# ka9q/ka9q-radio

Hardware: AMD Instinct MI355X
Metric: channels sustained @129.6 MS/s input (real-time-equivalent: channel-blocks/s / 50) (higher is better)
Workload: dtype f32; 1 GPU; config3: sig_gen real 129.6 MS/s, 1024 mixed usb/cw/iq 12 kHz channels (P=300), 1 MI355X; channels_total=1024, P=300, olen=240, N=3240000, L=2592000, M=648001, lanes=4

## Files before the change

include/chz_engine.h:

```cpp
#ifndef CHZ_ENGINE_H
#define CHZ_ENGINE_H
#include <stddef.h>
#ifdef __cplusplus
extern "C" {
#endif

#define CHZ_COMPLEX 1
#define CHZ_REAL    2
#define CHZ_ND      4

typedef struct chz_engine chz_engine;

typedef struct chz_info {
  int L, M, N, in_type, bins;
  int ring_blocks;
  int Na, Nb, Nc;
  int n_banks;
  int lanes;
  long spec_elems;
  int spec_na, spec_pitch, spec_off;
  char plan[320];
} chz_info;

typedef struct chz_timing {
  double total_ms;
  int blocks;
  double first_ms, cols_ms, rows_ms, notch_ms, chan_ms;
  int first_n, cols_n, rows_n, notch_n, chan_n;
  double enqueue_ms;
  double fix_ms; int fix_n;
  double demod_ms; int demod_n;
} chz_timing;

const char *chz_last_error(void);
int chz_process_exiting(void);
int chz_set_option(const char *name, const char *value);
int chz_device_count(void);

int chz_engine_create(chz_engine **out, int L, int M, int in_type, int device,
                      const char *plan_spec, int ring_blocks);
void chz_engine_destroy(chz_engine *e);
int chz_engine_info(const chz_engine *e, chz_info *info);
int chz_engine_set_stream(chz_engine *e, void *hip_stream);
int chz_sync(chz_engine *e);
int chz_engine_check(const chz_engine *e);

int chz_input_write(chz_engine *e, const float *host_samples, long n);
int chz_input_write_device(chz_engine *e, const float *dev_samples, long n);
int chz_input_write_i16(chz_engine *e, const short *host_samples, long n, float scale, int randomize);
int chz_input_write_i16_device(chz_engine *e, const short *dev_samples, long n, float scale, int randomize);
int chz_input_stats(chz_engine *e, int slot, unsigned long long *energy, unsigned *clips);
int chz_input_ring(chz_engine *e, float **dev_ring, long *ring_len_floats);
int chz_input_seek(chz_engine *e, unsigned job, const float *history);
int chz_input_mark(chz_engine *e, int k);
int chz_input_mark_wait(chz_engine *e, int k);
int chz_engine_notch_order(chz_engine *e, int by_event);

int chz_forward(chz_engine *e, unsigned job);
int chz_set_notches(chz_engine *e, const int *bins, int n, double alpha);
int chz_set_notches_alpha(chz_engine *e, const int *bins, const double *alpha, int n);
int chz_spectrum_read(chz_engine *e, int slot, float *host);
int chz_spectrum_device(chz_engine *e, int slot, float **dev);
int chz_slot_stream(chz_engine *e, int slot, void **hip_stream);
int chz_spectrum_attach(chz_engine *e, int slot, float *dev);

int chz_bank_create(chz_engine *e, int P, int olen, int capacity);
int chz_bank_create_real(chz_engine *e, int P, int olen, int capacity);
int chz_bank_create_shared(chz_engine *e, int P, int olen, int capacity, int nrows);
int chz_bank_set_rows(chz_engine *e, int bank, int ch0, int n, const int *rows);
int chz_bank_set_row_responses(chz_engine *e, int bank, int row0, int n, const float *resp);
int chz_bank_set_responses(chz_engine *e, int bank, int ch0, int n, const float *resp);
int chz_bank_set_shifts(chz_engine *e, int bank, int ch0, int n, const int *shifts);
int chz_bank_set_isb(chz_engine *e, int bank, int ch0, int n, const unsigned char *flags);
int chz_bank_set_beam(chz_engine *e, int bank, int ch0, int n, const double *ab, const unsigned char *on);
int chz_bank_set_active(chz_engine *e, int bank, int n);
int chz_bank_execute(chz_engine *e, int bank, unsigned job);
int chz_bank_execute_range(chz_engine *e, int bank, unsigned job, int ch0, int n);

int chz_bank_set_tuning(chz_engine *e, int bank, unsigned job, int ch0, int n, const int *shifts,
                        const double *freq, const double *rate);
int chz_bank_read_power(chz_engine *e, int bank, int slot, int ch0, int n, double *host);
int chz_bank_read_power_async(chz_engine *e, int bank, int slot, int ch0, int n, double *host);

int chz_bank_enable_noise(chz_engine *e, int bank, double samprate);
int chz_bank_read_noise(chz_engine *e, int bank, int slot, int ch0, int n, double *host);
int chz_bank_read_noise_async(chz_engine *e, int bank, int slot, int ch0, int n, double *host);
int chz_bank_destroy(chz_engine *e, int bank);
int chz_bank_read(chz_engine *e, int bank, int ch0, int n, float *host);
int chz_bank_read_async(chz_engine *e, int bank, int slot, int ch0, int n, float *host);
int chz_spectrum_read_async(chz_engine *e, int slot, float *host);
int chz_host_callback(chz_engine *e, int slot, void (*fn)(void *), void *arg);
int chz_slot_sync(chz_engine *e, int slot);
int chz_host_alloc(void **p, size_t bytes);
void chz_host_free(void *p);
int chz_host_register(void *p, size_t bytes);
void chz_host_unregister(void *p);
int chz_bank_output_device(chz_engine *e, int bank, int slot, float **dev);

int chz_step(chz_engine *e, unsigned job);

int chz_run_blocks(chz_engine *e, unsigned job0, int nblocks, int mode, int instrument,
                   chz_timing *timing);

#define CHZ_COMM_ID_BYTES 128
typedef struct chz_comm chz_comm;
int chz_comm_unique_id(void *id128);
int chz_comm_create(chz_comm **out, int rank, int world, const void *id128, int device);
int chz_comm_create_file(chz_comm **out, int rank, int world, const char *path, int device, double timeout_s);
int chz_comm_create_local(chz_comm **out, int n, const int *devices);
int chz_spectrum_broadcast_local(chz_engine *const *engines, chz_comm *const *comms, int n, int slot, int root);
void chz_comm_destroy(chz_comm *c);
int chz_comm_rank(const chz_comm *c);
int chz_comm_world(const chz_comm *c);
int chz_comm_barrier(chz_comm *c);
int chz_comm_allreduce_max(chz_comm *c, double *v, int n);
int chz_spectrum_broadcast(chz_engine *e, chz_comm *c, int slot, int root);
int chz_spectrum_exchange_rows(chz_engine *e, chz_comm *c, int slot, int root, const int *row_lo, const int *row_hi);
int chz_run_blocks_sharded(chz_engine *e, chz_comm *c, int root, int mode, const int *row_lo, const int *row_hi,
                           unsigned job0, int nblocks, chz_timing *timing);

#define CHZ_PCM_S16BE 0
#define CHZ_PCM_S16LE 1
#define CHZ_PCM_F32LE 2
#define CHZ_PCM_F32BE 3
#define CHZ_PCM_MULAW 4
#define CHZ_PCM_ALAW 5
#define CHZ_PCM_F16LE 6
#define CHZ_PCM_F16BE 7
typedef struct chz_demod_params {
  int channels;
  int env;
  int agc;
  int encoding;
  int snr_squelch;
  int squelch_tail;
  int tuned;
  int kind;
  double samprate;
  double headroom;
  double threshold, recovery_rate, hangtime, dc_alpha;
  double bandwidth;
  double shift;
  double squelch_open, squelch_close;
  double gain;
  double deemph_rate, deemph_gain;
  double threshold_extend;
  int pll_enable;
  int pll_square;
  double pll_loop_bw;
  double tone_freq;
} chz_demod_params;
#define CHZ_DEMOD_LINEAR 0
#define CHZ_DEMOD_FM 1
typedef struct chz_demod_status {
  int frame;
  int mute;
  int squelch_state;
  int pll_lock;
  double output_power;
  double gain;
  double n0;
  double snr;
  double foffset;
  double pdeviation;
  double pll_snr;
  double pll_cphase;
  double tone_deviation;
  int pll_rotations;
  int tone_mute;
} chz_demod_status;
int chz_bank_set_demod(chz_engine *e, int bank, unsigned job, int ch0, int n, const chz_demod_params *p, double blocktime);
int chz_bank_write_block(chz_engine *e, int bank, int slot, int ch0, int n, const float *samples, const double *bb_power, const double *n0);
int chz_bank_demod(chz_engine *e, int bank, unsigned job, int slot);
int chz_bank_demod_auto(chz_engine *e, int bank, int on);
int chz_bank_pcm_stride(chz_engine *e, int bank);
int chz_bank_set_pcm_stride(chz_engine *e, int bank, int bytes);
int chz_bank_read_pcm(chz_engine *e, int bank, int slot, int ch0, int n, void *pcm, chz_demod_status *status);
int chz_bank_read_pcm_async(chz_engine *e, int bank, int slot, int ch0, int n, void *pcm, chz_demod_status *status);
#define CHZ_FLAG_NO_SAMPLES 1
#define CHZ_FLAG_MUTE 2
#define CHZ_FLAG_PLL_LOCK 4
#define CHZ_FLAG_TONE_MUTE 8
int chz_bank_read_pcm_flags_async(chz_engine *e, int bank, int slot, int ch0, int n, void *pcm, unsigned char *flags);
int chz_bank_pcm_wait(chz_engine *e, int bank, int slot);

typedef struct chz_mini chz_mini;
int chz_mini_create(chz_mini **out, int L, int M, int capacity, int device);
void chz_mini_destroy(chz_mini *m);
int chz_mini_capacity(const chz_mini *m);
int chz_mini_add(chz_mini *m);
int chz_mini_release(chz_mini *m, int inst);
int chz_mini_set_response(chz_mini *m, int inst, const float *resp);
int chz_mini_execute(chz_mini *m, int n, const int *inst, const float *const *win, const int *shift, const unsigned char *isb,
                     float *const *out);

typedef struct chz_rmini chz_rmini;
int chz_rmini_create(chz_rmini **out, int L, int M, int nslaves, const int *olen, const int *out_type, int capacity, int device);
void chz_rmini_destroy(chz_rmini *m);
int chz_rmini_check(int L, int M, int nslaves, const int *olen, const int *out_type);
int chz_rmini_capacity(const chz_rmini *m);
int chz_rmini_add(chz_rmini *m);
int chz_rmini_release(chz_rmini *m, int inst);
int chz_rmini_set_response(chz_rmini *m, int inst, int slave, const float *resp);
int chz_rmini_execute(chz_rmini *m, int n, const int *inst, const float *const *win, const int *shift, const unsigned char *mask,
                      const unsigned char *isb, float *const *out);

int chz_welch_create(chz_engine *e, int fft_n, int capacity, int max_bins, int max_avg);
int chz_welch_destroy(chz_engine *e, int bank);
int chz_welch_set_window(chz_engine *e, int bank, int slot, const float *window);
// ... 21 lines not shown
```

ka9q-radio_amd/csrc/chz_engine.hip:

```cpp
#include <hip/hip_runtime.h>
#include <hip/hip_ext.h>
#include <atomic>
#include <condition_variable>
#include <cstdarg>
#include <cstdio>
#include <cstring>
#include <chrono>
#include <deque>
#include <functional>
#include <mutex>
#include <string>
#include <algorithm>
#include <vector>
#include <thread>
#include <cmath>
#include <unistd.h>
namespace chz_exit {
static std::atomic<int> exiting{0};
static std::atomic<long> inflight{0};
struct Scope {
  bool ok;
  Scope() { inflight.fetch_add(1, std::memory_order_seq_cst); ok = exiting.load(std::memory_order_seq_cst) == 0; }
  ~Scope() { inflight.fetch_sub(1, std::memory_order_release); }
};
// ... 47 lines not shown
  unsigned char* isb = nullptr;
  BeamDesc* beam = nullptr;
  std::vector<std::pair<int, int>> dirty[CHZ_ND];
  char* stage[CHZ_ND] = {nullptr, nullptr, nullptr, nullptr};
  hipEvent_t stage_ev[CHZ_ND][2] = {};
  bool stage_busy[CHZ_ND][2] = {};
  int stage_next[CHZ_ND] = {0, 0, 0, 0};
  float2* any_scratch = nullptr;
  DemodChan* dm_chan = nullptr;
  DemodState* dm_state = nullptr;
  DemodExt* dm_ext = nullptr;
  float2* dm_mix = nullptr;
  int dm_pll_lin = 0;
  int dm_fm_pll = 0, dm_fm_tone = 0;
  int dm_lin = 0, dm_fm = 0;
  int dm_fm_nopll = 0;
  DemodStatus* dm_status = nullptr;
  unsigned char* dm_flags = nullptr;
  unsigned char* dm_pcm = nullptr;
  std::vector<DemodChan> dm_chan_h;
  struct OscHost { bool init = false; double freq = 0.0, phase0 = 0.0; unsigned job0 = 0; };
  std::vector<OscHost> dm_osc;
  int shared_rows = 0;
  int dm_on = 0;
  bool dm_auto = true;
  int pcm_stride = 0;
  double dm_blocktime = 0.02;
  hipEvent_t ev_bank[CHZ_ND] = {nullptr, nullptr, nullptr, nullptr};
  hipEvent_t ev_tail[CHZ_ND] = {nullptr, nullptr, nullptr, nullptr};
  hipEvent_t ev_pcm[CHZ_ND] = {nullptr, nullptr, nullptr, nullptr};
  hipEvent_t ev_pcmgo[CHZ_ND] = {nullptr, nullptr, nullptr, nullptr};
  bool pcm_copying[CHZ_ND] = {false, false, false, false};
  bool tail_used[CHZ_ND] = {false, false, false, false};
  double* power = nullptr;
  double* agc_peak = nullptr;
  bool agc_peak_valid[CHZ_ND] = {false, false, false, false};
  double* n0 = nullptr;
  unsigned* noise_hint = nullptr;
  double noise_samprate = 0.0;
  BbRing* bb = nullptr;
  std::vector<BbRing> bb_h;
  int bb_n = 0;
  hipEvent_t ev_bb[CHZ_ND] = {nullptr, nullptr, nullptr, nullptr};
  bool bb_rec[CHZ_ND] = {false, false, false, false};
  unsigned bb_newest = 0;
  hipEvent_t bb_done = nullptr;
  int bb_busy = 0; unsigned bb_guard = 0;
};

struct Lane {
  hipStream_t s = nullptr;
  float2* buf = nullptr;
};

struct Issuer {
  std::thread th;
  std::mutex m;
  std::condition_variable cv;
  std::atomic<int> state{0};
  std::atomic<int> ready{0};
  bool sleeping = false;
  std::function<void()> fn;
  void loop() {
    for (;;) {
      const auto awake_until = std::chrono::steady_clock::now() + std::chrono::milliseconds(1);
      unsigned spins = 0;
      for (;;) {
        const int s = state.load(std::memory_order_acquire);
        if (s == 1 || s == 3) break;
        if ((++spins & 255u) || std::chrono::steady_clock::now() < awake_until) { __builtin_ia32_pause(); continue; }
        std::unique_lock<std::mutex> lk(m);
        sleeping = true;
        cv.wait(lk, [&] { const int t = state.load(std::memory_order_acquire); return t == 1 || t == 3; });
        sleeping = false;
      }
      if (state.load(std::memory_order_acquire) == 3) return;
      fn();
      state.store(2, std::memory_order_release);
    }
  }
  void post(std::function<void()> f) {
    fn = std::move(f);
    std::lock_guard<std::mutex> lk(m);
    state.store(1, std::memory_order_release);
    if (sleeping) cv.notify_one();
  }
  void wait() {
    while (state.load(std::memory_order_acquire) != 2) __builtin_ia32_pause();
    state.store(0, std::memory_order_release);
  }
  void quit() {
    { std::lock_guard<std::mutex> lk(m); state.store(3, std::memory_order_release); cv.notify_one(); }
    if (th.joinable()) th.join();
  }
};

struct NotchTurn {
  std::atomic<int> next{0};
  std::atomic<int> next_tail{0};
  std::atomic<int> abort{0};
};

#define CHZ_NOTCH_EVENTS 8
struct WelchBank;

struct chz_engine {
  int L = 0, M = 0, N = 0, in_type = 0, bins = 0, per = 1, device = 0, ring_blocks = 0;
  FwdPlan plan;
  float* energy[CHZ_ND] = {nullptr, nullptr, nullptr, nullptr};
  int noise_energy = -1;
  int demod_wave = -1;
  int chan_stage = -1;
  hipStream_t stream = nullptr;
  bool own_stream = false;
  hipStream_t upload = nullptr;
  hipStream_t tail = nullptr;
  hipStream_t pcmcopy = nullptr;
  Lane lanes[CHZ_MAX_LANES];
  int nlanes = 1;
#define CHZ_INPUT_MARKS 8
  hipEvent_t input_mark[CHZ_INPUT_MARKS] = {};
  hipEvent_t input_ready = nullptr;
  bool input_pending = false;
  float* ring = nullptr; long ring_len = 0;
  short* ring16 = nullptr; float scale16 = 1.0f; int derand = 0;
  unsigned long long* energy_part = nullptr; unsigned* clip_part = nullptr; int stat_n = 0;
  long wpos = 0;
  float2* spec[CHZ_ND] = {nullptr, nullptr, nullptr, nullptr};
  bool spec_owned[CHZ_ND] = {false, false, false, false};
  struct Blue {
    FwdPlan zp; long Mz = 0;
    float2* chirp = nullptr;
    float2* bf = nullptr;
    float2* za[CHZ_MAX_LANES] = {};
    float2* zs[CHZ_MAX_LANES] = {};
  };
  Blue* blue = nullptr;
  float2 *tw_sub_a = nullptr, *tw_sub_b = nullptr, *tw_sub_c = nullptr;
  float2 *tw1_tile = nullptr, *tw1_col = nullptr, *tw2_tile = nullptr, *tw2_col = nullptr, *tw2_full = nullptr;
  int n_notch = 0;
  int *notch_addr = nullptr, *notch_next = nullptr, *notch_head = nullptr;
  double* notch_alpha = nullptr; double* notch_state = nullptr;
  hipEvent_t notch_ev[CHZ_NOTCH_EVENTS] = {};
  unsigned notch_seq = 0; bool notch_have = false;
  bool opt_noise_hint = true, opt_pll_lane0 = false, opt_notch_fold = true;
  int notch_order = 0;
  long long notch_max_wait = 0;
  unsigned* notch_ver = nullptr;
  unsigned notch_tickets = 0;
  unsigned* notch_err = nullptr;
  NotchTables notch_tab; std::vector<double> notch_alpha_h;
  NotchOwn* notch_own = nullptr;
  RowsNotch notch_fold{};
  std::vector<Bank> banks;
  std::vector<WelchBank*> welch;
  hipStream_t welch_s = nullptr;
  hipEvent_t welch_in = nullptr, welch_done = nullptr;
  bool welch_busy = false;
  long long welch_lo = 0, welch_len = 0;
  hipGraphExec_t graph = nullptr; unsigned graph_job0 = 0; int graph_blocks = 0;
  int capture_blocks = 0;
  int graph_min_blocks = 32;
  hipEvent_t ev_t0 = nullptr, ev_t1 = nullptr, ev_fork = nullptr, ev_join[CHZ_MAX_LANES] = {nullptr, nullptr, nullptr, nullptr};
  hipEvent_t ev_begin[CHZ_MAX_LANES] = {nullptr, nullptr, nullptr, nullptr}, ev_end[CHZ_MAX_LANES] = {nullptr, nullptr, nullptr, nullptr}, ev_end_tail = nullptr;
  int tail_issued = 0;
  std::vector<Issuer*> issuers;
};

extern "C" { static int sync_all(chz_engine* e); }

template <class T> static int upload(T** dst, const std::vector<f2>& v) {
  *dst = nullptr;
  if (v.empty()) return 0;
  HIPOK(hipMalloc((void**)dst, v.size() * sizeof(f2)));
  HIPOK(hipMemcpy(*dst, v.data(), v.size() * sizeof(f2), hipMemcpyHostToDevice));
  return 0;
}

static void welch_free_all(chz_engine* e);
static void welch_bank_gone(chz_engine* e, int bank);
static int welch_guard(chz_engine* e, long long pos, long long n) {
  if (!e->welch_busy || n <= 0) return 0;
  const long long R = e->ring_len / e->per;
  { chz_exit::Scope xs; if (!xs.ok) return 0;
    if (hipEventQuery(e->welch_done) == hipSuccess) { e->welch_busy = false; return 0; }
    (void)hipGetLastError(); }
  const long long d1 = ((pos - e->welch_lo) % R + R) % R, d2 = ((e->welch_lo - pos) % R + R) % R;
  if (!(d1 < e->welch_len || d2 < n)) return 0;
  HIPOK(hipStreamWaitEvent(e->stream, e->welch_done, 0));
  e->welch_busy = false;
  return 0;
}

static void free_bank(Bank& b) {
  hipFree(b.resp); hipFree(b.desc); hipFree(b.out); hipFree(b.tw_sub); hipFree(b.any_scratch); b.any_scratch = nullptr;
  hipFree(b.fine); hipFree(b.power); hipFree(b.n0); hipFree(b.noise_hint); b.noise_hint = nullptr; hipFree(b.isb); hipFree(b.beam); hipFree(b.agc_peak); b.agc_peak = nullptr;
  hipFree(b.dm_chan); hipFree(b.dm_state); hipFree(b.dm_ext); hipFree(b.dm_status); hipFree(b.dm_flags); hipFree(b.dm_pcm); hipFree(b.dm_mix);
  b.dm_mix = nullptr; b.dm_pll_lin = 0; b.dm_fm_pll = 0; b.dm_fm_tone = 0; b.dm_lin = 0; b.dm_fm = 0; b.dm_fm_nopll = 0;
  b.dm_chan = nullptr; b.dm_state = nullptr; b.dm_ext = nullptr; b.dm_status = nullptr; b.dm_flags = nullptr; b.dm_pcm = nullptr; b.dm_on = 0; b.dm_chan_h.clear(); b.dm_osc.clear();
  for (int s = 0; s < CHZ_ND; s++) {
    if (b.ev_bank[s]) (void)hipEventDestroy(b.ev_bank[s]);
    if (b.ev_tail[s]) (void)hipEventDestroy(b.ev_tail[s]);
    if (b.ev_pcm[s]) (void)hipEventDestroy(b.ev_pcm[s]);
    if (b.ev_pcmgo[s]) (void)hipEventDestroy(b.ev_pcmgo[s]);
    b.ev_bank[s] = b.ev_tail[s] = b.ev_pcm[s] = b.ev_pcmgo[s] = nullptr; b.tail_used[s] = false; b.pcm_copying[s] = false;
  }
  hipFree(b.bb); b.bb = nullptr; b.bb_h.clear(); b.bb_n = 0; b.bb_busy = 0;
  if (b.bb_done) (void)hipEventDestroy(b.bb_done);
  b.bb_done = nullptr;
  for (int s = 0; s < CHZ_ND; s++) { if (b.ev_bb[s]) (void)hipEventDestroy(b.ev_bb[s]); b.ev_bb[s] = nullptr; b.bb_rec[s] = false; }
  for (int s = 0; s < CHZ_ND; s++) {
    if (b.stage[s]) (void)hipHostFree(b.stage[s]);
    for (int h = 0; h < 2; h++) { if (b.stage_ev[s][h]) (void)hipEventDestroy(b.stage_ev[s][h]); b.stage_ev[s][h] = nullptr; b.stage_busy[s][h] = false; }
    b.stage[s] = nullptr; b.stage_next[s] = 0; b.dirty[s].clear();
  }
  for (auto& r : b.retired) for (auto ev : r.ev) if (ev) (void)hipEventDestroy(ev);
  b.retired.clear(); b.free_rows.clear();
  b.resp = nullptr; b.desc = nullptr; b.out = nullptr; b.tw_sub = nullptr; b.fine = nullptr; b.power = nullptr;
  b.n0 = nullptr; b.isb = nullptr; b.beam = nullptr; b.noise_samprate = 0.0;
  b.desc_h.clear(); b.fine_h.clear(); b.fine_dh.clear(); b.isb_h.clear(); b.beam_h.clear();
  b.active = 0; b.cap = 0;
}

extern "C" {

int chz_process_exiting(void) { return chz_exit::exiting.load(std::memory_order_acquire); }
const char* chz_last_error(void) { return g_err; }

int chz_device_count(void) {
  int n = 0;
  if (hipGetDeviceCount(&n) != hipSuccess) return 0;
  return n;
}

int chz_gather_descriptor(int in_type, int master_bins, int P, int shift, int out6[6]) {
  ChanDescH d = make_chan_desc(in_type, master_bins, P, shift);
  out6[0] = d.t0; out6[1] = d.cnt; out6[2] = d.src0; out6[3] = d.dir; out6[4] = d.conj; out6[5] = d.wrap;
  return 0;
}

struct ChzOptions {
  int chan_stage = -1;
  int noise_energy = -1;
  int demod_wave = -1;
  int enq_threads = 2;
  int graph_blocks = 32;
  int notch_fold = 1;
  int noise_hint = 1;
  int pll_lane0 = 0;
  double notch_wait_ms = 3000.0;
  int fault_ticket_skew = 0;
  int allow_fault_injection = 0;
  int welch_packed = 1;
  char launch_id[64] = {0};
};
static ChzOptions g_opt;
static std::mutex g_opt_mu;
extern "C" int chz_set_option(const char* name, const char* value) {
  if (!name) return fail(-1, "null option name");
  std::lock_guard<std::mutex> lk(g_opt_mu);
  const ChzOptions def{};
  const bool d = value == nullptr || value[0] == 0;
  const int iv = d ? 0 : atoi(value);
  const std::string n(name);
  if (n == "chan_stage") g_opt.chan_stage = d ? def.chan_stage : (iv != 0);
  else if (n == "noise_energy") g_opt.noise_energy = d ? def.noise_energy : (iv != 0);
  else if (n == "demod_wave") g_opt.demod_wave = d ? def.demod_wave : (iv != 0);
  else if (n == "enq_threads") g_opt.enq_threads = d ? def.enq_threads : ((iv == 2 || iv == 4) ? iv : 1);
  else if (n == "graph_blocks") g_opt.graph_blocks = (d || iv <= 0 || iv > 4096) ? def.graph_blocks : iv;
  else if (n == "notch_fold") g_opt.notch_fold = d ? def.notch_fold : (value[0] != '0');
  else if (n == "noise_hint") g_opt.noise_hint = d ? def.noise_hint : (value[0] != '0');
  else if (n == "pll_lane0") g_opt.pll_lane0 = d ? def.pll_lane0 : 1;
  else if (n == "notch_wait_ms") g_opt.notch_wait_ms = (d || !(atof(value) > 0)) ? def.notch_wait_ms : atof(value);
  else if (n == "fault_ticket_skew") g_opt.fault_ticket_skew = d ? 0 : iv;
  else if (n == "allow_fault_injection") g_opt.allow_fault_injection = d ? 0 : (value[0] == '1');
  else if (n == "welch_packed") g_opt.welch_packed = d ? def.welch_packed : (iv != 0);
  else if (n == "launch_id") snprintf(g_opt.launch_id, sizeof g_opt.launch_id, "%s", d ? "" : value);
  else return fail(-1, "unknown option '%s'", name);
  return 0;
}
static ChzOptions options() { std::lock_guard<std::mutex> lk(g_opt_mu); return g_opt; }

static int own_queues() { static const int m = [] { const char* v = getenv("CHZ_OWN_QUEUES"); const int k = v ? atoi(v) : 1; return (k >= 0 && k <= 4) ? k : 1; }(); return m; }
static hipError_t stream_create_masked(hipStream_t* s, bool tail) {
#ifndef HIPEMU
  if (tail && own_queues() >= 3) {
    int lo = 0, hi = 0;
    if (hipDeviceGetStreamPriorityRange(&lo, &hi) == hipSuccess && lo != hi) {
      const hipError_t r = hipStreamCreateWithPriority(s, hipStreamNonBlocking, own_queues() == 3 ? hi : lo);
      if (r == hipSuccess) return r;
      (void)hipGetLastError();
    }
    return hipStreamCreateWithFlags(s, hipStreamNonBlocking);
  }
  if (own_queues() == 2 || (own_queues() == 1 && tail)) {
    int dev = 0, cus = 0;
    if (hipGetDevice(&dev) == hipSuccess && hipDeviceGetAttribute(&cus, hipDeviceAttributeMultiprocessorCount, dev) == hipSuccess && cus > 0 && cus <= 1024) {
      uint32_t mask[32] = {};
      for (int i = 0; i < cus; i++) mask[i / 32] |= 1u << (i % 32);
      const hipError_t r = hipExtStreamCreateWithCUMask(s, (uint32_t)((cus + 31) / 32), mask);
      if (r == hipSuccess) return r;
      (void)hipGetLastError();
    }
  }
#endif
  (void)tail;
  return hipStreamCreateWithFlags(s, hipStreamNonBlocking);
}

static int blue_setup(chz_engine* e);
int chz_engine_create(chz_engine** out, int L, int M, int in_type, int device, const char* plan_spec, int ring_blocks) {
  if (!out) return fail(-1, "null out pointer");
  *out = nullptr;
  if (L < 1 || M < 1) return fail(-1, "bad L/M");
  if (in_type != CHZ_REAL && in_type != CHZ_COMPLEX) return fail(-1, "in_type must be REAL or COMPLEX");
  int ndev = 0;
  if (hipGetDeviceCount(&ndev) != hipSuccess || ndev < 1)
    return fail(-2, "no HIP device: the channelizer engine has no CPU fallback");
  if (device < 0 || device >= ndev) return fail(-2, "device %d out of range (%d devices)", device, ndev);
  HIPOK(hipSetDevice(device));
  { void* probe = nullptr; HIPOK(hipMalloc(&probe, 256)); HIPOK(hipFree(probe)); }
  chz_exit::arm();
  const int N = L + M - 1;
  const int bins = in_type == CHZ_COMPLEX ? N : N / 2 + 1;
  if (bins < 2) return fail(-1, "transform too small");
  if (in_type == CHZ_REAL && (L & 1)) return fail(-1, "real input needs an even block length L");
  chz_engine* e = new chz_engine();
  struct Guard { chz_engine* e; ~Guard() { if (e) chz_engine_destroy(e); } } guard{e};
  e->L = L; e->M = M; e->N = N; e->in_type = in_type; e->bins = bins; e->device = device;
  e->per = in_type == CHZ_REAL ? 1 : 2;
  const char* envspec = getenv("CHZ_PLAN");
  if ((!plan_spec || !*plan_spec) && envspec && *envspec) plan_spec = envspec;
  if (!build_fwd_plan(N, in_type, plan_spec, e->plan)) {
    if (plan_spec && *plan_spec)
      return fail(-3, "no transform plan for N=%d (spec '%s'): N must factor into the compiled axis lengths, and no pass may want more than 1024 threads or 160 KB of LDS", N, plan_spec);
    chz_engine::Blue* bl = new chz_engine::Blue();
    e->blue = bl;
    double best = 1e300;
    for (long m = 2L * N - 1; m <= 4L * N + 4096 && m < (1L << 30); m++) {
      if (bl->Mz && (double)m > 1.04 * (double)bl->Mz + 64) break;
      { long r = m;
        for (int q : {2, 3, 5, 13, 19}) while (r % q == 0) r /= q;
        if (r != 1) continue; }
      FwdPlan cand; double sc = 0.0;
      if (!build_fwd_plan((int)m, CHZ_COMPLEX, nullptr, cand, &sc)) continue;
      if (!bl->Mz) bl->Mz = m;
      sc *= (double)m;
      if (sc < best) { best = sc; bl->zp = cand; }
    }
    if (bl->Mz) bl->Mz = bl->zp.N;
    if (!bl->Mz) return fail(-3, "no transform plan for N=%d, and no planned length above 2N-1 for the chirp-z form either", N);
    FwdPlan& q = e->plan;
    q = FwdPlan();
    q.N = N; q.in_type = in_type; q.bins = bins; q.Na = 128; q.Nb = 1; q.Nc = (bins + 127) / 128;
    q.spec_pitch = 128; q.spec_off = 0; q.spec_elems = (long)q.Nc * 128 + 16;
    char d[256];
    snprintf(d, sizeof d, "N=%d %s as chirp-z over [%s]", N, in_type == CHZ_REAL ? "real" : "complex", bl->zp.desc.c_str());
    q.desc = d;
  }
  const FwdPlan& tp = e->blue ? e->blue->zp : e->plan;
  if (fwd_lds_prepare(tp, !e->blue && in_type == CHZ_REAL))
    return fail(-3, "the forward kernels of N=%d (%s) cannot have the LDS their tiles need", N, tp.desc.c_str());
  const int minblocks = (N + L - 1) / L + 1;
  if (ring_blocks < minblocks) ring_blocks = minblocks < 8 ? 8 : minblocks;
  e->ring_blocks = ring_blocks;
  e->ring_len = (long)ring_blocks * L * e->per;
  HIPOK(stream_create_masked(&e->stream, false));
  e->own_stream = true;
  const ChzOptions opt = options();
  e->opt_noise_hint = opt.noise_hint != 0; e->opt_pll_lane0 = opt.pll_lane0 != 0; e->opt_notch_fold = opt.notch_fold != 0;
  if (opt.chan_stage >= 0) e->chan_stage = opt.chan_stage;
  if (opt.noise_energy >= 0) e->noise_energy = opt.noise_energy;
  if (opt.demod_wave >= 0) e->demod_wave = opt.demod_wave;
  const char* envl = getenv("CHZ_STREAMS");
  int nl = envl ? atoi(envl) : 4;
  e->nlanes = (nl >= 4) ? 4 : (nl >= 2) ? 2 : 1;
  HIPOK(hipEventCreateWithFlags(&e->input_ready, hipEventDisableTiming));
  HIPOK(hipEventCreate(&e->ev_t0)); HIPOK(hipEventCreate(&e->ev_t1));
  HIPOK(hipEventCreateWithFlags(&e->ev_fork, hipEventDisableTiming));
  for (int i = 0; i < CHZ_MAX_LANES; i++) HIPOK(hipEventCreateWithFlags(&e->ev_join[i], hipEventDisableTiming));
  for (int i = 0; i < CHZ_MAX_LANES; i++) { HIPOK(hipEventCreate(&e->ev_begin[i])); HIPOK(hipEventCreate(&e->ev_end[i])); }
  HIPOK(hipEventCreate(&e->ev_end_tail));
  for (int i = 0; i < CHZ_NOTCH_EVENTS; i++) HIPOK(hipEventCreateWithFlags(&e->notch_ev[i], hipEventDisableTiming | hipEventReleaseToDevice));
  {
    int khz = 0;
    if (hipDeviceGetAttribute(&khz, hipDeviceAttributeWallClockRate, e->device) != hipSuccess || khz <= 0) khz = 100000;
    const double ms = opt.notch_wait_ms;
    e->notch_max_wait = (long long)(ms * (double)khz);
  }
  e->graph_min_blocks = opt.graph_blocks;
  if (const char* no = getenv("CHZ_NOTCH_ORDER")) e->notch_order = strcmp(no, "event") == 0 ? 1 : (strcmp(no, "unordered-timing-only") == 0 ? 2 : 0);
  if (own_queues() == 2 && e->notch_order == 0) e->notch_order = 1;
  HIPOK(hipHostMalloc((void**)&e->notch_err, sizeof(unsigned), hipHostMallocMapped));
  *e->notch_err = 0;
  for (int i = 0; i < e->nlanes; i++) {
    if (i == 0) e->lanes[i].s = e->stream;
    else HIPOK(stream_create_masked(&e->lanes[i].s, false));
    HIPOK(hipMalloc((void**)&e->lanes[i].buf, sizeof(float2) * (size_t)tp.Ra * tp.inner));
  }
  HIPOK(hipMalloc((void**)&e->ring, sizeof(float) * (size_t)e->ring_len));
  HIPOK(hipMemset(e->ring, 0, sizeof(float) * (size_t)e->ring_len));
  e->wpos = (long)(M - 1) * e->per;
  for (int i = 0; i < CHZ_ND; i++) {
    HIPOK(hipMalloc((void**)&e->spec[i], sizeof(float2) * (size_t)e->plan.spec_elems));
    HIPOK(hipMemset(e->spec[i], 0, sizeof(float2) * (size_t)e->plan.spec_elems));
    e->spec_owned[i] = true;
  }
  int r;
  if ((r = upload(&e->tw_sub_a, tp.tw_sub_a)) || (r = upload(&e->tw_sub_b, tp.tw_sub_b)) ||
      (r = upload(&e->tw_sub_c, tp.tw_sub_c)) || (r = upload(&e->tw1_tile, tp.tw1_tile)) ||
      (r = upload(&e->tw1_col, tp.tw1_col)) || (r = upload(&e->tw2_tile, tp.tw2_tile)) ||
      (r = upload(&e->tw2_col, tp.tw2_col)) || (r = upload(&e->tw2_full, tp.tw2_full)))
    return r;
  HIPOK(hipDeviceSynchronize());
  if (e->blue) { r = blue_setup(e); if (r) return r; }
  guard.e = nullptr;
  *out = e;
  return 0;
}

static void drop_graph(chz_engine* e) {
  if (e->graph) { hipGraphExecDestroy(e->graph); e->graph = nullptr; }
}

static void free_notches(chz_engine* e) {
  hipFree(e->notch_addr); hipFree(e->notch_next); hipFree(e->notch_head); hipFree(e->notch_alpha); hipFree(e->notch_state); hipFree(e->notch_ver);
  hipFree(e->notch_own); e->notch_own = nullptr;
  e->notch_addr = e->notch_next = e->notch_head = nullptr; e->notch_alpha = nullptr; e->notch_state = nullptr; e->notch_ver = nullptr;
  e->n_notch = 0; e->notch_have = false; e->notch_tickets = 0; e->notch_fold = RowsNotch{};
}

void chz_engine_destroy(chz_engine* e) {
  if (!e) return;
  hipSetDevice(e->device);
  for (Issuer* is : e->issuers) { is->quit(); delete is; }
  e->issuers.clear();
  for (int i = 0; i < e->nlanes; i++) if (e->lanes[i].s) hipStreamSynchronize(e->lanes[i].s);
  if (e->upload) hipStreamSynchronize(e->upload);
  if (e->tail) hipStreamSynchronize(e->tail);
  if (e->pcmcopy) hipStreamSynchronize(e->pcmcopy);
  if (e->welch_s) hipStreamSynchronize(e->welch_s);
  drop_graph(e);
  welch_free_all(e);
  for (int i = 0; i < e->nlanes; i++) {
    hipFree(e->lanes[i].buf);
    if (i > 0 && e->lanes[i].s) hipStreamDestroy(e->lanes[i].s);
  }
  if (e->input_ready) hipEventDestroy(e->input_ready);
  for (auto ev : e->input_mark) if (ev) hipEventDestroy(ev);
  if (e->ev_t0) hipEventDestroy(e->ev_t0);
  if (e->ev_t1) hipEventDestroy(e->ev_t1);
  if (e->ev_fork) hipEventDestroy(e->ev_fork);
  for (auto ev : e->ev_join) if (ev) hipEventDestroy(ev);
  for (auto ev : e->ev_begin) if (ev) hipEventDestroy(ev);
  for (auto ev : e->ev_end) if (ev) hipEventDestroy(ev);
  if (e->ev_end_tail) hipEventDestroy(e->ev_end_tail);
  for (auto ev : e->notch_ev) if (ev) hipEventDestroy(ev);
  for (auto& b : e->banks) free_bank(b);
  hipFree(e->ring); hipFree(e->ring16); hipFree(e->energy_part); hipFree(e->clip_part);
  for (int i = 0; i < CHZ_ND; i++) if (e->spec_owned[i]) hipFree(e->spec[i]);
  for (int i = 0; i < CHZ_ND; i++) if (e->energy[i]) hipFree(e->energy[i]);
  if (e->blue) {
    hipFree(e->blue->chirp); hipFree(e->blue->bf);
    for (int i = 0; i < CHZ_MAX_LANES; i++) { hipFree(e->blue->za[i]); hipFree(e->blue->zs[i]); }
    delete e->blue;
  }
  hipFree(e->tw_sub_a); hipFree(e->tw_sub_b); hipFree(e->tw_sub_c);
  hipFree(e->tw1_tile); hipFree(e->tw1_col); hipFree(e->tw2_tile); hipFree(e->tw2_col); hipFree(e->tw2_full);
  free_notches(e);
  if (e->notch_err) (void)hipHostFree(e->notch_err);
  if (e->upload) hipStreamDestroy(e->upload);
  if (e->tail) hipStreamDestroy(e->tail);
  if (e->pcmcopy) hipStreamDestroy(e->pcmcopy);
  if (e->welch_s) hipStreamDestroy(e->welch_s);
  if (e->welch_in) hipEventDestroy(e->welch_in);
  if (e->welch_done) hipEventDestroy(e->welch_done);
  if (e->own_stream && e->stream) hipStreamDestroy(e->stream);
  delete e;
}

int chz_engine_info(const chz_engine* e, chz_info* info) {
  if (!e || !info) return fail(-1, "null argument");
  memset(info, 0, sizeof *info);
  info->L = e->L; info->M = e->M; info->N = e->N; info->in_type = e->in_type; info->bins = e->bins;
  info->ring_blocks = e->ring_blocks; info->Na = e->plan.Na; info->Nb = e->plan.Nb; info->Nc = e->plan.Nc;
  info->n_banks = (int)e->banks.size();
  info->spec_elems = e->plan.spec_elems; info->spec_na = e->plan.Na; info->spec_pitch = e->plan.spec_pitch; info->spec_off = e->plan.spec_off;
  info->lanes = e->nlanes;
  snprintf(info->plan, sizeof info->plan, "%s", e->plan.desc.c_str());
  return 0;
}

int chz_engine_set_stream(chz_engine* e, void* hip_stream) {
  if (e) { chz_exit::Scope _xd; if (_xd.ok) (void)hipSetDevice(e->device); }
  if (!e) return fail(-1, "null engine");
  int r = sync_all(e);
  if (r) return r;
  drop_graph(e);
  for (int i = 1; i < e->nlanes; i++) { hipFree(e->lanes[i].buf); hipStreamDestroy(e->lanes[i].s); e->lanes[i] = Lane(); }
  e->nlanes = 1;
  if (e->own_stream) { hipStreamDestroy(e->stream); e->own_stream = false; }
  e->stream = (hipStream_t)hip_stream;
  e->lanes[0].s = e->stream;
  e->notch_have = false;
  return 0;
}

static int check_device_errors(const chz_engine* e) {
  const unsigned v = e->notch_err ? __atomic_load_n(e->notch_err, __ATOMIC_ACQUIRE) : 0u;
  if (v) return fail(-8, "spur-notch ordering failed at ticket %u: a block's notch kernel waited for its predecessor in vain; "
                         "the engine must be re-created (CHZ_NOTCH_ORDER=event orders by HIP events instead)", v - 1u);
  return 0;
}
static int sync_all(chz_engine* e) {
  if (e) { chz_exit::Scope _xd; if (_xd.ok) (void)hipSetDevice(e->device); }
  for (int i = 0; i < e->nlanes; i++) HIPOK(hipStreamSynchronize(e->lanes[i].s));
  if (e->tail) HIPOK(hipStreamSynchronize(e->tail));
  if (e->pcmcopy) HIPOK(hipStreamSynchronize(e->pcmcopy));
  if (e->welch_s) { HIPOK(hipStreamSynchronize(e->welch_s)); e->welch_busy = false; for (auto& b : e->banks) b.bb_busy = 0; }
  for (auto& b : e->banks) for (int s = 0; s < CHZ_ND; s++) b.pcm_copying[s] = false;
  return check_device_errors(e);
}
int chz_sync(chz_engine* e) {
  if (!e) return fail(-1, "null engine");
  return sync_all(e);
}
int chz_engine_check(const chz_engine* e) {
  if (!e) return fail(-1, "null engine");
  return check_device_errors(e);
}

static int ring_write(chz_engine* e, const float* src, long n, hipMemcpyKind kind) {
  if (e) { chz_exit::Scope _xd; if (_xd.ok) (void)hipSetDevice(e->device); }
  if (e->ring16) return fail(-1, "int16 and float input cannot be mixed on one engine");
  const long nf = n * e->per;
  if (nf < 0 || nf > e->ring_len) return fail(-1, "write of %ld samples does not fit the ring", n);
  { int r = welch_guard(e, e->wpos / e->per, n); if (r) return r; }
  const long first = (e->wpos + nf <= e->ring_len) ? nf : e->ring_len - e->wpos;
  if (first > 0) HIPOK(hipMemcpyAsync(e->ring + e->wpos, src, sizeof(float) * (size_t)first, kind, e->stream));
  if (nf > first) HIPOK(hipMemcpyAsync(e->ring, src + first, sizeof(float) * (size_t)(nf - first), kind, e->stream));
  e->wpos = (e->wpos + nf) % e->ring_len;
  if (e->nlanes > 1) { HIPOK(hipEventRecord(e->input_ready, e->stream)); e->input_pending = true; }
  return 0;
}
int chz_input_write(chz_engine* e, const float* host, long n) {
  if (!e || !host) return fail(-1, "null argument");
  return ring_write(e, host, n, hipMemcpyHostToDevice);
}
int chz_input_write_device(chz_engine* e, const float* dev, long n) {
  if (!e || !dev) return fail(-1, "null argument");
  return ring_write(e, dev, n, hipMemcpyDeviceToDevice);
}
static inline int blue_grid(long n);
static int ring16_write(chz_engine* e, const short* src, long n, float scale, int randomize, hipMemcpyKind kind) {
  if (e->in_type != CHZ_REAL) return fail(-1, "int16 input is a real A/D stream");
  if (n < 0 || n > e->ring_len) return fail(-1, "write of %ld samples does not fit the ring", n);
  HIPOK(hipSetDevice(e->device));
  if (!e->ring16) {
    if (e->wpos != (long)(e->M - 1)) return fail(-1, "int16 and float input cannot be mixed on one engine");
    HIPOK(hipMalloc((void**)&e->ring16, sizeof(short) * (size_t)e->ring_len));
    HIPOK(hipMemset(e->ring16, 0, sizeof(short) * (size_t)e->ring_len));
    e->stat_n = e->blue ? blue_grid(e->blue->Mz) * 4 : e->plan.grid1 * (e->plan.block1 / 64);
    HIPOK(hipMalloc((void**)&e->energy_part, sizeof(unsigned long long) * (size_t)CHZ_ND * e->stat_n));
    HIPOK(hipMalloc((void**)&e->clip_part, sizeof(unsigned) * (size_t)CHZ_ND * e->stat_n));
    HIPOK(hipMemset(e->energy_part, 0, sizeof(unsigned long long) * (size_t)CHZ_ND * e->stat_n));
    HIPOK(hipMemset(e->clip_part, 0, sizeof(unsigned) * (size_t)CHZ_ND * e->stat_n));
    HIPOK(hipDeviceSynchronize());
    drop_graph(e);
  }
  if (scale != e->scale16 || (randomize != 0) != (e->derand != 0)) drop_graph(e);
  e->scale16 = scale; e->derand = randomize != 0;
  { int r = welch_guard(e, e->wpos, n); if (r) return r; }
  const long first = (e->wpos + n <= e->ring_len) ? n : e->ring_len - e->wpos;
  if (first > 0) HIPOK(hipMemcpyAsync(e->ring16 + e->wpos, src, sizeof(short) * (size_t)first, kind, e->stream));
  if (n > first) HIPOK(hipMemcpyAsync(e->ring16, src + first, sizeof(short) * (size_t)(n - first), kind, e->stream));
  e->wpos = (e->wpos + n) % e->ring_len;
  if (e->nlanes > 1) { HIPOK(hipEventRecord(e->input_ready, e->stream)); e->input_pending = true; }
  return 0;
}
int chz_input_write_i16(chz_engine* e, const short* host, long n, float scale, int randomize) {
  if (!e || !host) return fail(-1, "null argument");
  return ring16_write(e, host, n, scale, randomize, hipMemcpyHostToDevice);
}
int chz_input_write_i16_device(chz_engine* e, const short* dev, long n, float scale, int randomize) {
  if (!e || !dev) return fail(-1, "null argument");
  return ring16_write(e, dev, n, scale, randomize, hipMemcpyDeviceToDevice);
}
int chz_input_stats(chz_engine* e, int slot, unsigned long long* energy, unsigned* clips) {
  if (e) { chz_exit::Scope _xd; if (_xd.ok) (void)hipSetDevice(e->device); }
  if (!e || slot < 0 || slot >= CHZ_ND) return fail(-1, "bad argument");
  if (!e->ring16) return fail(-1, "input statistics exist for int16 input only");
  std::vector<unsigned long long> en((size_t)e->stat_n); std::vector<unsigned> cl((size_t)e->stat_n);
  hipStream_t st = e->lanes[slot % e->nlanes].s;
  HIPOK(hipMemcpyAsync(en.data(), e->energy_part + (size_t)slot * e->stat_n, sizeof(unsigned long long) * en.size(), hipMemcpyDeviceToHost, st));
  HIPOK(hipMemcpyAsync(cl.data(), e->clip_part + (size_t)slot * e->stat_n, sizeof(unsigned) * cl.size(), hipMemcpyDeviceToHost, st));
  HIPOK(hipStreamSynchronize(st));
  unsigned long long se = 0; unsigned sc = 0;
  for (size_t i = 0; i < en.size(); i++) { se += en[i]; sc += cl[i]; }
  if (energy) *energy = se;
  if (clips) *clips = sc;
  return 0;
}
int chz_input_seek(chz_engine* e, unsigned job, const float* history) {
  if (!e) return fail(-1, "null engine");
  if (e->ring16) return fail(-1, "chz_input_seek re-seats a float ring (this engine takes int16 input)");
  HIPOK(hipSetDevice(e->device));
  { int r = sync_all(e); if (r) return r; }
  const long start = (long)(((unsigned long long)job * (unsigned long long)e->L) % (unsigned long long)((long)e->ring_blocks * e->L)) * e->per;
  const long nh = (long)(e->M - 1) * e->per;
  e->wpos = start;
  if (history) { int r = ring_write(e, history, e->M - 1, hipMemcpyHostToDevice); if (r) return r; }
  else {
    const long first = (start + nh <= e->ring_len) ? nh : e->ring_len - start;
    if (first > 0) HIPOK(hipMemsetAsync(e->ring + start, 0, sizeof(float) * (size_t)first, e->stream));
    if (nh > first) HIPOK(hipMemsetAsync(e->ring, 0, sizeof(float) * (size_t)(nh - first), e->stream));
    e->wpos = (start + nh) % e->ring_len;
  }
  HIPOK(hipStreamSynchronize(e->stream));
  e->input_pending = false;
  return 0;
}
int chz_input_mark(chz_engine* e, int k) {
  if (e) { chz_exit::Scope _xd; if (_xd.ok) (void)hipSetDevice(e->device); }
  if (!e || k < 0 || k >= CHZ_INPUT_MARKS) return fail(-1, "bad argument");
  if (!e->input_mark[k]) HIPOK(hipEventCreateWithFlags(&e->input_mark[k], hipEventDisableTiming));
  HIPOK(hipEventRecord(e->input_mark[k], e->stream));
  return 0;
}
int chz_input_mark_wait(chz_engine* e, int k) {
  if (e) { chz_exit::Scope _xd; if (_xd.ok) (void)hipSetDevice(e->device); }
  if (!e || k < 0 || k >= CHZ_INPUT_MARKS) return fail(-1, "bad argument");
  if (e->input_mark[k]) HIPOK(hipEventSynchronize(e->input_mark[k]));
  return 0;
}
int chz_engine_notch_order(chz_engine* e, int by_event) {
  if (!e) return fail(-1, "null engine");
  { int r = sync_all(e); if (r) return r; }
  drop_graph(e);
  e->notch_order = by_event ? 1 : 0;
  e->notch_have = false;
  return 0;
}
int chz_input_ring(chz_engine* e, float** dev_ring, long* ring_len_floats) {
  if (!e) return fail(-1, "null engine");
  if (dev_ring) *dev_ring = e->ring;
  if (ring_len_floats) *ring_len_floats = e->ring_len;
  return 0;
}

struct Instr {
  Instr() = default;
  Instr(const Instr&) = delete;
  ~Instr() { for (auto e : ev) hipEventDestroy(e); }
  bool on = false;
  std::vector<hipEvent_t> ev;
  std::vector<int> kind;
  hipEvent_t e0 = nullptr, e1 = nullptr;
};
static void mark(Instr* in, hipStream_t, int kind, bool begin) {
  if (!in || !in->on) return;
  if (begin) {
    hipEventCreate(&in->e0); hipEventCreate(&in->e1);
    in->ev.push_back(in->e0); in->ev.push_back(in->e1); in->kind.push_back(kind);
  } else { in->e0 = nullptr; in->e1 = nullptr; }
}
#define IN_E0(in) ((in) && (in)->on ? (in)->e0 : nullptr)
#define IN_E1(in) ((in) && (in)->on ? (in)->e1 : nullptr)

static inline int lane_of(const chz_engine* e, unsigned job, const Instr* in) {
  return (in && in->on) ? 0 : (int)(job % (unsigned)e->nlanes);
}

static int enqueue_notch(chz_engine* e, int slot, hipStream_t st, Instr* in, NotchTurn* turn, int seq, bool capture_first, bool capturing) {
  if (e->n_notch <= 0) return 0;
  if (turn) {
    while (turn->next.load(std::memory_order_acquire) != seq) {
      if (turn->abort.load(std::memory_order_relaxed)) return fail(-6, "another issuing thread failed");
      __builtin_ia32_pause();
    }
  }
  int rc = 0;
  const bool by_event = e->notch_order == 1;
  do {
    if (by_event && e->notch_have && !capture_first && e->nlanes > 1) {
      hipError_t he = hipStreamWaitEvent(st, e->notch_ev[(e->notch_seq - 1u) % CHZ_NOTCH_EVENTS], 0);
      if (he != hipSuccess) { rc = fail(-10, "hipStreamWaitEvent failed: %s", hipGetErrorString(he)); break; }
    }
    NotchFixParams q{};
    q.spec = e->spec[slot]; q.addr = e->notch_addr; q.next = e->notch_next; q.head = e->notch_head;
    q.alpha = e->notch_alpha; q.state = e->notch_state; q.n = e->n_notch;
    e->notch_tab.fill_inline(q, e->notch_alpha_h.data());
    q.err = e->notch_err; q.max_wait = e->notch_max_wait;
    const bool ticket = !by_event && e->nlanes > 1 && e->notch_order != 2;
    if (ticket && capturing) {
      q.ver = e->notch_ver; q.seq_base = e->notch_ver + 2; q.seq = (unsigned)seq;
      q.adv = seq == e->capture_blocks - 1 ? (unsigned)e->capture_blocks : 0u;
    } else if (ticket) { q.ver = e->notch_ver; q.seq = e->notch_tickets; }
    mark(in, st, 5, true);
    if (launch_notch_fix(st, q, IN_E0(in), IN_E1(in))) { rc = fail(-4, "notch list too long"); break; }
    mark(in, st, 5, false);
    if (ticket && !capturing) e->notch_tickets++;
    if (by_event && e->nlanes > 1) {
      hipError_t he = hipEventRecord(e->notch_ev[e->notch_seq % CHZ_NOTCH_EVENTS], st);
      if (he != hipSuccess) { rc = fail(-10, "hipEventRecord failed: %s", hipGetErrorString(he)); break; }
      e->notch_seq++; e->notch_have = true;
    }
  } while (0);
  if (turn) {
    if (rc) turn->abort.store(1, std::memory_order_relaxed);
    turn->next.store(seq + 1, std::memory_order_release);
  }
  return rc;
}

static int blue_fft(chz_engine* e, const float2* za, float2* lbuf, float2* zs, hipStream_t st) {
  const FwdPlan& p = e->blue->zp;
  ColsParams a{};
  a.in = za; a.in_len = 0; a.in_start = 0; a.out = lbuf; a.rows = 1; a.inner = p.inner; a.T = p.T1; a.padk = p.padk1;
  a.tw_sub = e->tw_sub_a; a.tw_tile = e->tw1_tile; a.tw_col = e->tw1_col;
  if (launch_cols(p.ra, p.grid1, p.block1, p.lds1, st, a)) return fail(-4, "no kernel for axis a");
  if (p.Nb > 1) {
    ColsParams b{};
    b.in = lbuf; b.in_len = 0; b.in_start = 0; b.out = lbuf; b.rows = p.Ra; b.inner = p.Nc; b.T = p.T2;
    b.padk = p.padk2; b.tw_sub = e->tw_sub_b; b.tw_tile = e->tw2_tile; b.tw_col = e->tw2_col; b.tw_full = e->tw2_full;
    if (launch_cols(p.rb, p.grid2, p.block2, p.lds2, st, b)) return fail(-4, "no kernel for axis b");
  }
  RowsParams c{};
  c.lay = SpecLayout{p.Na, p.spec_pitch, p.spec_off}; c.ka_shift = p.ka_shift;
  c.buf = lbuf; c.spec = zs; c.Ra = p.Ra; c.Na = p.Na; c.Nb = p.Nb; c.Ta = p.Ta; c.ld = p.ld3;
  c.padg = p.padg3; c.N = p.N; c.mirror = false; c.tw_sub = e->tw_sub_c;
  if (launch_rows(p.rc, p.grid3, p.block3, p.lds3, st, c)) return fail(-4, "no kernel for axis c");
  return 0;
}
static inline int blue_grid(long n) { const long g = (n + 255) / 256; return (int)(g > 4096 ? 4096 : (g < 1 ? 1 : g)); }
static int blue_setup(chz_engine* e) {
  chz_engine::Blue& b = *e->blue;
  const int N = e->N; const long Mz = b.Mz;
  std::vector<f2> c((size_t)N);
  for (long n = 0; n < N; n++) c[(size_t)n] = root_of_unity((long long)((unsigned long long)n * (unsigned long long)n % (unsigned long long)(2L * N)), 2LL * N, -1);
  int r = upload(&b.chirp, c);
  if (r) return r;
  for (int i = 0; i < e->nlanes; i++) {
    HIPOK(hipMalloc((void**)&b.za[i], sizeof(float2) * (size_t)Mz));
    HIPOK(hipMalloc((void**)&b.zs[i], sizeof(float2) * (size_t)b.zp.spec_elems));
    HIPOK(hipMemset(b.zs[i], 0, sizeof(float2) * (size_t)b.zp.spec_elems));
  }
  HIPOK(hipMalloc((void**)&b.bf, sizeof(float2) * (size_t)b.zp.spec_elems));
  std::vector<f2> bz((size_t)Mz, f2{0.f, 0.f});
  for (long m = 0; m < N; m++) {
    const f2 v{c[(size_t)m].x, -c[(size_t)m].y};
    bz[(size_t)m] = v;
    if (m) bz[(size_t)(Mz - m)] = v;
  }
  HIPOK(hipMemcpy(b.za[0], bz.data(), sizeof(f2) * (size_t)Mz, hipMemcpyHostToDevice));
  HIPOK(hipDeviceSynchronize());
  r = blue_fft(e, b.za[0], e->lanes[0].buf, b.zs[0], e->stream);
  if (r) return r;
  HIPOK(hipMemcpyAsync(b.bf, b.zs[0], sizeof(float2) * (size_t)b.zp.spec_elems, hipMemcpyDeviceToDevice, e->stream));
  HIPOK(hipStreamSynchronize(e->stream));
  HIPOK(hipGetLastError());
  return 0;
}
static int enqueue_forward_blue(chz_engine* e, unsigned job, int ln, hipStream_t st, long start, Instr* in) {
  chz_engine::Blue& b = *e->blue;
  const int slot = job % CHZ_ND;
  float2* lbuf = e->lanes[ln].buf;
  const SpecLayout zlay{b.zp.Na, b.zp.spec_pitch, b.zp.spec_off};
  mark(in, st, 0, true);
  BluePreParams pre{e->ring, e->ring_len, start, e->per, b.chirp, b.za[ln], e->N, b.Mz, nullptr, 1.0f, 0, 0, nullptr, nullptr};
  if (e->ring16) {
    pre.ring16 = e->ring16; pre.scale16 = e->scale16; pre.derand = e->derand; pre.new_from = e->M - 1;
    pre.energy_part = e->energy_part + (size_t)slot * e->stat_n; pre.clip_part = e->clip_part + (size_t)slot * e->stat_n;
  }
  CHZ_LAUNCH(blue_pre, blue_grid(b.Mz), 256, 0, st, IN_E0(in), IN_E1(in), pre);
  mark(in, st, 0, false);
  int r = blue_fft(e, b.za[ln], lbuf, b.zs[ln], st);
  if (r) return r;
  mark(in, st, 1, true);
  BlueMulParams mul{b.zs[ln], b.bf, b.za[ln], zlay, b.Mz};
  CHZ_LAUNCH(blue_mul, blue_grid(b.Mz), 256, 0, st, IN_E0(in), IN_E1(in), mul);
  mark(in, st, 1, false);
  r = blue_fft(e, b.za[ln], lbuf, b.zs[ln], st);
  if (r) return r;
  mark(in, st, 2, true);
  BluePostParams post{b.zs[ln], b.chirp, e->spec[slot], zlay, SpecLayout{e->plan.Na, e->plan.spec_pitch, e->plan.spec_off}, e->bins, (float)(1.0 / (double)b.Mz)};
  CHZ_LAUNCH(blue_post, blue_grid(e->bins), 256, 0, st, IN_E0(in), IN_E1(in), post);
  mark(in, st, 2, false);
  return 0;
}

static int enqueue_forward(chz_engine* e, unsigned job, Instr* in, NotchTurn* turn = nullptr, int seq = 0, bool capture_first = false, bool capturing = false) {
  const FwdPlan& p = e->plan;
  const int slot = job % CHZ_ND;
  const int ln = lane_of(e, job, in);
  hipStream_t st = e->lanes[ln].s;
  float2* lbuf = e->lanes[ln].buf;
  if (ln != 0 && e->input_pending) HIPOK(hipStreamWaitEvent(st, e->input_ready, 0));
  const long start = (long)(((unsigned long long)job * (unsigned long long)e->L) % (unsigned long long)((long)e->ring_blocks * e->L)) * e->per;
  if (e->blue) {
    const int r = enqueue_forward_blue(e, job, ln, st, start, in);
    return r ? r : enqueue_notch(e, slot, st, in, turn, seq, capture_first, capturing);
  }
  if (e->in_type == CHZ_REAL) {
    FirstRealParams a{};
    a.ring = e->ring; a.ring_len = e->ring_len; a.start = start; a.buf = lbuf; a.inner = p.inner;
    a.T = p.T1; a.Ra = p.Ra; a.padk = p.padk1; a.tw_sub = e->tw_sub_a; a.tw_tile = e->tw1_tile; a.tw_col = e->tw1_col;
#if CHZ_TW_SHUFFLE
    if (p.T1 != 16) return fail(-4, "this A/B build generates its twiddles across rows of 16 lanes: T1 must be 16");
#endif
    if (e->ring16) {
      a.ring16 = e->ring16; a.scale16 = e->scale16; a.derand = e->derand; a.new_from = e->M - 1;
      a.energy_part = e->energy_part + (size_t)slot * e->stat_n; a.clip_part = e->clip_part + (size_t)slot * e->stat_n;
    }
    mark(in, st, 0, true);
    if (launch_first_real(p.ra, p.grid1, p.block1, p.lds1, st, a, IN_E0(in), IN_E1(in))) return fail(-4, "no kernel for axis a");
    mark(in, st, 0, false);
  } else {
    ColsParams a{};
    a.in = reinterpret_cast<const float2*>(e->ring); a.in_len = e->ring_len / 2; a.in_start = start / 2;
    a.out = lbuf; a.rows = 1; a.inner = p.inner; a.T = p.T1; a.padk = p.padk1;
    a.tw_sub = e->tw_sub_a; a.tw_tile = e->tw1_tile; a.tw_col = e->tw1_col;
    mark(in, st, 0, true);
    if (launch_cols(p.ra, p.grid1, p.block1, p.lds1, st, a, IN_E0(in), IN_E1(in))) return fail(-4, "no kernel for axis a");
    mark(in, st, 0, false);
  }
  if (p.Nb > 1) {
    ColsParams b{};
    b.in = lbuf; b.in_len = 0; b.in_start = 0; b.out = lbuf; b.rows = p.Ra; b.inner = p.Nc; b.T = p.T2;
    b.padk = p.padk2; b.tw_sub = e->tw_sub_b; b.tw_tile = e->tw2_tile; b.tw_col = e->tw2_col;
    b.tw_full = e->tw2_full;
    mark(in, st, 1, true);
    if (launch_cols(p.rb, p.grid2, p.block2, p.lds2, st, b, IN_E0(in), IN_E1(in))) return fail(-4, "no kernel for axis b");
    mark(in, st, 1, false);
  }
  RowsParams c{};
  c.lay = SpecLayout{p.Na, p.spec_pitch, p.spec_off}; c.ka_shift = p.ka_shift;
  c.buf = lbuf; c.spec = e->spec[slot]; c.Ra = p.Ra; c.Na = p.Na; c.Nb = p.Nb; c.Ta = p.Ta; c.ld = p.ld3;
  c.padg = p.padg3; c.N = p.N; c.mirror = e->in_type == CHZ_REAL; c.tw_sub = e->tw_sub_c;
  const bool by_event = e->notch_order == 1;
  const bool fold = e->n_notch > 0 && e->notch_fold.n > 0 && !by_event && e->notch_order != 2;
  if (fold) {
    if (turn) {
      while (turn->next.load(std::memory_order_acquire) != seq) {
        if (turn->abort.load(std::memory_order_relaxed)) return fail(-6, "another issuing thread failed");
        __builtin_ia32_pause();
      }
    }
    c.nf = e->notch_fold;
    c.nf.state = e->notch_state; c.nf.err = e->notch_err; c.nf.max_wait = e->notch_max_wait;
    const bool ticket = e->nlanes > 1;
    if (ticket && capturing) {
      c.nf.ver = e->notch_ver; c.nf.seq_base = e->notch_ver + 2; c.nf.seq = (unsigned)seq;
      c.nf.adv = seq == e->capture_blocks - 1 ? (unsigned)e->capture_blocks : 0u;
    } else if (ticket) { c.nf.ver = e->notch_ver; c.nf.seq = e->notch_tickets; }
    mark(in, st, 2, true);
    const int lr = launch_rows(p.rc, p.grid3, p.block3, p.lds3, st, c, IN_E0(in), IN_E1(in));
    mark(in, st, 2, false);
    if (!lr && ticket && !capturing) e->notch_tickets++;
    if (turn) {
      if (lr) turn->abort.store(1, std::memory_order_relaxed);
      turn->next.store(seq + 1, std::memory_order_release);
    }
    if (lr) return fail(-4, "no kernel for axis c");
    return 0;
  }
  mark(in, st, 2, true);
  if (launch_rows(p.rc, p.grid3, p.block3, p.lds3, st, c, IN_E0(in), IN_E1(in))) return fail(-4, "no kernel for axis c");
  mark(in, st, 2, false);
  return enqueue_notch(e, slot, st, in, turn, seq, capture_first, capturing);
}

static inline size_t bank_sample_bytes(const Bank& b) { return b.out_real ? sizeof(float) : sizeof(float2); }
static inline float2* bank_out(const Bank& b, int slot) {
  return reinterpret_cast<float2*>(reinterpret_cast<char*>(b.out) + (size_t)slot * b.cap * b.olen * bank_sample_bytes(b));
}
static inline char* bank_out_at(const Bank& b, int slot, int ch) {
  return reinterpret_cast<char*>(bank_out(b, slot)) + (size_t)ch * b.olen * bank_sample_bytes(b);
}

#define CHZ_DIRTY_MAX 16
static inline void mark_dirty(Bank& b, int ch0, int n) {
  if (n <= 0) return;
  for (int s = 0; s < CHZ_ND; s++) {
    auto& d = b.dirty[s];
    int lo = ch0, hi = ch0 + n;
    size_t i = 0;
    while (i < d.size() && d[i].second < lo) i++;
    size_t j = i;
    while (j < d.size() && d[j].first <= hi) { if (d[j].first < lo) lo = d[j].first; if (d[j].second > hi) hi = d[j].second; j++; }
    d.erase(d.begin() + (long)i, d.begin() + (long)j);
    d.insert(d.begin() + (long)i, std::make_pair(lo, hi));
    while (d.size() > CHZ_DIRTY_MAX) {
      size_t best = 0; int gap = d[1].first - d[0].second;
      for (size_t k = 1; k + 1 < d.size(); k++) if (d[k + 1].first - d[k].second < gap) { gap = d[k + 1].first - d[k].second; best = k; }
      d[best].second = d[best + 1].second;
      d.erase(d.begin() + (long)best + 1);
    }
  }
}
static inline size_t stage_bytes_per_channel() { return sizeof(ChanDesc) + sizeof(FineDesc) + sizeof(BeamDesc) + 1; }

static int refresh_slot(chz_engine* e, Bank& b, int slot, hipStream_t st) {
  if (b.dirty[slot].empty()) return 0;
  const int chunk = b.cap < CHZ_STAGE_CAP ? b.cap : CHZ_STAGE_CAP;
  const size_t half_bytes = (stage_bytes_per_channel() * (size_t)chunk + 64 + 63) & ~(size_t)63;
  if (!b.stage[slot]) {
    HIPOK(hipHostMalloc((void**)&b.stage[slot], 2 * half_bytes, hipHostMallocDefault));
    for (int h = 0; h < 2; h++) HIPOK(hipEventCreateWithFlags(&b.stage_ev[slot][h], hipEventDisableTiming));
  }
  for (const auto& range : b.dirty[slot]) {
    const int lo = range.first, hi = range.second > b.cap ? b.cap : range.second;
    for (int c0 = lo; c0 < hi; c0 += chunk) {
      const int n = hi - c0 < chunk ? hi - c0 : chunk;
      const int h = b.stage_next[slot]; b.stage_next[slot] ^= 1;
      if (b.stage_busy[slot][h]) HIPOK(hipEventSynchronize(b.stage_ev[slot][h]));
      char* sp = b.stage[slot] + (size_t)h * half_bytes;
      PushParams pp{};
      auto seg = [&](void* dst, const void* src, size_t bytes) {
        memcpy(sp, src, bytes);
        pp.seg[pp.nseg].dst = dst; pp.seg[pp.nseg].src = sp; pp.seg[pp.nseg].bytes = (unsigned)bytes; pp.nseg++;
        sp += (bytes + 7) & ~(size_t)7;
      };
      seg(b.desc + (size_t)slot * b.cap + c0, b.desc_h.data() + c0, sizeof(ChanDesc) * (size_t)n);
      if (b.fine) seg(b.fine + (size_t)slot * b.cap + c0, b.fine_dh.data() + c0, sizeof(FineDesc) * (size_t)n);
      if (b.beam) seg(b.beam + (size_t)slot * b.cap + c0, b.beam_h.data() + c0, sizeof(BeamDesc) * (size_t)n);
      if (b.isb) seg(b.isb + (size_t)slot * b.cap + c0, b.isb_h.data() + c0, (size_t)n);
      launch_desc_push(pp, st);
      HIPOK(hipEventRecord(b.stage_ev[slot][h], st));
      b.stage_busy[slot][h] = true;
    }
  }
  b.dirty[slot].clear();
  return 0;
}
static int refresh_all_bulk(chz_engine* e, Bank& b) {
  int r = sync_all(e);
  if (r) return r;
  for (int s = 0; s < CHZ_ND; s++) {
    for (const auto& range : b.dirty[s]) {
      const int lo = range.first, hi = range.second > b.cap ? b.cap : range.second;
      if (lo >= hi) continue;
      const size_t n = (size_t)(hi - lo), off = (size_t)s * b.cap + lo;
      HIPOK(hipMemcpy(b.desc + off, b.desc_h.data() + lo, sizeof(ChanDesc) * n, hipMemcpyHostToDevice));
      if (b.fine) HIPOK(hipMemcpy(b.fine + off, b.fine_dh.data() + lo, sizeof(FineDesc) * n, hipMemcpyHostToDevice));
      if (b.beam) HIPOK(hipMemcpy(b.beam + off, b.beam_h.data() + lo, sizeof(BeamDesc) * n, hipMemcpyHostToDevice));
      if (b.isb) HIPOK(hipMemcpy(b.isb + off, b.isb_h.data() + lo, n, hipMemcpyHostToDevice));
    }
    b.dirty[s].clear();
  }
  return 0;
}
static int after_edit(chz_engine* e, Bank& b, int ch0, int n) {
  mark_dirty(b, ch0, n);
  if (n > CHZ_STAGE_CAP) return refresh_all_bulk(e, b);
  return 0;
}

static void demod_paths(const chz_engine* e, const Bank& b, DemodParams& d) {
  d.lin_lanes = (b.dm_lin > 0 && (e->demod_wave == 0 || (e->demod_wave < 0 && b.dm_lin >= 65536))) ? 1 : 0;
  d.fm_lanes = (b.dm_fm_nopll > 0 && b.dm_mix != nullptr && (e->demod_wave == 0 || (e->demod_wave < 0 && b.dm_fm_nopll >= 65536))) ? 1 : 0;
  if (d.fm_lanes) d.mix = b.dm_mix;
  const bool fm_wave = b.dm_fm > 0 && (!d.fm_lanes || b.dm_fm > b.dm_fm_nopll);
  const bool lin_wave = b.dm_lin > 0 && (!d.lin_lanes || (b.dm_pll_lin > 0 && d.mix == nullptr));
  d.wave_any = (fm_wave || lin_wave) ? 1 : 0;
}
static int enqueue_bb_append(chz_engine* e, Bank& b, unsigned job, int slot, hipStream_t st, int ch0, int n, bool whole) {
  const auto by_ch = [](const BbRing& a, int ch) { return a.ch < ch; };
  const int lo = (int)(std::lower_bound(b.bb_h.begin(), b.bb_h.end(), ch0, by_ch) - b.bb_h.begin());
  const int hi = (int)(std::lower_bound(b.bb_h.begin(), b.bb_h.end(), ch0 + n, by_ch) - b.bb_h.begin());
  if (hi <= lo) return 0;
  if (__atomic_load_n(&b.bb_busy, __ATOMIC_ACQUIRE) && (int)(job - b.bb_guard) > 0) HIPOK(hipStreamWaitEvent(st, b.bb_done, 0));
  const int prev = (slot + CHZ_ND - 1) % CHZ_ND;
  if (whole && b.bb_rec[prev]) HIPOK(hipStreamWaitEvent(st, b.ev_bb[prev], 0));
  BbAppendParams q{};
  q.out = bank_out(b, slot); q.list = b.bb; q.first = lo; q.olen = b.olen; q.job = job;
  launch_bb_append(q, hi - lo, st);
  HIPOK(hipEventRecord(b.ev_bb[slot], st));
  b.bb_rec[slot] = true;
  unsigned cur = __atomic_load_n(&b.bb_newest, __ATOMIC_RELAXED);
  while (whole && (int)(job - cur) > 0 && !__atomic_compare_exchange_n(&b.bb_newest, &cur, job, true, __ATOMIC_RELAXED, __ATOMIC_RELAXED)) {}
  return 0;
}
static int enqueue_bank(chz_engine* e, int bank, unsigned job, Instr* in, int ch0 = 0, int n = -1, bool partial = false) {
  Bank& b = e->banks[(size_t)bank];
  if (n < 0) n = b.active;
  if (n <= 0 || !b.resp) return 0;
  const int slot = (int)(job % CHZ_ND);
  hipStream_t st = e->lanes[lane_of(e, (unsigned)slot, in)].s;
  __atomic_store_n(&b.last_slot, slot, __ATOMIC_RELAXED);
  { int r = refresh_slot(e, b, slot, st); if (r) return r; }
  const bool whole_bank = !partial && ch0 == 0 && n == b.active;
  if (b.tail_used[slot] && !(in && in->on)) HIPOK(hipStreamWaitEvent(st, b.ev_tail[slot], 0));
  const size_t so = (size_t)slot * b.cap;
  ChanParams c{};
  if (!chan_layout(c, SpecLayout{e->plan.Na, e->plan.spec_pitch, e->plan.spec_off}, e->bins)) return fail(-4, "spectrum layout beyond the reach of the index reciprocal");
  c.spec = e->spec[slot]; c.resp = b.resp; c.desc = b.desc + so; c.out = bank_out(b, slot); c.ch0 = ch0; c.nch = n; c.olen = b.olen;
  c.tw_sub = b.tw_sub;
  c.stage = e->chan_stage >= 0 ? e->chan_stage : (n >= 16384);
  c.isb = b.isb ? b.isb + so : nullptr; c.beam = b.beam ? b.beam + so : nullptr;
  c.fine = b.fine ? b.fine + so : nullptr; c.power = b.power ? b.power + so : nullptr; c.job = job;
  if (b.fine) fine_launch(c, 1 + e->L / (e->M - 1), job);
  const bool peaks = b.agc_peak && whole_bank && c.stage && !b.g.any && !b.out_real && (c.fine || c.power) && b.dm_on > 0 && b.dm_auto &&
                     b.dm_lin > b.dm_pll_lin && (e->demod_wave == 0 || (e->demod_wave < 0 && b.dm_lin >= 65536));
  if (peaks) { c.agc_peak = b.agc_peak + so; int sps = (int)std::rint(b.olen * .002 / b.dm_blocktime); c.agc_sps = sps < 1 ? 1 : sps; }
  if (whole_bank) b.agc_peak_valid[slot] = peaks;
  const int per_block = b.g.any ? 1 : b.g.wpb * b.g.cpw;
  const int grid = (n + per_block - 1) / per_block;
  mark(in, st, 4, true);
  if (b.g.any) {
    c.m_bins = e->bins; c.m_real = e->in_type == CHZ_REAL;
    if (b.out_real) { c.fine = nullptr; c.power = nullptr; }
    if (launch_chan_any(b.g, n, st, c, b.tw_sub, b.out_real != 0, b.any_scratch ? b.any_scratch + (size_t)slot * b.cap * 2 * b.g.lb + (size_t)ch0 * 2 * b.g.lb : nullptr,
                        IN_E0(in), IN_E1(in))) return fail(-4, "no scratch for P=%d", b.P);
  } else if (b.out_real) {
    c.m_bins = e->bins; c.m_real = e->in_type == CHZ_REAL; c.fine = nullptr; c.power = nullptr; c.stage = 0;
    if (launch_chan_real(b.g.r, grid, b.g.wpb * 64, b.g.lds, st, c, IN_E0(in), IN_E1(in))) return fail(-4, "no real-output kernel for P=%d", b.P);
  } else if (launch_chan(b.g.r, grid, b.g.wpb * 64, b.g.lds, st, c, IN_E0(in), IN_E1(in))) return fail(-4, "no kernel for P=%d", b.P);
  mark(in, st, 4, false);
  if (b.bb_n > 0) { int r = enqueue_bb_append(e, b, job, slot, st, ch0, n, whole_bank); if (r) return r; }
  if (b.n0 && b.noise_samprate > 0.0) {
// ... 575 lines not shown
  HIPOK(hipGetLastError());
  return 0;
}
int chz_bank_pcm_stride(chz_engine* e, int bank) {
  BANK_CHECK(e, bank, 0, 0);
  const Bank& b = e->banks[(size_t)bank];
  return b.pcm_stride ? b.pcm_stride : b.olen * 8;
}
int chz_bank_set_pcm_stride(chz_engine* e, int bank, int bytes) {
  if (e) { chz_exit::Scope _xd; if (_xd.ok) (void)hipSetDevice(e->device); }
  BANK_CHECK(e, bank, 0, 0);
  Bank& b = e->banks[(size_t)bank];
  if (b.dm_chan) return fail(-1, "the PCM row size is fixed once demodulators exist");
  if (bytes < b.olen || bytes > 8 * b.olen || (bytes & 3)) return fail(-1, "PCM rows hold %d..%d bytes, a multiple of 4", b.olen, 8 * b.olen);
  b.pcm_stride = bytes;
  return 0;
}
static int read_pcm(chz_engine* e, int bank, int slot, int ch0, int n, void* pcm, chz_demod_status* status, bool wait) {
  BANK_CHECK(e, bank, ch0, n);
  if (slot < 0 || slot >= CHZ_ND) return fail(-1, "bad slot");
  Bank& b = e->banks[(size_t)bank];
  if (!b.dm_chan) return fail(-1, "bank has no demodulator: call chz_bank_set_demod first");
  static_assert(sizeof(chz_demod_status) == sizeof(DemodStatus), "status layouts must agree");
  const size_t so = (size_t)slot * b.cap + ch0, stride = (size_t)b.pcm_stride;
  if (b.pcm_copying[slot]) HIPOK(hipStreamWaitEvent(e->tail, b.ev_pcm[slot], 0));
  if (pcm) HIPOK(hipMemcpyAsync(pcm, b.dm_pcm + so * stride, stride * (size_t)n, hipMemcpyDeviceToHost, e->tail));
  if (status) HIPOK(hipMemcpyAsync(status, b.dm_status + so, sizeof(DemodStatus) * (size_t)n, hipMemcpyDeviceToHost, e->tail));
  HIPOK(hipEventRecord(b.ev_pcm[slot], e->tail));
  if (wait) HIPOK(hipStreamSynchronize(e->tail));
  return 0;
}
int chz_bank_read_pcm_flags_async(chz_engine* e, int bank, int slot, int ch0, int n, void* pcm, unsigned char* flags) {
  if (e) { chz_exit::Scope _xd; if (_xd.ok) (void)hipSetDevice(e->device); }
  BANK_CHECK(e, bank, ch0, n);
  if (slot < 0 || slot >= CHZ_ND) return fail(-1, "bad slot");
  Bank& b = e->banks[(size_t)bank];
  if (!b.dm_chan) return fail(-1, "bank has no demodulator: call chz_bank_set_demod first");
  const size_t so = (size_t)slot * b.cap + ch0, stride = (size_t)b.pcm_stride;
  if (!e->pcmcopy) HIPOK(stream_create_masked(&e->pcmcopy, true));
  HIPOK(hipEventRecord(b.ev_pcmgo[slot], e->tail));
  HIPOK(hipStreamWaitEvent(e->pcmcopy, b.ev_pcmgo[slot], 0));
  if (pcm) HIPOK(hipMemcpyAsync(pcm, b.dm_pcm + so * stride, stride * (size_t)n, hipMemcpyDeviceToHost, e->pcmcopy));
  if (flags) HIPOK(hipMemcpyAsync(flags, b.dm_flags + so, (size_t)n, hipMemcpyDeviceToHost, e->pcmcopy));
  HIPOK(hipEventRecord(b.ev_pcm[slot], e->pcmcopy));
  b.pcm_copying[slot] = true;
  return 0;
}
int chz_bank_pcm_wait(chz_engine* e, int bank, int slot) {
  if (e) { chz_exit::Scope _xd; if (_xd.ok) (void)hipSetDevice(e->device); }
  BANK_CHECK(e, bank, 0, 0);
  if (slot < 0 || slot >= CHZ_ND) return fail(-1, "bad slot");
  Bank& b = e->banks[(size_t)bank];
  if (!b.dm_chan) return fail(-1, "bank has no demodulator: call chz_bank_set_demod first");
  HIPOK(hipEventSynchronize(b.ev_pcm[slot]));
  return check_device_errors(e);
}
int chz_bank_read_pcm(chz_engine* e, int bank, int slot, int ch0, int n, void* pcm, chz_demod_status* status) {
  return read_pcm(e, bank, slot, ch0, n, pcm, status, true);
}
int chz_bank_read_pcm_async(chz_engine* e, int bank, int slot, int ch0, int n, void* pcm, chz_demod_status* status) {
  if (e) { chz_exit::Scope _xd; if (_xd.ok) (void)hipSetDevice(e->device); }
  return read_pcm(e, bank, slot, ch0, n, pcm, status, false);
}
int chz_bank_set_active(chz_engine* e, int bank, int n) {
  BANK_CHECK(e, bank, 0, n);
  if (e->banks[(size_t)bank].active != n) drop_graph(e);
  e->banks[(size_t)bank].active = n;
  return 0;
}
int chz_bank_execute(chz_engine* e, int bank, unsigned job) {
  BANK_CHECK(e, bank, 0, 0);
  HIPOK(hipSetDevice(e->device));
  int r = enqueue_bank(e, bank, job, nullptr);
  if (r) return r;
  HIPOK(hipGetLastError());
  return 0;
}
int chz_bank_execute_range(chz_engine* e, int bank, unsigned job, int ch0, int n) {
  BANK_CHECK(e, bank, ch0, n);
  HIPOK(hipSetDevice(e->device));
  int r = enqueue_bank(e, bank, job, nullptr, ch0, n, true);
  if (r) return r;
  HIPOK(hipGetLastError());
  return 0;
}
int chz_bank_destroy(chz_engine* e, int bank) {
  if (e) { chz_exit::Scope _xd; if (_xd.ok) (void)hipSetDevice(e->device); }
  BANK_CHECK(e, bank, 0, 0);
  Bank& b = e->banks[(size_t)bank];
  { int r = sync_all(e); if (r) return r; }
  drop_graph(e);
  welch_bank_gone(e, bank);
  free_bank(b);
  return 0;
}
int chz_bank_read_async(chz_engine* e, int bank, int slot, int ch0, int n, float* host) {
  if (e) { chz_exit::Scope _xd; if (_xd.ok) (void)hipSetDevice(e->device); }
  BANK_CHECK(e, bank, ch0, n);
  if (slot < 0 || slot >= CHZ_ND) return fail(-1, "bad slot");
  Bank& b = e->banks[(size_t)bank];
  if (n == 0) return 0;
  HIPOK(hipMemcpyAsync(host, bank_out_at(b, slot, ch0), bank_sample_bytes(b) * (size_t)n * b.olen,
                       hipMemcpyDeviceToHost, slot_stream(e, slot)));
  return 0;
}
int chz_spectrum_read_async(chz_engine* e, int slot, float* host) {
  if (e) { chz_exit::Scope _xd; if (_xd.ok) (void)hipSetDevice(e->device); }
  if (!e || !host || slot < 0 || slot >= CHZ_ND) return fail(-1, "bad argument");
  return copy_spectrum(e, slot, host, slot_stream(e, slot));
}
int chz_host_callback(chz_engine* e, int slot, void (*fn)(void*), void* arg) {
  if (e) { chz_exit::Scope _xd; if (_xd.ok) (void)hipSetDevice(e->device); }
  if (e && fn && slot == CHZ_SLOT_WELCH && e->welch_s) { HIPOK(hipLaunchHostFunc(e->welch_s, fn, arg)); return 0; }
  if (!e || !fn || slot < 0 || slot >= CHZ_ND) return fail(-1, "bad argument");
  HIPOK(hipLaunchHostFunc(slot_stream(e, slot), fn, arg));
  return 0;
}
int chz_slot_sync(chz_engine* e, int slot) {
  if (e) { chz_exit::Scope _xd; if (_xd.ok) (void)hipSetDevice(e->device); }
  if (e && slot == CHZ_SLOT_WELCH && e->welch_s) { HIPOK(hipStreamSynchronize(e->welch_s)); return 0; }
  if (!e || slot < 0 || slot >= CHZ_ND) return fail(-1, "bad argument");
  HIPOK(hipStreamSynchronize(slot_stream(e, slot)));
  return 0;
}
int chz_host_alloc(void** p, size_t bytes) {
  if (!p) return fail(-1, "null pointer");
  HIPOK(hipHostMalloc(p, bytes ? bytes : 1, hipHostMallocPortable));
  return 0;
}
void chz_host_free(void* p) { if (p) (void)hipHostFree(p); }
int chz_host_register(void* p, size_t bytes) {
  if (!p || !bytes) return fail(-1, "bad argument");
  hipError_t e = hipHostRegister(p, bytes, hipHostRegisterPortable);
  if (e != hipSuccess) { (void)hipGetLastError(); return fail(-10, "hipHostRegister failed: %s", hipGetErrorString(e)); }
  return 0;
}
void chz_host_unregister(void* p) { if (p) (void)hipHostUnregister(p); }
int chz_bank_read(chz_engine* e, int bank, int ch0, int n, float* host) {
  if (e) { chz_exit::Scope _xd; if (_xd.ok) (void)hipSetDevice(e->device); }
  BANK_CHECK(e, bank, ch0, n);
  Bank& b = e->banks[(size_t)bank];
  hipStream_t st = slot_stream(e, b.last_slot);
  HIPOK(hipMemcpyAsync(host, bank_out_at(b, b.last_slot, ch0), bank_sample_bytes(b) * (size_t)n * b.olen, hipMemcpyDeviceToHost, st));
  HIPOK(hipStreamSynchronize(st));
  return 0;
}
int chz_bank_output_device(chz_engine* e, int bank, int slot, float** dev) {
  BANK_CHECK(e, bank, 0, 0);
  if (slot < 0 || slot >= CHZ_ND) return fail(-1, "bad slot");
  *dev = reinterpret_cast<float*>(bank_out(e->banks[(size_t)bank], slot));
  return 0;
}

static int enqueue_step(chz_engine* e, unsigned job, Instr* in, NotchTurn* turn = nullptr, int seq = 0, bool capture_first = false, bool capturing = false) {
  int r = enqueue_forward(e, job, in, turn, seq, capture_first, capturing);
  if (r) return r;
  bool demod = false;
  for (const Bank& b : e->banks) demod = demod || b.dm_on > 0 || b.bb_n > 0;
  if (demod && turn) {
    while (turn->next_tail.load(std::memory_order_acquire) != seq) {
      if (turn->abort.load(std::memory_order_relaxed)) return fail(-6, "another issuing thread failed");
      __builtin_ia32_pause();
    }
  }
  for (int b = 0; b < (int)e->banks.size() && !r; b++) r = enqueue_bank(e, b, job, in);
  if (demod && turn) {
    if (r) turn->abort.store(1, std::memory_order_relaxed);
    turn->next_tail.store(seq + 1, std::memory_order_release);
  }
  return r;
}

int chz_step(chz_engine* e, unsigned job) {
  if (!e) return fail(-1, "null engine");
  HIPOK(hipSetDevice(e->device));
  int r = enqueue_step(e, job, nullptr);
  if (r) return r;
  HIPOK(hipGetLastError());
  return 0;
}

static int lanes_fork(chz_engine* e, hipEvent_t ev) {
  if (e->nlanes < 2) return 0;
  HIPOK(hipEventRecord(ev, e->lanes[0].s));
  for (int i = 1; i < e->nlanes; i++) HIPOK(hipStreamWaitEvent(e->lanes[i].s, ev, 0));
  return 0;
}
static int lanes_join(chz_engine* e, hipEvent_t* evs) {
  for (int i = 1; i < e->nlanes; i++) {
    HIPOK(hipEventRecord(evs[i], e->lanes[i].s));
    HIPOK(hipStreamWaitEvent(e->lanes[0].s, evs[i], 0));
  }
  return 0;
}

static int issue_threads() {
  return options().enq_threads;
}

int chz_run_blocks(chz_engine* e, unsigned job0, int nblocks, int mode, int instrument, chz_timing* timing) {
  if (!e || nblocks < 0) return fail(-1, "bad argument");
  if (mode == 1)
    for (const Bank& b : e->banks)
      if (b.fine || b.dm_on || b.bb_n) return fail(-5, "graph replay bakes the block number into the captured launches; fine-tuned and demodulated banks and banks with attached spectrum analysers need eager mode");
  HIPOK(hipSetDevice(e->device));
  { int r = sync_all(e); if (r) return r; }
  e->input_pending = false;
  e->notch_have = false;
  e->tail_issued = 0;
  hipEvent_t t0 = e->ev_t0, t1 = e->ev_t1, fork_ev = e->ev_fork;
  hipEvent_t* join_ev = e->ev_join;
  Instr in; in.on = instrument != 0 && mode == 0;
  const bool host_join = mode == 0 && !in.on;
  hipStream_t s0 = e->lanes[0].s;
  int done = 0, rc = 0;
  const auto host_t0 = std::chrono::steady_clock::now();
  if (mode == 1) {
    int unit = e->ring_blocks;
    while (unit % CHZ_ND) unit += e->ring_blocks;
    int cycle = unit;
    while (cycle < e->graph_min_blocks && cycle + unit <= nblocks) cycle += unit;
    const unsigned phase = job0 % (unsigned)unit;
    if (!e->graph || e->graph_blocks != cycle || e->graph_job0 != phase) {
      drop_graph(e);
      for (Bank& b : e->banks) { int r = refresh_all_bulk(e, b); if (r) return r; }
      hipGraph_t g = nullptr;
      e->capture_blocks = cycle;
      HIPOK(hipStreamBeginCapture(s0, hipStreamCaptureModeThreadLocal));
      rc = lanes_fork(e, fork_ev);
      for (int i = 0; i < cycle && !rc; i++) rc = enqueue_step(e, phase + (unsigned)i, nullptr, nullptr, i, i == 0, true);
      if (!rc) rc = lanes_join(e, join_ev);
      hipError_t ce = hipStreamEndCapture(s0, &g);
      e->capture_blocks = 0;
      e->notch_have = false;
      if (rc) { if (g) hipGraphDestroy(g); return rc; }
      if (ce != hipSuccess) return fail(-10, "graph capture failed: %s", hipGetErrorString(ce));
      HIPOK(hipGraphInstantiate(&e->graph, g, nullptr, nullptr, 0));
      hipGraphDestroy(g);
      e->graph_blocks = cycle; e->graph_job0 = phase;
    }
    for (Bank& b : e->banks) { int r = refresh_all_bulk(e, b); if (r) return r; }
    const bool graph_ticket = e->n_notch > 0 && e->nlanes > 1 && e->notch_order == 0;
    if (graph_ticket)
      HIPOK(hipMemsetD32Async(reinterpret_cast<hipDeviceptr_t>(e->notch_ver + 2), (int)e->notch_tickets, 1, s0));
    HIPOK(hipEventRecord(t0, s0));
    while (nblocks - done >= cycle) {
      HIPOK(hipGraphLaunch(e->graph, s0)); done += cycle;
      if (graph_ticket) e->notch_tickets += (unsigned)cycle;
    }
    if (done < nblocks) {
      if ((rc = lanes_fork(e, fork_ev))) return rc;
      for (; done < nblocks; done++) if ((rc = enqueue_step(e, job0 + (unsigned)done, nullptr))) return rc;
      if ((rc = lanes_join(e, join_ev))) return rc;
    }
  } else {
    if (!host_join) HIPOK(hipEventRecord(t0, s0));
    if (!host_join && !in.on && (rc = lanes_fork(e, fork_ev))) return rc;
    auto issue = [&](int b, Instr* ins, NotchTurn* turn) -> int {
      const unsigned job = job0 + (unsigned)b;
      const int ln = (int)(job % (unsigned)e->nlanes);
      if (host_join && b < e->nlanes) HIPOK(hipEventRecord(e->ev_begin[ln], e->lanes[ln].s));
      const int r = enqueue_step(e, job, ins, turn, b);
      if (r) return r;
      if (host_join && b >= nblocks - e->nlanes) HIPOK(hipEventRecord(e->ev_end[ln], e->lanes[ln].s));
      return 0;
    };
    const int T = issue_threads();
    if (T > 1 && !in.on && e->nlanes >= T) {
      while ((int)e->issuers.size() < T - 1) {
        Issuer* is = new Issuer();
        const int dev = e->device;
        is->th = std::thread([is, dev] { (void)hipSetDevice(dev); is->ready.store(1, std::memory_order_release); is->loop(); });
        e->issuers.push_back(is);
      }
    }
    bool issuers_ready = T > 1 && (int)e->issuers.size() >= T - 1;
    for (int t = 1; t < T && issuers_ready; t++) issuers_ready = e->issuers[(size_t)(t - 1)]->ready.load(std::memory_order_acquire) != 0;
    if (issuers_ready && !in.on && done == 0 && e->nlanes >= T && nblocks >= 2 * e->nlanes) {
      NotchTurn turn;
      std::vector<int> rcs((size_t)T, 0);
      std::vector<std::string> errs((size_t)T);
      auto work = [&](int t) {
        for (int b = done; b < nblocks && !rcs[(size_t)t]; b++) {
          const unsigned job = job0 + (unsigned)b;
          if ((int)(job % (unsigned)e->nlanes) % T != t) continue;
          if ((rcs[(size_t)t] = issue(b, nullptr, &turn))) { errs[(size_t)t] = g_err; turn.abort.store(1); }
        }
      };
      for (int t = 1; t < T; t++) e->issuers[(size_t)(t - 1)]->post([&work, t] { work(t); });
      work(0);
      for (int t = 1; t < T; t++) e->issuers[(size_t)(t - 1)]->wait();
      for (size_t t = 0; t < rcs.size(); t++) if (rcs[t]) return fail(rcs[t], "%s", errs[t].c_str());
      for (Bank& b : e->banks) b.last_slot = (int)((job0 + (unsigned)nblocks - 1u) % CHZ_ND);
      done = nblocks;
    }
    for (; done < nblocks; done++) if ((rc = issue(done, &in, nullptr))) return rc;
    if (!host_join && !in.on && (rc = lanes_join(e, join_ev))) return rc;
  }
  double enqueue_ms = 0.0, total_ms = 0.0;
  if (host_join) {
    const bool tail = __atomic_load_n(&e->tail_issued, __ATOMIC_RELAXED) != 0;
    if (tail) HIPOK(hipEventRecord(e->ev_end_tail, e->tail));
    enqueue_ms = std::chrono::duration<double, std::milli>(std::chrono::steady_clock::now() - host_t0).count();
    const int used = nblocks < e->nlanes ? nblocks : e->nlanes;
    for (int i = 0; i < used; i++) HIPOK(hipEventSynchronize(e->ev_end[(job0 + (unsigned)i) % (unsigned)e->nlanes]));
    if (tail) HIPOK(hipEventSynchronize(e->ev_end_tail));
    HIPOK(hipGetLastError());
    if (timing && used > 0) {
      hipEvent_t ref = e->ev_begin[job0 % (unsigned)e->nlanes];
      float lo = 0.f, hi = 0.f, d = 0.f;
      for (int i = 0; i < used; i++) {
        const unsigned ln = (job0 + (unsigned)i) % (unsigned)e->nlanes;
        if (i) { HIPOK(hipEventElapsedTime(&d, ref, e->ev_begin[ln])); if (d < lo) lo = d; }
        HIPOK(hipEventElapsedTime(&d, ref, e->ev_end[ln])); if (d > hi) hi = d;
      }
      if (tail) { HIPOK(hipEventElapsedTime(&d, ref, e->ev_end_tail)); if (d > hi) hi = d; }
      total_ms = (double)hi - (double)lo;
    }
  } else {
    if (e->tail && !in.on) {
      HIPOK(hipEventRecord(join_ev[0], e->tail));
      HIPOK(hipStreamWaitEvent(s0, join_ev[0], 0));
    }
    HIPOK(hipEventRecord(t1, s0));
    enqueue_ms = std::chrono::duration<double, std::milli>(std::chrono::steady_clock::now() - host_t0).count();
    HIPOK(hipEventSynchronize(t1));
    HIPOK(hipGetLastError());
    if (timing) { float ms = 0; HIPOK(hipEventElapsedTime(&ms, t0, t1)); total_ms = ms; }
  }
  if (timing) {
    memset(timing, 0, sizeof *timing);
    timing->enqueue_ms = enqueue_ms;
    timing->total_ms = total_ms; timing->blocks = nblocks;
    double* acc[7] = {&timing->first_ms, &timing->cols_ms, &timing->rows_ms, &timing->notch_ms, &timing->chan_ms, &timing->fix_ms, &timing->demod_ms};
    int* cnt[7] = {&timing->first_n, &timing->cols_n, &timing->rows_n, &timing->notch_n, &timing->chan_n, &timing->fix_n, &timing->demod_n};
    for (size_t i = 0; i < in.kind.size(); i++) {
      float k = 0; hipEventElapsedTime(&k, in.ev[2 * i], in.ev[2 * i + 1]);
      *acc[in.kind[i]] += k; *cnt[in.kind[i]] += 1;
    }
  }
  return 0;
}

}

#include "chz_comm.inc"
#include "chz_mini.inc"
#include "chz_rmini.inc"
#include "chz_welch.inc"
```

ka9q-radio_amd/csrc/chz_kernels.h:

```cpp
#pragma once
#include <hip/hip_runtime.h>
#include "regfft.h"

#if defined(__HIP_DEVICE_COMPILE__)
#define CHZ_ROUNDED_F32(x) asm volatile("" : "+v"(x))
#define CHZ_ROUNDED_F64(x) asm volatile("" : "+v"(x))
#else
#define CHZ_ROUNDED_F32(x) ((void)0)
#define CHZ_ROUNDED_F64(x) ((void)0)
#endif

#if defined(__HIP_DEVICE_COMPILE__)
#define CHZ_WAVE_SYNC() __builtin_amdgcn_wave_barrier()
#elif defined(HIPEMU)
#define CHZ_WAVE_SYNC() hipemu_wave_barrier(hipemu_linear_tid())
#else
#define CHZ_WAVE_SYNC() ((void)0)
#endif

namespace chz {

#ifndef CHZ_WT
#define CHZ_WT 1
#endif
// ... 329 lines not shown
__global__ void fwd_cols(ColsParams p) {
  constexpr int NP = R1 * R2;
  HIP_DYNAMIC_SHARED(float2, lds)
  const int tid = threadIdx.x;
  const int T = p.T;
  const int tpr = p.inner / T;
  const int row = blockIdx.x / tpr, ct = blockIdx.x - row * tpr;
  const int c0 = ct * T;
  const long base = (long)row * NP * p.inner + c0;
  const float2* __restrict__ gin = p.in;
  float2* __restrict__ gout = p.out;
  const float2* __restrict__ tws = p.tw_sub;
  const float2* __restrict__ twt = p.tw_tile;
  const float2* __restrict__ twc = p.tw_col;

  const int k1o = tid / T, to = tid - k1o * T;
  const bool act2 = tid < R1 * T;
  float2 wt[R2], wc[R2];
  const bool full = p.tw_full != nullptr;
  if (act2) {
    if (full) {
      const float2* __restrict__ twf = p.tw_full + c0 + to;
      static_for<R2>([&](auto k2) { constexpr int K2 = decltype(k2)::value; wt[K2] = twf[(k1o + R1 * K2) * p.inner]; });
    } else {
      static_for<R2>([&](auto k2) {
        constexpr int K2 = decltype(k2)::value;
        const int k = k1o + R1 * K2;
        wt[K2] = twt[ct * NP + k];
        wc[K2] = twc[k * T + to];
      });
    }
  }
  const int gstep = R2 * T + p.padk;
  if (tid < R2 * T) {
    const int j = tid / T, t = tid - j * T;
    float2 v[R1], w1[R1];
    const int qstep = R2 * p.inner;
    if (p.in_len) {
      const int first = (int)((base + p.in_start + (long)j * p.inner + t) % p.in_len);
      const int len = (int)p.in_len;
      static_for<R1>([&](auto q) {
        constexpr int Q = decltype(q)::value;
        int idx = first + Q * qstep;
        if (idx >= len) idx -= len;
        v[Q] = gin[idx];
        if constexpr (Q > 0) w1[Q] = tws[j * R1 + Q];
      });
    } else {
      const float2* __restrict__ g0 = gin + base + (long)j * p.inner + t;
      static_for<R1>([&](auto q) {
        constexpr int Q = decltype(q)::value;
        v[Q] = g0[Q * qstep];
        if constexpr (Q > 0) w1[Q] = tws[j * R1 + Q];
      });
    }
    reg_dft<R1, -1>(v);
    const int l1 = j * T + t;
    static_for<R1>([&](auto k1) {
      constexpr int K1 = decltype(k1)::value;
      float2 x = v[K1];
      if constexpr (K1 > 0) x = cmul(x, w1[K1]);
      lds[l1 + K1 * gstep] = x;
    });
  }
  __syncthreads();
  if (act2) {
    float2 u[R2];
    const int l2 = k1o * gstep + to;
    static_for<R2>([&](auto j) {
      constexpr int J = decltype(j)::value;
      u[J] = lds[l2 + J * T];
    });
    reg_dft<R2, -1>(u);
    CHZ_OUT_DESC(odesc, gout);
    const int o0 = (int)base + k1o * p.inner + to;
    const int ostep = R1 * p.inner;
    static_for<R2>([&](auto k2) {
      constexpr int K2 = decltype(k2)::value;
      CHZ_STORE(odesc, gout, o0 + K2 * ostep, cmul(u[K2], full ? wt[K2] : cmul(wt[K2], wc[K2])));
    });
  }
}

__device__ __forceinline__ float2 rows_notch_apply(const RowsNotch& nf, int e, int addr_e, double alpha_e, float2 x, int at, bool stored) {
  if (at != addr_e || !stored) {
#if defined(__HIP_DEVICE_COMPILE__)
    if (nf.ver != nullptr) __hip_atomic_store(nf.ver + 1, 1u, __ATOMIC_RELAXED, __HIP_MEMORY_SCOPE_AGENT);
    if (nf.err != nullptr) __hip_atomic_store(nf.err, 0x80000000u | (unsigned)e, __ATOMIC_RELAXED, __HIP_MEMORY_SCOPE_SYSTEM);
#else
    if (nf.err != nullptr) *nf.err = 0x80000000u | (unsigned)e;
#endif
    return x;
  }
#if defined(__HIP_DEVICE_COMPILE__)
  if (nf.ver != nullptr) {
    if (__hip_atomic_load(nf.ver + 1, __ATOMIC_RELAXED, __HIP_MEMORY_SCOPE_AGENT) != 0u) return x;
    unsigned seq = nf.seq;
    if (nf.seq_base != nullptr) seq += __hip_atomic_load(nf.seq_base, __ATOMIC_RELAXED, __HIP_MEMORY_SCOPE_AGENT);
    unsigned v = 0;
    const long long t0 = wall_clock64();
    for (;;) {
      v = __hip_atomic_load(nf.ver, __ATOMIC_RELAXED, __HIP_MEMORY_SCOPE_AGENT);
      if (v == seq || wall_clock64() - t0 > nf.max_wait) break;
      __builtin_amdgcn_s_sleep(8);
    }
    __builtin_amdgcn_fence(__ATOMIC_ACQUIRE, "agent");
    if (v != seq) {
      __hip_atomic_store(nf.ver + 1, 1u, __ATOMIC_RELAXED, __HIP_MEMORY_SCOPE_AGENT);
      __hip_atomic_store(nf.err, seq + 1u, __ATOMIC_RELAXED, __HIP_MEMORY_SCOPE_SYSTEM);
      return x;
    }
  }
#endif
  for (int q = e; q >= 0; q = nf.next[q]) {
    double sr = nf.state[2 * q], si = nf.state[2 * q + 1];
    const double al = q == e ? alpha_e : nf.alpha[q];
    double dr = al * ((double)x.x - sr), di = al * ((double)x.y - si);
    CHZ_ROUNDED_F64(dr); CHZ_ROUNDED_F64(di);
    sr += dr; si += di;
    nf.state[2 * q] = sr; nf.state[2 * q + 1] = si;
    x = make_float2((float)((double)x.x - sr), (float)((double)x.y - si));
  }
#if defined(__HIP_DEVICE_COMPILE__)
  asm volatile("s_waitcnt vmcnt(0)" ::: "memory");
#endif
  return x;
}
__device__ __forceinline__ void rows_notch_publish(const RowsNotch& nf, int tid) {
#if defined(__HIP_DEVICE_COMPILE__)
  if (nf.ver == nullptr) return;
  __syncthreads();
  if (tid == 0) {
    bool last = true;
    if (nf.nwg > 1) {
      const unsigned c = __hip_atomic_fetch_add(nf.ver + 3, 1u, __ATOMIC_ACQ_REL, __HIP_MEMORY_SCOPE_AGENT) + 1u;
      last = c == (unsigned)nf.nwg;
      if (last) __hip_atomic_store(nf.ver + 3, 0u, __ATOMIC_RELAXED, __HIP_MEMORY_SCOPE_AGENT);
    }
    if (last && __hip_atomic_load(nf.ver + 1, __ATOMIC_RELAXED, __HIP_MEMORY_SCOPE_AGENT) == 0u) {
      unsigned seq = nf.seq;
      if (nf.seq_base != nullptr) seq += __hip_atomic_load(nf.seq_base, __ATOMIC_RELAXED, __HIP_MEMORY_SCOPE_AGENT);
      if (nf.adv != 0u) __hip_atomic_store(nf.seq_base, seq + 1u, __ATOMIC_RELAXED, __HIP_MEMORY_SCOPE_AGENT);
      __builtin_amdgcn_fence(__ATOMIC_RELEASE, "agent");
      asm volatile("s_waitcnt vmcnt(0)" ::: "memory");
      __hip_atomic_store(nf.ver, seq + 1u, __ATOMIC_RELAXED, __HIP_MEMORY_SCOPE_AGENT);
    }
  }
#else
  (void)nf; (void)tid;
#endif
}

template <int R1, int R2>
__global__ void fwd_rows(RowsParams p) {
  constexpr int NC = R1 * R2;
  HIP_DYNAMIC_SHARED(float2, lds)
  const int tid = threadIdx.x, nthr = blockDim.x;
  const int Ta = p.Ta, ld = p.ld, padg = p.padg;
  const int kb = blockIdx.x % p.Nb, at = blockIdx.x / p.Nb;
  const int a0 = at * Ta - p.ka_shift;
  const int rowstride = p.Nb * NC;
  const int gstep = R2 * ld + padg;

  const float2* __restrict__ tws = p.tw_sub;
  const float2* __restrict__ gin = p.buf + (long)kb * NC;
  bool nf_owner = false;
  static_for<CHZ_NOTCH_INLINE>([&](auto ee) { constexpr int E = decltype(ee)::value; nf_owner = nf_owner || (E < p.nf.n && p.nf.wg[E] == (int)blockIdx.x); });
  unsigned nf_mask = 0;
  float2 nf_x = make_float2(0.f, 0.f); int nf_at = -1; bool nf_ok = false;
  int nf_e = -1, nf_addr = -1; double nf_alpha = 0.0;
  if (nf_owner)
    for (int e = 0; e < p.nf.n; e++)
      if (p.nf.head[e] != 0 && p.nf.own[e].wg == (int)blockIdx.x && p.nf.own[e].tid == tid) {
        nf_mask |= 1u << p.nf.own[e].k2; nf_e = e; nf_addr = p.nf.addr[e]; nf_alpha = p.nf.alpha[e];
      }
  if constexpr (R2 % 16 == 0) {
    const int r1 = tid / R2, j1 = tid - r1 * R2;
    const bool act1 = tid < R2 * Ta;
    if (act1) {
      const int ka = a0 + r1;
      const bool in = ka >= 0 && ka < p.Ra;
      const float2* __restrict__ g = gin + (in ? ka : 0) * rowstride + j1;
      float2 v[R1], w1[R1];
      static_for<R1>([&](auto q) {
        constexpr int Q = decltype(q)::value;
        v[Q] = g[Q * R2];
        if constexpr (Q > 0) w1[Q] = tws[j1 * R1 + Q];
      });
      if (!in) static_for<R1>([&](auto q) { constexpr int Q = decltype(q)::value; v[Q] = make_float2(0.f, 0.f); });
      reg_dft<R1, -1>(v);
      const int b1 = j1 * ld + r1;
      static_for<R1>([&](auto k1) {
        constexpr int K1 = decltype(k1)::value;
        float2 x = v[K1];
        if constexpr (K1 > 0) x = cmul(x, w1[K1]);
        lds[b1 + K1 * gstep] = x;
      });
    }
  } else {
  const int j1 = tid / Ta, r1 = tid - j1 * Ta;
  const bool act1 = tid < R2 * Ta;
  float2 w1[R1];
  static_for<R1>([&](auto q) {
    constexpr int Q = decltype(q)::value;
    if constexpr (Q > 0) w1[Q] = tws[(act1 ? j1 : 0) * R1 + Q];
  });
  constexpr int LOAD_U = 6;
  for (int e0 = tid; e0 < Ta * NC; e0 += nthr * LOAD_U) {
    float2 x[LOAD_U];
    int la[LOAD_U];
    static_for<LOAD_U>([&](auto u) {
      constexpr int U = decltype(u)::value;
      const int e = e0 + U * nthr;
      const int r = e / NC, nc = e - r * NC;
      const int ka = a0 + r;
      la[U] = (e < Ta * NC) ? nc * ld + (nc / R2) * padg + r : -1;
      x[U] = make_float2(0.f, 0.f);
      if (la[U] >= 0 && ka >= 0 && ka < p.Ra) x[U] = gin[ka * rowstride + nc];
    });
    static_for<LOAD_U>([&](auto u) {
      constexpr int U = decltype(u)::value;
      if (la[U] >= 0) lds[la[U]] = x[U];
    });
  }
  __syncthreads();
  if (act1) {
    const int b1 = j1 * ld + r1;
    float2 v[R1];
    static_for<R1>([&](auto q) {
      constexpr int Q = decltype(q)::value;
      v[Q] = lds[b1 + Q * gstep];
    });
    reg_dft<R1, -1>(v);
    static_for<R1>([&](auto k1) {
      constexpr int K1 = decltype(k1)::value;
      float2 x = v[K1];
      if constexpr (K1 > 0) x = cmul(x, w1[K1]);
      lds[b1 + K1 * gstep] = x;
    });
  }
  }
  __syncthreads();
  if (tid < R1 * Ta) {
    const int k1 = tid / Ta, r = tid - k1 * Ta;
    const int ka = a0 + r;
    const int b2 = k1 * gstep + r;
    float2 u[R2];
    static_for<R2>([&](auto j) {
      constexpr int J = decltype(j)::value;
      u[J] = lds[b2 + J * ld];
    });
    reg_dft<R2, -1>(u);
    if (ka >= 0 && ka < p.Ra) {
      const bool selfconj = (ka == 0) || (2 * ka == p.Na);
      const int half = (int)(p.N >> 1);
      const int xrows = (int)(p.N / p.Na);
      const int x0 = kb + p.Nb * k1, xs = p.Nb * R1;
      const int kk0 = ka + p.Na * x0, kks = p.Na * xs;
      const int d0 = x0 * p.lay.pitch + p.lay.off + ka, ds = xs * p.lay.pitch;
      const int m0 = (xrows - 1 - x0) * p.lay.pitch + p.lay.off + (p.Na - ka);
      float2* __restrict__ sp = p.spec;
      CHZ_OUT_DESC(sdesc, sp);
      static_for<R2>([&](auto k2) {
        constexpr int K2 = decltype(k2)::value;
        const bool direct = !p.mirror || kk0 + K2 * kks <= half;
        const int at = direct ? d0 + K2 * ds : m0 - K2 * ds;
        float2 x = u[K2];
        if (!direct) x.y = -x.y;
        if (nf_mask >> K2 & 1u) { nf_x = x; nf_at = at; nf_ok = direct || !selfconj; }
        CHZ_STORE_IF(sdesc, sp, at, x, direct || !selfconj);
      });
      if (nf_mask != 0u) {
        const float2 y = rows_notch_apply(p.nf, nf_e, nf_addr, nf_alpha, nf_x, nf_at, nf_ok);
        CHZ_STORE_IF(sdesc, sp, nf_at, y, nf_ok);
      }
    }
  }
  if (nf_owner) rows_notch_publish(p.nf, tid);
}

struct NotchFixParams {
  float2* spec;
  const int* addr;
  const int* next;
  const int* head;
  const double* alpha;
  double* state;
  int n;
  int inl;
  unsigned* ver;
  unsigned seq;
  unsigned* seq_base;
  unsigned adv;
  unsigned* err;
  long long max_wait;
  int i_addr[CHZ_NOTCH_INLINE];
  signed char i_next[CHZ_NOTCH_INLINE], i_head[CHZ_NOTCH_INLINE];
  double i_alpha[CHZ_NOTCH_INLINE];
};
__global__ void __launch_bounds__(1024) notch_fix(NotchFixParams p) {
  const int i = (int)threadIdx.x;
  bool mine = false; int a = 0;
  if (i < p.n) {
    if (p.inl) { mine = p.i_head[i] != 0; a = p.i_addr[i]; }
    else { mine = p.head[i] != 0; a = p.addr[i]; }
  }
  float2 x = mine ? p.spec[a] : make_float2(0.f, 0.f);
  unsigned seq = p.seq; (void)seq;
#if defined(__HIP_DEVICE_COMPILE__)
  if (p.ver != nullptr) {
    if (__hip_atomic_load(p.ver + 1, __ATOMIC_RELAXED, __HIP_MEMORY_SCOPE_AGENT) != 0u) return;
    if (p.seq_base != nullptr) seq += __hip_atomic_load(p.seq_base, __ATOMIC_RELAXED, __HIP_MEMORY_SCOPE_AGENT);
    unsigned v = 0;
    const long long t0 = wall_clock64();
    for (;;) {
      v = __hip_atomic_load(p.ver, __ATOMIC_RELAXED, __HIP_MEMORY_SCOPE_AGENT);
      if (v == seq || wall_clock64() - t0 > p.max_wait) break;
      __builtin_amdgcn_s_sleep(8);
    }
    __builtin_amdgcn_fence(__ATOMIC_ACQUIRE, "agent");
    if (v != seq) {
      if (i == 0) {
        __hip_atomic_store(p.ver + 1, 1u, __ATOMIC_RELAXED, __HIP_MEMORY_SCOPE_AGENT);
        __hip_atomic_store(p.err, seq + 1u, __ATOMIC_RELAXED, __HIP_MEMORY_SCOPE_SYSTEM);
      }
      return;
    }
  }
#endif
  if (mine) {
    for (int e = i; e >= 0; e = p.inl ? (int)p.i_next[e] : p.next[e]) {
      double sr = p.state[2 * e], si = p.state[2 * e + 1];
      const double al = p.inl ? p.i_alpha[e] : p.alpha[e];
      double dr = al * ((double)x.x - sr), di = al * ((double)x.y - si);
      CHZ_ROUNDED_F64(dr); CHZ_ROUNDED_F64(di);
      sr += dr; si += di;
      p.state[2 * e] = sr; p.state[2 * e + 1] = si;
      x = make_float2((float)((double)x.x - sr), (float)((double)x.y - si));
    }
    p.spec[a] = x;
  }
#if defined(__HIP_DEVICE_COMPILE__)
  if (p.ver != nullptr) {
    __syncthreads();
    if (i == 0) {
      if (p.adv != 0u) __hip_atomic_store(p.seq_base, seq + 1u, __ATOMIC_RELAXED, __HIP_MEMORY_SCOPE_AGENT);
      __builtin_amdgcn_fence(__ATOMIC_RELEASE, "agent");
      asm volatile("s_waitcnt vmcnt(0)" ::: "memory");
      __hip_atomic_store(p.ver, seq + 1u, __ATOMIC_RELAXED, __HIP_MEMORY_SCOPE_AGENT);
    }
  }
#endif
}

template <int R1, int R2, int EPI>
__global__ void __launch_bounds__(256, (R1 <= 15 && R2 <= 20) ? (EPI == 0 ? 6 : (EPI == 1 ? 5 : 1)) : 1) chan_ifft(ChanParams p) {
  constexpr int P = R1 * R2;
  constexpr int LPC = R1 > R2 ? R1 : R2;
  constexpr int CPW = 64 / LPC;
  constexpr int LDC = R2 + 1;
  static_assert(CPW >= 1, "radix too wide for one wavefront");
  HIP_DYNAMIC_SHARED(float2, lds)
  const int tid = threadIdx.x;
  const int wave = tid >> 6, lane = tid & 63;
  const int wpb = blockDim.x >> 6;
  const int cw = lane / LPC, jl = lane - cw * LPC;
  const int lc = (blockIdx.x * wpb + wave) * CPW + cw;
  const int ch = p.ch0 + lc;
  const bool live = (cw < CPW) && (lc < p.nch);
  float2* my = lds + ((wave * CPW + (cw < CPW ? cw : 0)) * (R1 * LDC));
  const float2* __restrict__ tws = p.tw_sub;

  float2 v[R1];
  const bool act1 = live && jl < R2;
  if (act1) {
    const ChanDesc d = p.desc[ch];
    const float2* __restrict__ H = p.resp + (long)d.row * P;
    const float2* __restrict__ X = p.spec;
    float2 h[R1];
    bool ok[R1];
    int srcs[EPI == 2 ? R1 : 1];
    CHZ_IN_DESC(xdesc, X);
    const int dm = d.dir >> 31;
    const float2* __restrict__ Hl = H + jl;
    static_for<R1>([&](auto q) {
      constexpr int Q = decltype(q)::value;
      constexpr int H2 = (P + 1) / 2;
      const int i = jl + Q * R2;
      int t = i - H2; if (t < 0) t += P;
      const int u = t - d.t0;
      ok[Q] = ((unsigned)u < (unsigned)d.cnt) && (i != H2);
      int src = d.src0 + ((u ^ dm) - dm);
      if (d.wrap && src >= d.wrap) src -= d.wrap;
      if (!ok[Q]) src = 0;
      v[Q] = CHZ_LOAD2(xdesc, X, spec_index(p.lay.off, p.magic, p.dpitch, src));
      h[Q] = CHZ_LOAD_RESP(Hl + Q * R2);
      if constexpr (EPI == 2) srcs[Q] = src;
    });
    bool beamed = false;
    if constexpr (EPI == 2) {
      if (p.beam != nullptr) {
        const BeamDesc bd = p.beam[ch];
        if (bd.on && d.wrap > 0) {
          beamed = true;
          float2 w[R1];
          static_for<R1>([&](auto q) {
            constexpr int Q = decltype(q)::value;
            int mp = srcs[Q] == 0 ? 0 : d.wrap - srcs[Q];
            int row = (int)((float)mp * p.inv_na), col = mp - row * p.lay.na;
            if (col < 0) { row--; col += p.lay.na; } else if (col >= p.lay.na) { row++; col -= p.lay.na; }
            w[Q] = X[(long)row * p.lay.pitch + p.lay.off + col];
          });
          static_for<R1>([&](auto q) {
            constexpr int Q = decltype(q)::value;
            const double xr = v[Q].x, xi = v[Q].y, hr = h[Q].x, hi = h[Q].y;
            double sr, si;
            if (srcs[Q] == 0 || srcs[Q] == d.wrap / 2) {
              const double t1r = xr * bd.ar, t1i = xr * bd.ai, t2r = xi * bd.br, t2i = xi * bd.bi;
              sr = (t1r * hr - t1i * hi) + (t2r * hr - t2i * hi);
              si = (t1r * hi + t1i * hr) + (t2r * hi + t2i * hr);
            } else {
              const double yr = w[Q].x, yi = -(double)w[Q].y;
              const double cr = (bd.ar * xr - bd.ai * xi) + (bd.br * yr - bd.bi * yi);
              const double ci = (bd.ar * xi + bd.ai * xr) + (bd.br * yi + bd.bi * yr);
              sr = cr * hr - ci * hi; si = cr * hi + ci * hr;
            }
            v[Q] = ok[Q] ? make_float2((float)sr, (float)si) : make_float2(0.f, 0.f);
          });
        }
      }
    }
    if (!beamed) {
      static_for<R1>([&](auto q) {
        constexpr int Q = decltype(q)::value;
        float2 x = v[Q];
        if (d.conj) x.y = -x.y;
        x = cmul(x, h[Q]);
        v[Q] = ok[Q] ? x : make_float2(0.f, 0.f);
      });
    }
  }
  if constexpr (EPI == 2) {
    if (p.isb != nullptr) {
      const bool mine = act1 && p.isb[ch] != 0;
      const int src_lane = (cw < CPW ? cw : 0) * LPC + (jl == 0 || jl >= R2 ? 0 : R2 - jl);
      float2 part2[R1];
      static_for<R1>([&](auto q) {
        constexpr int Q = decltype(q)::value;
        const float2 mine_v = act1 ? v[R1 - 1 - Q] : make_float2(0.f, 0.f);
        part2[Q] = make_float2(__shfl(mine_v.x, src_lane), __shfl(mine_v.y, src_lane));
      });
      if (mine) {
        float2 orig[R1];
        static_for<R1>([&](auto q) { constexpr int Q = decltype(q)::value; orig[Q] = v[Q]; });
        static_for<R1>([&](auto q) {
          constexpr int Q = decltype(q)::value;
          const int i = jl + Q * R2;
          float2 partner = part2[Q];
          if (jl == 0) { if constexpr (Q >= 1) partner = orig[R1 - Q]; else partner = make_float2(0.f, 0.f); }
          if (i == 0) v[Q] = make_float2(0.f, 0.f);
          else if (2 * i < P) v[Q] = make_float2(orig[Q].x + partner.x, orig[Q].y - partner.y);
          else if (2 * i > P) v[Q] = make_float2(orig[Q].x - partner.x, orig[Q].y + partner.y);
          if (i == (P + 1) / 2) v[Q] = make_float2(0.f, 0.f);
        });
      }
    }
  }
  if (act1) {
    reg_dft<R1, +1>(v);
    static_for<R1>([&](auto k1) {
      constexpr int K1 = decltype(k1)::value;
      float2 x = v[K1];
      if constexpr (K1 > 0) x = cmul(x, tws[jl * R1 + K1]);
      my[K1 * LDC + jl] = x;
    });
  }
  __syncthreads();
  double part = 0.0;
  float2 u[R2];
  if (live && jl < R1) {
    static_for<R2>([&](auto j) {
      constexpr int J = decltype(j)::value;
      u[J] = my[jl * LDC + J];
    });
  }
  CHZ_WAVE_SYNC();
  if (live && jl < R1) {
    reg_dft<R2, +1>(u);
    const int drop = P - p.olen;
    if (EPI && p.fine != nullptr) {
      const FineDesc f = p.fine[ch];
      if (f.on) {
        const double kb = (double)(p.job - f.job0);
        const int m0 = jl - drop;
        const double g0 = kb * (double)p.olen + (double)m0;
        const int V = p.fine_V;
        int kbm = p.fine_jobm - f.job0m + (p.job < f.job0 ? p.fine_wrapm : 0);
        kbm += kbm < 0 ? V : 0; kbm -= kbm >= V ? V : 0;
        const double x = (double)(kbm + 1) * (double)f.adj_num;
        double r = fma(-floor(x * p.fine_invV), (double)V, x);
        r += r < 0.0 ? (double)V : 0.0; r -= r >= (double)V ? (double)V : 0.0;
        const double base = f.phase0 + r * p.fine_invV;
        if (f.rate == 0.0) {
          double hi = g0 * f.freq, lo = fma(g0, f.freq, -hi);
          hi -= rint(hi);
          double s0, c0, s1, c1;
          sincospi(2.0 * (base + hi + lo), &s0, &c0);
          c1 = f.step_c; s1 = f.step_s;
          static_for<R2>([&](auto k2) {
            constexpr int K2 = decltype(k2)::value;
            const double xr = u[K2].x, xi = u[K2].y;
            u[K2] = make_float2((float)(xr * c0 - xi * s0), (float)(xr * s0 + xi * c0));
            const double nc = c0 * c1 - s0 * s1; s0 = c0 * s1 + s0 * c1; c0 = nc;
          });
        } else {
          static_for<R2>([&](auto k2) {
            constexpr int K2 = decltype(k2)::value;
            const double g = g0 + (double)(R1 * K2);
            double hi = g * f.freq, lo = fma(g, f.freq, -hi);
            hi -= rint(hi);
            double q = 0.5 * f.rate * g * (g + 1.0);
            q -= rint(q);
            double sn, cs;
            sincospi(2.0 * (base + hi + lo + q), &sn, &cs);
            const double xr = u[K2].x, xi = u[K2].y;
            u[K2] = make_float2((float)(xr * cs - xi * sn), (float)(xr * sn + xi * cs));
          });
        }
      }
    }
    if (p.stage) {
      static_for<R2>([&](auto k2) {
        constexpr int K2 = decltype(k2)::value;
        const int n = jl + R1 * K2;
        if (n >= drop) my[n - drop] = u[K2];
      });
    } else {
      float2* __restrict__ o = p.out + (long)ch * p.olen;
      static_for<R2>([&](auto k2) {
        constexpr int K2 = decltype(k2)::value;
        const int n = jl + R1 * K2;
        if (n >= drop) o[n - drop] = u[K2];
      });
    }
    if constexpr (EPI) {
      static_for<R2>([&](auto k2) {
        constexpr int K2 = decltype(k2)::value;
        if (jl + R1 * K2 >= drop) part += (double)(u[K2].x * u[K2].x + u[K2].y * u[K2].y);
      });
    }
  }
  CHZ_WAVE_SYNC();
  if constexpr (EPI) {
    if (p.stage && p.agc_peak != nullptr) {
      const int sps = p.agc_sps, N = p.olen;
      double peak = 0.0;
      if (live) {
        for (int s0 = jl; (s0 + 1) * sps < N; s0 += LPC) {
          double energy = 0.0;
          for (int n = s0 * sps; n < (s0 + 1) * sps; n++) {
            const float2 w = my[n];
            float a = w.x * w.x, b = w.y * w.y;
            CHZ_ROUNDED_F32(a); CHZ_ROUNDED_F32(b);
            energy += (double)(a + b);
          }
          if (energy > peak) peak = energy;
        }
      }
      double tot = peak;
#pragma unroll
      for (int d = 32; d >= 1; d >>= 1) if (d < LPC) { const double o = __shfl_down(tot, (unsigned)d); if (jl + d < LPC && o > tot) tot = o; }
      if (live && jl == 0) p.agc_peak[ch] = tot;
    }
  }
  if (p.stage) {
    const int first_lc = (blockIdx.x * wpb + wave) * CPW;
    int nl = p.nch - first_lc; if (nl > CPW) nl = CPW;
    const int tot2 = nl > 0 ? (nl * p.olen) >> 1 : 0;
    const float2* wl = lds + (wave * CPW) * (R1 * LDC);
    float4* __restrict__ og = reinterpret_cast<float4*>(p.out + (long)(p.ch0 + first_lc) * p.olen);
    (void)tot2;
    const int half = p.olen >> 1;
    for (int c = 0; c < nl; c++) {
      const float2* wc = wl + c * (R1 * LDC);
      float4* __restrict__ oc = og + (long)c * half;
      for (int e = lane; e < half; e += 64) {
        const float2 a = wc[2 * e], b = wc[2 * e + 1];
        CHZ_STORE_OUT4(oc + e, make_float4(a.x, a.y, b.x, b.y));
      }
    }
  }
  if (EPI && p.power != nullptr) {
    double tot = part;
#pragma unroll
    for (int d = 32; d >= 1; d >>= 1) if (d < LPC) { const double o = __shfl_down(tot, (unsigned)d); if (jl + d < LPC) tot += o; }
    if (live && jl == 0) p.power[ch] = tot / (double)p.olen;
  }
}

template <int R1, int R2>
__global__ void __launch_bounds__(256) chan_c2r(ChanParams p) {
  constexpr int P = R1 * R2;
  constexpr int LPC = R1 > R2 ? R1 : R2;
  constexpr int CPW = 64 / LPC;
  constexpr int LDC = R2 + 1;
  static_assert(CPW >= 1, "radix too wide for one wavefront");
  static_assert(P % 2 == 0, "real-output channels need an even P");
  HIP_DYNAMIC_SHARED(float2, lds)
  const int tid = threadIdx.x;
  const int wave = tid >> 6, lane = tid & 63;
  const int wpb = blockDim.x >> 6;
  const int cw = lane / LPC, jl = lane - cw * LPC;
  const int lc = (blockIdx.x * wpb + wave) * CPW + cw;
  const int ch = p.ch0 + lc;
  const bool live = (cw < CPW) && (lc < p.nch);
  float2* my = lds + ((wave * CPW + (cw < CPW ? cw : 0)) * (R1 * LDC));
  const float2* __restrict__ tws = p.tw_sub;

  if (live && jl < R2) {
    const ChanDesc d = p.desc[ch];
    const int shift = d.shift;
    const float2* __restrict__ H = p.resp + (long)d.row * P;
    const float2* __restrict__ X = p.spec;
    constexpr int SB = P / 2 + 1;
    float2 v[R1], w[R1], h[R1];
    bool ok[R1];
    static_for<R1>([&](auto q) {
      constexpr int Q = decltype(q)::value;
      const int i = jl + Q * R2;
      const int k = i <= P / 2 ? i : P - i;
      const int mi = k + shift;
      int a, b = 0;
      if (p.m_real) {
        ok[Q] = mi >= 0 && mi < p.m_bins;
        a = ok[Q] ? mi : 0;
      } else {
        ok[Q] = mi >= -(p.m_bins / 2) && mi < p.m_bins / 2;
        a = mi % p.m_bins; if (a < 0) a += p.m_bins;
        b = (p.m_bins - mi) % p.m_bins; if (b < 0) b += p.m_bins;
        if (!ok[Q]) { a = 0; b = 0; }
      }
      if (k == (SB + 1) / 2) ok[Q] = false;
      int row = (int)((float)a * p.inv_na), col = a - row * p.lay.na;
      if (col < 0) { row--; col += p.lay.na; } else if (col >= p.lay.na) { row++; col -= p.lay.na; }
      v[Q] = X[(long)row * p.lay.pitch + p.lay.off + col];
      if (!p.m_real) {
        int rowb = (int)((float)b * p.inv_na), colb = b - rowb * p.lay.na;
        if (colb < 0) { rowb--; colb += p.lay.na; } else if (colb >= p.lay.na) { rowb++; colb -= p.lay.na; }
        w[Q] = X[(long)rowb * p.lay.pitch + p.lay.off + colb];
      }
      h[Q] = H[k];
    });
    static_for<R1>([&](auto q) {
      constexpr int Q = decltype(q)::value;
      const int i = jl + Q * R2;
      const int k = i <= P / 2 ? i : P - i;
      float2 x = v[Q];
      if (!p.m_real) x = make_float2(x.x + w[Q].x, x.y - w[Q].y);
      x = cmul(x, h[Q]);
      if (k == 0 || 2 * k == P) x.y = 0.f;
      if (i > P / 2) x.y = -x.y;
      v[Q] = ok[Q] ? x : make_float2(0.f, 0.f);
    });
    reg_dft<R1, +1>(v);
    static_for<R1>([&](auto k1) {
      constexpr int K1 = decltype(k1)::value;
      float2 x = v[K1];
      if constexpr (K1 > 0) x = cmul(x, tws[jl * R1 + K1]);
      my[K1 * LDC + jl] = x;
    });
  }
  __syncthreads();
  if (live && jl < R1) {
    float2 u[R2];
    static_for<R2>([&](auto j) {
      constexpr int J = decltype(j)::value;
      u[J] = my[jl * LDC + J];
    });
    reg_dft<R2, +1>(u);
    const int drop = P - p.olen;
    float* __restrict__ o = reinterpret_cast<float*>(p.out) + (long)ch * p.olen;
    static_for<R2>([&](auto k2) {
      constexpr int K2 = decltype(k2)::value;
      const int n = jl + R1 * K2;
      if (n >= drop) o[n - drop] = u[K2].x;
    });
  }
}

struct BluePreParams {
  const float* ring; long ring_len, start; int per; const float2* chirp; float2* za; int N; long Mz;
  const short* ring16; float scale16; int derand, new_from;
  unsigned long long* energy_part; unsigned* clip_part;
};
__global__ void __launch_bounds__(256) blue_pre(BluePreParams p) {
  const long stride = (long)gridDim.x * blockDim.x;
  unsigned long long energy = 0; unsigned clips = 0;
  for (long i = (long)blockIdx.x * blockDim.x + threadIdx.x; i < p.Mz; i += stride) {
    float2 v = make_float2(0.f, 0.f);
    if (i < p.N) {
      long idx = p.start + i * p.per;
      if (idx >= p.ring_len) idx -= p.ring_len;
      float2 x;
      if (p.ring16 != nullptr) {
        int a = (int)p.ring16[idx];
        if (p.derand) { a ^= -(a & 1) & 0xfffe; a = (int)(short)a; }
        float fa = (float)a * p.scale16;
        CHZ_ROUNDED_F32(fa);
        x = make_float2(fa, 0.f);
        if (i >= p.new_from) { energy += (unsigned)(a * a); clips += (a > 32766 || a < -32766); }
      } else x = p.per == 1 ? make_float2(p.ring[idx], 0.f) : make_float2(p.ring[idx], p.ring[idx + 1]);
      v = cmul(x, p.chirp[i]);
    }
    p.za[i] = v;
  }
  if (p.energy_part != nullptr) {
#pragma unroll
    for (int d = 32; d >= 1; d >>= 1) { energy += __shfl_xor(energy, d); clips += __shfl_xor(clips, d); }
    if ((threadIdx.x & 63) == 0) {
      const int w = (int)blockIdx.x * ((int)blockDim.x >> 6) + ((int)threadIdx.x >> 6);
      p.energy_part[w] = energy; p.clip_part[w] = clips;
    }
  }
}
struct BlueMulParams { const float2* zs; const float2* bf; float2* za; SpecLayout lay; long Mz; };
__global__ void __launch_bounds__(256) blue_mul(BlueMulParams p) {
  const long stride = (long)gridDim.x * blockDim.x;
  for (long k = (long)blockIdx.x * blockDim.x + threadIdx.x; k < p.Mz; k += stride) {
    const long a = spec_addr(p.lay, k);
    const float2 t = cmul(p.zs[a], p.bf[a]);
    p.za[k] = make_float2(t.x, -t.y);
  }
}
struct BluePostParams { const float2* zs; const float2* chirp; float2* spec; SpecLayout zlay, lay; int bins; float inv; };
__global__ void __launch_bounds__(256) blue_post(BluePostParams p) {
  const long stride = (long)gridDim.x * blockDim.x;
  for (long k = (long)blockIdx.x * blockDim.x + threadIdx.x; k < p.bins; k += stride) {
    const float2 y = p.zs[spec_addr(p.zlay, k)];
    p.spec[spec_addr(p.lay, k)] = cmul(make_float2(y.x * p.inv, -y.y * p.inv), p.chirp[k]);
  }
}

__device__ __forceinline__ float cnrm_unfused(float2 x) {
  float a = x.x * x.x;
  float b = x.y * x.y;
  CHZ_ROUNDED_F32(a); CHZ_ROUNDED_F32(b);
  return a + b;
}

struct NoiseParams {
// ... 2288 lines not shown
```

ka9q-radio_amd/csrc/chz_launch.h:

```cpp
#pragma once
#include <cstring>
#include <cmath>
#include <cmath>
#include "chz_kernels.h"
#include "chz_plan.h"

namespace chz {

#ifndef CHZ_EXIT_SCOPE
#define CHZ_EXIT_SCOPE(name) struct { bool ok; } name = {true}
#endif
#define CHZ_LAUNCH(kern, grid, block, lds, s, ev0, ev1, p)                                              \
  do {                                                                                                  \
    CHZ_EXIT_SCOPE(_xs);                                                                                \
    if (!_xs.ok) break;                                                                                 \
    if ((ev0) || (ev1)) hipExtLaunchKernelGGL(kern, dim3(grid), dim3(block), (unsigned)(lds), s, (ev0), (ev1), 0, p); \
    else hipLaunchKernelGGL(kern, dim3(grid), dim3(block), lds, s, p);                                \
  } while (0)

inline int launch_first_real(Radix2 r, dim3 grid, int block, size_t lds, hipStream_t s, const FirstRealParams& p, hipEvent_t e0 = nullptr, hipEvent_t e1 = nullptr) {
#define X(a, b) if (r.r1 == a && r.r2 == b) { CHZ_LAUNCH((fwd_first_real<a, b>), grid, block, lds, s, e0, e1, p); return 0; }
  CHZ_FWD_MENU(X)
#undef X
  return -1;
}
inline int launch_cols(Radix2 r, dim3 grid, int block, size_t lds, hipStream_t s, const ColsParams& p, hipEvent_t e0 = nullptr, hipEvent_t e1 = nullptr) {
#define X(a, b) if (r.r1 == a && r.r2 == b) { CHZ_LAUNCH((fwd_cols<a, b>), grid, block, lds, s, e0, e1, p); return 0; }
  CHZ_FWD_MENU(X)
#undef X
  return -1;
}
inline int launch_rows(Radix2 r, dim3 grid, int block, size_t lds, hipStream_t s, const RowsParams& p, hipEvent_t e0 = nullptr, hipEvent_t e1 = nullptr) {
#define X(a, b) if (r.r1 == a && r.r2 == b) { CHZ_LAUNCH((fwd_rows<a, b>), grid, block, lds, s, e0, e1, p); return 0; }
  CHZ_FWD_MENU(X)
#undef X
  return -1;
}
inline bool chan_layout(ChanParams& c, const SpecLayout& lay, long bins) {
  c.lay = lay; c.inv_na = 1.0f / (float)lay.na;
  c.dpitch = lay.pitch - lay.na;
  const unsigned long long m = ((1ull << 32) + (unsigned long long)lay.na - 1) / (unsigned long long)lay.na;
  c.magic = (unsigned)(m > 0xffffffffull ? 0xffffffffull : m);
  if (c.dpitch == 0) return true;
  if (c.dpitch < 0 || c.dpitch >= (1 << 24) || bins >= (1 << 24)) return false;
  const unsigned long long e = m * (unsigned long long)lay.na - (1ull << 32);
  return e * (unsigned long long)(bins > 0 ? bins - 1 : 0) < (1ull << 32);
}
inline int launch_chan(Radix2 r, int grid, int block, size_t lds, hipStream_t s, const ChanParams& p, hipEvent_t e0 = nullptr, hipEvent_t e1 = nullptr) {
#define X(a, b) if (r.r1 == a && r.r2 == b) { \
    if (p.isb || p.beam) { CHZ_LAUNCH((chan_ifft<a, b, 2>), grid, block, lds, s, e0, e1, p); } \
    else if (p.fine || p.power) { CHZ_LAUNCH((chan_ifft<a, b, 1>), grid, block, lds, s, e0, e1, p); } \
    else { CHZ_LAUNCH((chan_ifft<a, b, 0>), grid, block, lds, s, e0, e1, p); } \
    return 0; }
  CHZ_CHAN_MENU(X)
#undef X
  return -1;
}
inline int launch_chan_real(Radix2 r, int grid, int block, size_t lds, hipStream_t s, const ChanParams& p, hipEvent_t e0 = nullptr, hipEvent_t e1 = nullptr) {
#define X(a, b) if (r.r1 == a && r.r2 == b) { if constexpr ((a * b) % 2 == 0) { CHZ_LAUNCH((chan_c2r<a, b>), grid, block, lds, s, e0, e1, p); return 0; } }
  CHZ_CHAN_MENU(X)
#undef X
  return -1;
}
inline int big_lds_prepare(const void* kern) {
#if defined(__HIPCC__) && !defined(HIPEMU)
  return hipFuncSetAttribute(kern, hipFuncAttributeMaxDynamicSharedMemorySize, 160 * 1024) == hipSuccess ? 0 : -1;
#else
  (void)kern; return 0;
#endif
}
inline int fwd_lds_prepare(const FwdPlan& p, bool first_real) {
  if (p.lds1 > CHZ_FWD_LDS_MAX || p.lds2 > CHZ_FWD_LDS_MAX || p.lds3 > CHZ_FWD_LDS_MAX) return -1;
  int rc = 0;
#define X(a, b) \
  if (p.lds1 > CHZ_FWD_LDS_DEFAULT && p.ra.r1 == a && p.ra.r2 == b) \
    rc |= first_real ? big_lds_prepare(reinterpret_cast<const void*>(fwd_first_real<a, b>)) : big_lds_prepare(reinterpret_cast<const void*>(fwd_cols<a, b>)); \
  if (p.Nb > 1 && p.lds2 > CHZ_FWD_LDS_DEFAULT && p.rb.r1 == a && p.rb.r2 == b) rc |= big_lds_prepare(reinterpret_cast<const void*>(fwd_cols<a, b>)); \
  if (p.lds3 > CHZ_FWD_LDS_DEFAULT && p.rc.r1 == a && p.rc.r2 == b) rc |= big_lds_prepare(reinterpret_cast<const void*>(fwd_rows<a, b>));
  CHZ_FWD_MENU(X)
#undef X
  return rc ? -1 : 0;
}
inline int chan_any_prepare() {
#if defined(__HIPCC__) && !defined(HIPEMU)
  static int done = -1;
  if (done < 0) done = hipFuncSetAttribute(reinterpret_cast<const void*>(chan_any<false>), hipFuncAttributeMaxDynamicSharedMemorySize, 160 * 1024) == hipSuccess ? 1 : 0;
  return done == 1 ? 0 : -1;
#else
  return 0;
#endif
}
inline int launch_chan_any(const ChanGeom& g, int nch, hipStream_t s, const ChanParams& p, const float2* tw, bool real_out, float2* scratch = nullptr,
                           hipEvent_t e0 = nullptr, hipEvent_t e1 = nullptr) {
  if (nch <= 0) return 0;
  if (g.big && !scratch) return -1;
  AnyParams q{};
  q.c = p; q.real_out = real_out ? 1 : 0; q.scratch = scratch;
  q.P = g.P;
  q.m.N = g.lb; q.m.olen = p.olen; q.m.nstages = g.nstages; q.m.tw = tw;
  for (int i = 0; i < g.nstages; i++) q.m.radix[i] = g.radix[i];
  if (g.big) { CHZ_LAUNCH(chan_any<true>, nch, g.any_threads, 0, s, e0, e1, q); }
  else { CHZ_LAUNCH(chan_any<false>, nch, g.any_threads, g.lds, s, e0, e1, q); }
  return 0;
}
inline int welch_prepare() {
#if defined(__HIPCC__) && !defined(HIPEMU)
  static int done = -1;
  if (done < 0) done = hipFuncSetAttribute(reinterpret_cast<const void*>(welch_seg<false>), hipFuncAttributeMaxDynamicSharedMemorySize, 160 * 1024) == hipSuccess ? 1 : 0;
  return done == 1 ? 0 : -1;
#else
  return 0;
#endif
}
inline int launch_welch(const ChanGeom& g, WelchParams q, const float2* tw, int scratch_wgs, hipStream_t s, hipEvent_t e0 = nullptr, hipEvent_t e1 = nullptr) {
  if (q.nslots <= 0) return 0;
  if (q.segs > 0) {
    q.m.N = g.lb; q.m.olen = 0; q.m.nstages = g.nstages; q.m.tw = tw;
    for (int i = 0; i < g.nstages; i++) q.m.radix[i] = g.radix[i];
    const long items = (long)q.nslots * q.segs;
    if (g.big) {
      if (!q.scratch || scratch_wgs < 1) return -1;
      const int grid = (int)(items < scratch_wgs ? items : scratch_wgs);
      CHZ_LAUNCH(welch_seg<true>, grid, g.any_threads, 0, s, e0, nullptr, q);
    } else {
      const int grid = (int)(items < 65536 ? items : 65536);
      CHZ_LAUNCH(welch_seg<false>, grid, g.any_threads, g.lds, s, e0, nullptr, q);
    }
  }
  CHZ_LAUNCH(welch_sum, q.nslots, 256, 8 * sizeof(double), s, (q.segs > 0 ? (hipEvent_t) nullptr : e0), e1, q);
  return 0;
}
inline void launch_bb_append(BbAppendParams q, int n, hipStream_t s) {
  if (n <= 0) return;
  CHZ_LAUNCH(bb_ring_append, n, q.olen >= 256 ? 256 : 64, 0, s, (hipEvent_t) nullptr, (hipEvent_t) nullptr, q);
}
inline int launch_notch_fix(hipStream_t s, const NotchFixParams& p, hipEvent_t e0 = nullptr, hipEvent_t e1 = nullptr) {
  if (p.n <= 0) return 0;
  if (p.n > 1024) return -1;
  CHZ_LAUNCH(notch_fix, 1, (p.n + 63) / 64 * 64, 0, s, e0, e1, p);
  return 0;
}
struct NotchTables {
  std::vector<int> addr, next, head;
  void fill_inline(NotchFixParams& q, const double* alpha) const {
    const int n = (int)addr.size();
    q.inl = n <= CHZ_NOTCH_INLINE;
    if (!q.inl) return;
    for (int i = 0; i < n; i++) { q.i_addr[i] = addr[(size_t)i]; q.i_next[i] = (signed char)next[(size_t)i]; q.i_head[i] = (signed char)head[(size_t)i]; q.i_alpha[i] = alpha[i]; }
  }
};
inline NotchTables notch_tables(const int* bins, int n, const SpecLayout& lay) {
  NotchTables t;
  t.addr.resize((size_t)n); t.next.assign((size_t)n, -1); t.head.assign((size_t)n, 1);
  for (int i = 0; i < n; i++) {
    t.addr[(size_t)i] = (int)spec_addr(lay, bins[i]);
    for (int j = i - 1; j >= 0; j--)
      if (bins[j] == bins[i]) { t.next[(size_t)j] = i; t.head[(size_t)i] = 0; break; }
  }
  return t;
}
inline bool notch_owner(const FwdPlan& p, bool real, int bin, int* wg, int* tid, int* k2) {
  const int R1 = p.rc.r1, R2 = p.rc.r2;
  const long xrows = (long)p.Nb * p.Nc;
  long ka = bin % p.Na, x = bin / p.Na;
  if (real && ka >= p.Ra) { ka = p.Na - ka; x = xrows - 1 - x; }
  if (ka < 0 || ka >= p.Ra || x < 0 || x >= xrows) return false;
  const long kb = x % p.Nb, kc = x / p.Nb;
  const long k1 = kc % R1, K2 = kc / R1;
  if (K2 >= R2) return false;
  const long at = (ka + p.ka_shift) / p.Ta, r = (ka + p.ka_shift) % p.Ta;
  *wg = (int)(at * p.Nb + kb); *tid = (int)(k1 * p.Ta + r); *k2 = (int)K2;
  return *wg < p.grid3 && *tid < p.block3;
}
inline bool rows_notch_fill(RowsNotch& nf, std::vector<NotchOwn>& own, const FwdPlan& p, bool real, const int* bins, int n) {
  nf = RowsNotch{}; own.clear();
  if (n < 1 || n > CHZ_NOTCH_INLINE) return false;
  for (int i = 0; i < n; i++) {
    int wg = 0, tid = 0, k2 = 0;
    if (!notch_owner(p, real, bins[i], &wg, &tid, &k2) || k2 > 31) { nf = RowsNotch{}; own.clear(); return false; }
    for (int j = 0; j < i; j++) if (bins[j] != bins[i] && own[(size_t)j].wg == wg && own[(size_t)j].tid == tid) { nf = RowsNotch{}; own.clear(); return false; }
    nf.wg[i] = wg;
    own.push_back(NotchOwn{wg, tid, k2, 0});
    bool seen = false;
    for (int j = 0; j < i; j++) seen = seen || nf.wg[j] == wg;
    if (!seen) nf.nwg++;
  }
  nf.n = n;
  return true;
}
inline int launch_demod(hipStream_t s, const DemodParams& p_in, hipEvent_t e0 = nullptr, hipEvent_t e1 = nullptr) {
  if (p_in.nch <= 0) return 0;
  DemodParams p = p_in;
  p.fm_alpha = -std::expm1(-p.blocktime / 1.0);
  const size_t lds = 16 * (size_t)p.olen;
  if (lds > 160 * 1024) return -1;
  if (lds > 64 * 1024) {
    static int big = -1;
    if (big < 0) big = big_lds_prepare(reinterpret_cast<const void*>(demod_linear_tail)) == 0 ? 1 : 0;
    if (big != 1) return -1;
  }
  const bool lanes = p.mix != nullptr;
  const bool lin = lanes && p.lin_pll, fpll = lanes && p.fm_pll, ftone = lanes && p.fm_tone;
  const bool linl = p.lin_lanes != 0, fml = lanes && p.fm_lanes != 0, wave = p.wave_any != 0 || !(linl || fml);
  if ((fpll || ftone) && 8 * (size_t)p.olen > 64 * 1024) {
    static int big2 = -1;
    if (big2 < 0) big2 = (big_lds_prepare(reinterpret_cast<const void*>(fm_front_k)) == 0 && big_lds_prepare(reinterpret_cast<const void*>(fm_finish)) == 0) ? 1 : 0;
    if (big2 != 1) return -1;
// ... 71 lines not shown
```

ka9q-radio_amd/csrc/chz_plan.h:

```cpp
#pragma once
#include <cmath>
#include <cstdio>
#include <cstdlib>
#include <cstring>
#include <string>
#include <vector>
#include <complex>

namespace chz {

#define CHZ_FWD_MENU(X) \
  X(4, 4) X(5, 5) X(6, 6) X(5, 9) X(5, 10) X(5, 15) X(8, 8) X(8, 9) X(9, 9) X(10, 10) X(10, 12) X(5, 25) X(9, 15) \
  X(12, 12) X(10, 15) X(8, 19) X(10, 16) X(12, 15) X(12, 16) X(15, 15) X(15, 16) X(16, 16) X(16, 20) X(20, 20) X(9, 16) \
  X(10, 20) X(10, 13)
#define CHZ_CHAN_MENU(X) \
  X(4, 5) X(5, 6) X(10, 15) X(10, 16) X(10, 20) X(15, 20) X(16, 20) X(20, 20) X(20, 24) \
  X(24, 25) X(25, 32) X(30, 32) X(30, 40) X(40, 48)

struct Radix2 { int r1, r2; };

inline bool fwd_menu_lookup(int np, Radix2* out) {
#define X(a, b) if ((a) * (b) == np) { if (out) { out->r1 = a; out->r2 = b; } return true; }
  CHZ_FWD_MENU(X)
#undef X
  return false;
}
inline bool fwd_menu_lookup_c(int np, Radix2* out) {
#define X(a, b) if ((a) * (b) == np && (b) % 16 == 0) { if (out) { out->r1 = a; out->r2 = b; } return true; }
  CHZ_FWD_MENU(X)
#undef X
  return fwd_menu_lookup(np, out);
}
inline bool chan_menu_lookup(int p, Radix2* out) {
#define X(a, b) if ((a) * (b) == p) { if (out) { out->r1 = a; out->r2 = b; } return true; }
  CHZ_CHAN_MENU(X)
#undef X
  return false;
}

struct f2 { float x, y; };

inline f2 root_of_unity(long long num, long long den, int sign, double scale_re = 1.0, double scale_im = 0.0) {
  num %= den; if (num < 0) num += den;
  long long k8 = 8 * num, oct = k8 / den, rem = k8 - oct * den;
  double a = (M_PI / 4.0) * ((double)rem / (double)den), c, s;
  if (oct & 1) { a = M_PI / 4.0 - a; s = std::cos(a); c = std::sin(a); }
  else { c = std::cos(a); s = std::sin(a); }
  double cc, ss;
  switch (oct >> 1) {
    case 0: cc = c; ss = s; break;
    case 1: cc = -s; ss = c; break;
    case 2: cc = -c; ss = -s; break;
    default: cc = s; ss = -c; break;
  }
  ss *= sign;
  double re = cc * scale_re - ss * scale_im, im = cc * scale_im + ss * scale_re;
  return f2{(float)re, (float)im};
}

inline int round_up(int x, int m) { return (x + m - 1) / m * m; }

inline std::vector<f2> make_tw_sub(int r1, int r2, int sign) {
  std::vector<f2> t((size_t)r1 * r2);
  for (int j = 0; j < r2; j++)
    for (int k1 = 0; k1 < r1; k1++) t[(size_t)j * r1 + k1] = root_of_unity((long long)j * k1, (long long)r1 * r2, sign);
  return t;
}

enum { CHZ_IN_COMPLEX = 1, CHZ_IN_REAL = 2 };
#define CHZ_FWD_LDS_DEFAULT (64 * 1024)
#define CHZ_FWD_LDS_MAX (160 * 1024)

struct FwdPlan {
  int N = 0, in_type = 0, bins = 0;
  int Na = 0, Nb = 1, Nc = 0;
  Radix2 ra{}, rb{}, rc{};
  int Ra = 0;
  int inner = 0;
  int T1 = 0, T2 = 0, Ta = 0;
  int padk1 = 0, padk2 = 0, ld3 = 0, padg3 = 0;
  int spec_pitch = 0, spec_off = 0, ka_shift = 0;
  long spec_elems = 0;
  int grid1 = 0, block1 = 0, grid2 = 0, block2 = 0, grid3 = 0, block3 = 0;
  size_t lds1 = 0, lds2 = 0, lds3 = 0;
  std::vector<f2> tw_sub_a, tw_sub_b, tw_sub_c, tw1_tile, tw1_col, tw2_tile, tw2_col, tw2_full;
  std::string desc;
};

inline int padk_for(int r2, int T) { int v = (T - r2 * T) % 32; if (v < 0) v += 32; return v; }

inline int pick_tile(int n, int want, int lo, int hi, int lanes_per_col, int max_threads) {
  int best = 0; double bestscore = 1e30;
  for (int t = 1; t <= n && t <= hi; t++) {
    if (n % t) continue;
    if (t * lanes_per_col > max_threads) continue;
    double score = std::fabs(std::log((double)t / want)) + (t < lo ? 1.0 : 0.0) - (t % 16 == 0 ? 0.75 : 0.0);
    if (score < bestscore) { bestscore = score; best = t; }
  }
  return best;
}

inline bool fwd_plan_geometry(FwdPlan& p, int T1_over, int T2_over, int Ta_over) {
  const bool real = p.in_type == CHZ_IN_REAL;
  p.inner = p.Nb * p.Nc;
  p.Ra = real ? p.Na / 2 + 1 : p.Na;
  p.bins = real ? p.N / 2 + 1 : p.N;
  const int la = p.ra.r1 > p.ra.r2 ? p.ra.r1 : p.ra.r2;
  if (real) {
    if (p.inner & 1) return false;
    const int cols_p = p.inner / 2;
    p.T1 = T1_over > 0 ? T1_over : pick_tile(cols_p, 16, 8, 64, la, 1024);
    if (p.T1 <= 0 || cols_p % p.T1) return false;
    p.grid1 = cols_p / p.T1;
  } else {
    p.T1 = T1_over > 0 ? T1_over : pick_tile(p.inner, 16, 8, 64, la, 1024);
    if (p.T1 <= 0 || p.inner % p.T1) return false;
    p.grid1 = p.inner / p.T1;
  }
  p.padk1 = padk_for(p.ra.r2, p.T1);
  p.block1 = round_up(la * p.T1, 64);
  p.lds1 = sizeof(f2) * ((size_t)p.Na * p.T1 + (size_t)p.ra.r1 * p.padk1);
  if (real) p.lds1 += sizeof(f2) * (size_t)p.Na * p.T1;
  if (p.Nb > 1) {
    const int lb = p.rb.r1 > p.rb.r2 ? p.rb.r1 : p.rb.r2;
    p.T2 = T2_over > 0 ? T2_over : pick_tile(p.Nc, 16, 8, 64, lb, 1024);
    if (p.T2 <= 0 || p.Nc % p.T2) return false;
    p.grid2 = p.Ra * (p.Nc / p.T2);
    p.block2 = round_up(lb * p.T2, 64);
    p.padk2 = padk_for(p.rb.r2, p.T2);
    p.lds2 = sizeof(f2) * ((size_t)p.Nb * p.T2 + (size_t)p.rb.r1 * p.padk2);
  }
  const int lc = p.rc.r1 > p.rc.r2 ? p.rc.r1 : p.rc.r2;
  p.Ta = Ta_over > 0 ? Ta_over : 16;
  if (p.Ta > p.Ra) p.Ta = p.Ra;
  while (lc * p.Ta > 1024) p.Ta--;
  p.spec_pitch = p.Na; p.spec_off = 0; p.ka_shift = 0;
  if (real && (p.Na & 1) && p.Ta == 16 && p.Nc % 16 == 0) {
    int s2 = ((15 - p.Na) % 16 + 16) % 16;
    p.spec_off = s2 / 2;
    p.ka_shift = p.spec_off;
    p.spec_pitch = round_up(p.spec_off + p.Na, 16);
  }
  {
    const long xrows = real ? ((long)p.N / 2) / p.Na + 1 : (long)p.N / p.Na;
    p.spec_elems = xrows * p.spec_pitch + 16;
  }
  p.ld3 = p.Ta + 1 + (p.Ta & 1);
  if (!(p.ld3 & 1)) p.ld3++;
  p.padg3 = (16 - (p.rc.r2 * p.ld3) % 32 + 32) % 32;
  p.grid3 = p.Nb * ((p.Ra + p.ka_shift + p.Ta - 1) / p.Ta);
  p.block3 = round_up(lc * p.Ta, 64);
  p.lds3 = sizeof(f2) * ((size_t)p.Nc * p.ld3 + (size_t)p.rc.r1 * p.padg3 + 8);
  if (p.lds1 > CHZ_FWD_LDS_MAX || p.lds2 > CHZ_FWD_LDS_MAX || p.lds3 > CHZ_FWD_LDS_MAX) return false;
  if (p.block1 > 1024 || p.block2 > 1024 || p.block3 > 1024) return false;
  char b[256];
  snprintf(b, sizeof b, "N=%d %s axes %dx%dx%d radices (%d,%d)(%d,%d)(%d,%d) tiles T1=%d T2=%d Ta=%d grids %d/%d/%d blocks %d/%d/%d spec pitch %d off %d",
           p.N, real ? "real" : "complex", p.Na, p.Nb, p.Nc, p.ra.r1, p.ra.r2, p.rb.r1, p.rb.r2, p.rc.r1, p.rc.r2,
           p.T1, p.T2, p.Ta, p.grid1, p.grid2, p.grid3, p.block1, p.block2, p.block3, p.spec_pitch, p.spec_off);
  p.desc = b;
  return true;
}
inline void fwd_plan_tables(FwdPlan& p) {
  const bool real = p.in_type == CHZ_IN_REAL;
  if (real) {
    p.tw1_tile.resize((size_t)p.grid1 * p.Ra);
    for (int tile = 0; tile < p.grid1; tile++)
      for (int k = 0; k < p.Ra; k++)
        p.tw1_tile[(size_t)tile * p.Ra + k] = root_of_unity((long long)k * 2 * tile * p.T1, p.N, -1);
    p.tw1_col.resize((size_t)p.Ra * 2 * p.T1);
    for (int k = 0; k < p.Ra; k++)
      for (int cc = 0; cc < 2 * p.T1; cc++)
        p.tw1_col[(size_t)k * 2 * p.T1 + cc] =
            (cc & 1) ? root_of_unity((long long)k * cc, p.N, -1, 0.0, -0.5) : root_of_unity((long long)k * cc, p.N, -1, 0.5, 0.0);
  } else {
    p.tw1_tile.resize((size_t)p.grid1 * p.Na);
    for (int tile = 0; tile < p.grid1; tile++)
      for (int k = 0; k < p.Na; k++)
        p.tw1_tile[(size_t)tile * p.Na + k] = root_of_unity((long long)k * tile * p.T1, p.N, -1);
    p.tw1_col.resize((size_t)p.Na * p.T1);
    for (int k = 0; k < p.Na; k++)
      for (int t = 0; t < p.T1; t++) p.tw1_col[(size_t)k * p.T1 + t] = root_of_unity((long long)k * t, p.N, -1);
  }
  p.tw_sub_a = make_tw_sub(p.ra.r1, p.ra.r2, -1);
  if (p.Nb > 1) {
// ... 245 lines not shown
```

ka9q-radio_amd/engine.py:

```python
import ctypes as C
import os

import numpy as np

HERE = os.path.dirname(os.path.abspath(__file__))
LIB_PATH = os.environ.get("CHZ_LIB") or os.path.join(HERE, "libchz_hip.so")

COMPLEX, REAL = 1, 2
ND = 4

_vp, _i, _u, _d, _l = C.c_void_p, C.c_int, C.c_uint, C.c_double, C.c_long


class ChzInfo(C.Structure):
    _fields_ = [("L", _i), ("M", _i), ("N", _i), ("in_type", _i), ("bins", _i), ("ring_blocks", _i),
                ("Na", _i), ("Nb", _i), ("Nc", _i), ("n_banks", _i), ("lanes", _i), ("spec_elems", _l),
                ("spec_na", _i), ("spec_pitch", _i), ("spec_off", _i), ("plan", C.c_char * 320)]


class ChzTiming(C.Structure):
    _fields_ = [("total_ms", _d), ("blocks", _i),
                ("first_ms", _d), ("cols_ms", _d), ("rows_ms", _d), ("notch_ms", _d), ("chan_ms", _d),
                ("first_n", _i), ("cols_n", _i), ("rows_n", _i), ("notch_n", _i), ("chan_n", _i), ("enqueue_ms", _d),
                ("fix_ms", _d), ("fix_n", _i), ("demod_ms", _d), ("demod_n", _i)]


class DemodParams(C.Structure):
    _fields_ = [("channels", _i), ("env", _i), ("agc", _i), ("encoding", _i), ("snr_squelch", _i), ("squelch_tail", _i),
                ("tuned", _i), ("kind", _i),
                ("samprate", _d), ("headroom", _d), ("threshold", _d), ("recovery_rate", _d), ("hangtime", _d), ("dc_alpha", _d),
                ("bandwidth", _d), ("shift", _d), ("squelch_open", _d), ("squelch_close", _d), ("gain", _d),
                ("deemph_rate", _d), ("deemph_gain", _d), ("threshold_extend", _d),
                ("pll_enable", _i), ("pll_square", _i), ("pll_loop_bw", _d), ("tone_freq", _d)]


class DemodStatus(C.Structure):
    _fields_ = [("frame", _i), ("mute", _i), ("squelch_state", _i), ("pll_lock", _i),
                ("output_power", _d), ("gain", _d), ("n0", _d), ("snr", _d), ("foffset", _d), ("pdeviation", _d),
                ("pll_snr", _d), ("pll_cphase", _d), ("tone_deviation", _d), ("pll_rotations", _i), ("tone_mute", _i)]


PCM_S16BE, PCM_S16LE, PCM_F32LE, PCM_F32BE, PCM_MULAW, PCM_ALAW, PCM_F16LE, PCM_F16BE = 0, 1, 2, 3, 4, 5, 6, 7


SYMBOLS = [
    "chz_last_error", "chz_process_exiting", "chz_device_count", "chz_engine_create", "chz_engine_destroy", "chz_engine_info",
    "chz_engine_set_stream", "chz_sync", "chz_input_write", "chz_input_write_device", "chz_input_ring",
    "chz_forward", "chz_slot_stream", "chz_set_notches", "chz_spectrum_read", "chz_spectrum_device", "chz_spectrum_attach",
    "chz_bank_create", "chz_bank_create_shared", "chz_bank_set_rows", "chz_bank_set_row_responses", "chz_bank_set_responses", "chz_bank_set_shifts", "chz_bank_set_active",
    "chz_bank_execute", "chz_bank_execute_range", "chz_bank_destroy", "chz_bank_read", "chz_bank_read_async",
    "chz_spectrum_read_async", "chz_host_callback", "chz_host_alloc", "chz_host_free", "chz_host_register", "chz_host_unregister",
    "chz_bank_output_device", "chz_bank_write_block", "chz_bank_demod", "chz_bank_demod_auto", "chz_bank_read_pcm_flags_async", "chz_bank_pcm_wait", "chz_step", "chz_run_blocks", "chz_gather_descriptor",
    "chz_bank_set_tuning", "chz_bank_read_power", "chz_bank_read_power_async",
    "chz_input_write_i16", "chz_input_write_i16_device", "chz_input_stats",
    "chz_bank_enable_noise", "chz_bank_read_noise", "chz_bank_read_noise_async", "chz_bank_create_real", "chz_bank_set_isb", "chz_bank_set_beam",
    "chz_set_notches_alpha", "chz_slot_sync", "chz_engine_check", "chz_input_seek", "chz_input_mark", "chz_input_mark_wait", "chz_engine_notch_order",
    "chz_bank_set_demod", "chz_bank_pcm_stride", "chz_bank_set_pcm_stride", "chz_bank_read_pcm", "chz_bank_read_pcm_async",
    "chz_comm_unique_id", "chz_comm_create", "chz_comm_create_file", "chz_comm_destroy", "chz_comm_rank", "chz_comm_world",
    "chz_mini_create", "chz_mini_destroy", "chz_mini_capacity", "chz_mini_add", "chz_mini_release", "chz_mini_set_response", "chz_mini_execute",
    "chz_rmini_create", "chz_rmini_destroy", "chz_rmini_check", "chz_rmini_capacity", "chz_rmini_add", "chz_rmini_release", "chz_rmini_set_response", "chz_rmini_execute",
    "chz_comm_barrier", "chz_comm_allreduce_max", "chz_spectrum_broadcast", "chz_spectrum_exchange_rows", "chz_run_blocks_sharded",
    "chz_comm_create_local", "chz_spectrum_broadcast_local", "chz_set_option",
    "chz_welch_create", "chz_welch_destroy", "chz_welch_set_window", "chz_welch_configure", "chz_welch_poll", "chz_welch_read", "chz_welch_read_async",
    "chz_bank_welch_create", "chz_bank_welch_attach", "chz_bank_welch_detach", "chz_bank_welch_configure", "chz_bank_welch_poll", "chz_bank_welch_steps",
]

ENV_OPTIONS = {"CHZ_CHAN_STAGE": "chan_stage", "CHZ_NOISE_ENERGY": "noise_energy", "CHZ_DEMOD_WAVE": "demod_wave", "CHZ_ENQ_THREADS": "enq_threads",
               "CHZ_GRAPH_BLOCKS": "graph_blocks", "CHZ_NOTCH_FOLD": "notch_fold", "CHZ_NOISE_HINT": "noise_hint", "CHZ_PLL_LANE0": "pll_lane0",
               "CHZ_NOTCH_WAIT_MS": "notch_wait_ms", "CHZ_FAULT_TICKET_SKEW": "fault_ticket_skew", "CHZ_ALLOW_FAULT_INJECTION": "allow_fault_injection",
               "CHZ_LAUNCH_ID": "launch_id"}


def apply_env_options():
    L = lib()
    for env, opt in ENV_OPTIONS.items():
        v = os.environ.get(env)
        _check(L.chz_set_option(opt.encode(), v.encode() if v is not None else None))

_lib = None


def lib():
    global _lib
    if _lib is None:
        if not os.path.exists(LIB_PATH):
            raise RuntimeError("libchz_hip.so is missing: build it with `make -C ka9q-radio_amd/csrc` "
                               "(there is no CPU fallback)")
        L = C.CDLL(LIB_PATH)
        if hasattr(L, "chz_emulated_build") and os.environ.get("CHZ_ALLOW_EMULATED_ENGINE") != "1":
            raise RuntimeError("%s is a CPU-emulated TEST build of the engine: refusing to use it as the product "
                               "(there is no CPU fallback)" % LIB_PATH)
        L.chz_last_error.restype = C.c_char_p
        L.chz_set_option.argtypes = [C.c_char_p, C.c_char_p]
        L.chz_device_count.restype = _i
        L.chz_engine_create.argtypes = [C.POINTER(_vp), _i, _i, _i, _i, C.c_char_p, _i]
        L.chz_engine_destroy.argtypes = [_vp]; L.chz_engine_destroy.restype = None
        L.chz_engine_info.argtypes = [_vp, C.POINTER(ChzInfo)]
        L.chz_engine_set_stream.argtypes = [_vp, _vp]
        L.chz_sync.argtypes = [_vp]
        L.chz_input_write.argtypes = [_vp, _vp, _l]
        L.chz_input_write_device.argtypes = [_vp, _vp, _l]
        L.chz_input_ring.argtypes = [_vp, C.POINTER(_vp), C.POINTER(_l)]
        L.chz_input_write_i16.argtypes = [_vp, _vp, _l, C.c_float, _i]
        L.chz_input_write_i16_device.argtypes = [_vp, _vp, _l, C.c_float, _i]
        L.chz_input_stats.argtypes = [_vp, _i, C.POINTER(C.c_ulonglong), C.POINTER(C.c_uint)]
        L.chz_forward.argtypes = [_vp, _u]
        L.chz_set_notches.argtypes = [_vp, _vp, _i, _d]
        L.chz_set_notches_alpha.argtypes = [_vp, _vp, _vp, _i]
        L.chz_slot_sync.argtypes = [_vp, _i]
        L.chz_engine_check.argtypes = [_vp]
        L.chz_bank_set_demod.argtypes = [_vp, _i, _u, _i, _i, _vp, _d]
        L.chz_bank_pcm_stride.argtypes = [_vp, _i]
        L.chz_bank_set_pcm_stride.argtypes = [_vp, _i, _i]
        L.chz_bank_read_pcm.argtypes = [_vp, _i, _i, _i, _i, _vp, _vp]
        L.chz_bank_read_pcm_async.argtypes = [_vp, _i, _i, _i, _i, _vp, _vp]
        L.chz_mini_create.argtypes = [C.POINTER(_vp), _i, _i, _i, _i]
        L.chz_mini_destroy.argtypes = [_vp]; L.chz_mini_destroy.restype = None
        L.chz_mini_capacity.argtypes = [_vp]
        L.chz_mini_add.argtypes = [_vp]
        L.chz_mini_release.argtypes = [_vp, _i]
        L.chz_mini_set_response.argtypes = [_vp, _i, _vp]
        L.chz_mini_execute.argtypes = [_vp, _i, _vp, _vp, _vp, _vp, _vp]
        L.chz_rmini_create.argtypes = [C.POINTER(_vp), _i, _i, _i, _vp, _vp, _i, _i]
        L.chz_rmini_destroy.argtypes = [_vp]; L.chz_rmini_destroy.restype = None
        L.chz_rmini_check.argtypes = [_i, _i, _i, _vp, _vp]
        L.chz_rmini_capacity.argtypes = [_vp]
        L.chz_rmini_add.argtypes = [_vp]
        L.chz_rmini_release.argtypes = [_vp, _i]
        L.chz_rmini_set_response.argtypes = [_vp, _i, _i, _vp]
        L.chz_rmini_execute.argtypes = [_vp, _i, _vp, _vp, _vp, _vp, _vp, _vp]
        L.chz_comm_unique_id.argtypes = [_vp]
        L.chz_comm_create.argtypes = [C.POINTER(_vp), _i, _i, _vp, _i]
        L.chz_comm_create_file.argtypes = [C.POINTER(_vp), _i, _i, C.c_char_p, _i, _d]
        L.chz_comm_destroy.argtypes = [_vp]; L.chz_comm_destroy.restype = None
        L.chz_comm_rank.argtypes = [_vp]
        L.chz_comm_world.argtypes = [_vp]
        L.chz_comm_barrier.argtypes = [_vp]
        L.chz_comm_allreduce_max.argtypes = [_vp, _vp, _i]
        L.chz_spectrum_broadcast.argtypes = [_vp, _vp, _i, _i]
        L.chz_spectrum_exchange_rows.argtypes = [_vp, _vp, _i, _i, _vp, _vp]
        L.chz_run_blocks_sharded.argtypes = [_vp, _vp, _i, _i, _vp, _vp, _u, _i, C.POINTER(ChzTiming)]
        L.chz_spectrum_read.argtypes = [_vp, _i, _vp]
        L.chz_spectrum_device.argtypes = [_vp, _i, C.POINTER(_vp)]
        L.chz_slot_stream.argtypes = [_vp, _i, C.POINTER(_vp)]
        L.chz_spectrum_attach.argtypes = [_vp, _i, _vp]
        L.chz_bank_create.argtypes = [_vp, _i, _i, _i]
        L.chz_bank_create_real.argtypes = [_vp, _i, _i, _i]
        L.chz_bank_set_isb.argtypes = [_vp, _i, _i, _i, _vp]
        L.chz_bank_set_beam.argtypes = [_vp, _i, _i, _i, _vp, _vp]
        L.chz_bank_set_responses.argtypes = [_vp, _i, _i, _i, _vp]
        L.chz_bank_set_shifts.argtypes = [_vp, _i, _i, _i, _vp]
        L.chz_bank_set_active.argtypes = [_vp, _i, _i]
        L.chz_bank_execute.argtypes = [_vp, _i, _u]
        L.chz_bank_read.argtypes = [_vp, _i, _i, _i, _vp]
        L.chz_bank_execute_range.argtypes = [_vp, _i, _u, _i, _i]
        L.chz_bank_set_tuning.argtypes = [_vp, _i, _u, _i, _i, _vp, _vp, _vp]
        L.chz_bank_read_power.argtypes = [_vp, _i, _i, _i, _i, _vp]
        L.chz_bank_read_power_async.argtypes = [_vp, _i, _i, _i, _i, _vp]
        L.chz_bank_enable_noise.argtypes = [_vp, _i, _d]
        L.chz_bank_read_noise.argtypes = [_vp, _i, _i, _i, _i, _vp]
        L.chz_bank_read_noise_async.argtypes = [_vp, _i, _i, _i, _i, _vp]
        L.chz_bank_destroy.argtypes = [_vp, _i]
        L.chz_bank_read_async.argtypes = [_vp, _i, _i, _i, _i, _vp]
        L.chz_bank_output_device.argtypes = [_vp, _i, _i, C.POINTER(_vp)]
        L.chz_step.argtypes = [_vp, _u]
        L.chz_run_blocks.argtypes = [_vp, _u, _i, _i, _i, C.POINTER(ChzTiming)]
        L.chz_gather_descriptor.argtypes = [_i, _i, _i, _i, C.POINTER(_i * 6)]
        L.chz_welch_create.argtypes = [_vp, _i, _i, _i, _i]
        L.chz_welch_destroy.argtypes = [_vp, _i]
        L.chz_welch_set_window.argtypes = [_vp, _i, _i, _vp]
        L.chz_welch_configure.argtypes = [_vp, _i, _i, _i, _i, _i, _d]
        L.chz_welch_poll.argtypes = [_vp, _i, _i, _vp, C.c_longlong]
        L.chz_welch_read.argtypes = [_vp, _i, _i, _i, _vp, _vp]
        L.chz_welch_read_async.argtypes = [_vp, _i, _i, _i, _vp, _vp]
        L.chz_bank_welch_create.argtypes = [_vp, _i, _i, _i, _i, _i]
        L.chz_bank_welch_attach.argtypes = [_vp, _i, _i, _i, _u]
        L.chz_bank_welch_detach.argtypes = [_vp, _i, _i]
        L.chz_bank_welch_configure.argtypes = [_vp, _i, _i, _i, _i, _d]
        L.chz_bank_welch_poll.argtypes = [_vp, _i, _i, _vp, _u]
        L.chz_bank_welch_steps.argtypes = [_i, _i, _d, _u, _u, _i, C.c_longlong, C.POINTER(C.c_longlong * 3)]
        _lib = L
    return _lib


class ChzError(RuntimeError):
    pass


def _check(r):
    if r < 0:
        raise ChzError(lib().chz_last_error().decode())
    return r


def gather_descriptor(in_type, master_bins, P, shift):
    out = (_i * 6)()
    lib().chz_gather_descriptor(in_type, master_bins, P, int(shift), C.byref(out))
    return tuple(out)


class Engine:

    def __init__(self, L, M, in_type, device=0, plan="", ring_blocks=0):
        self._h = _vp()
        apply_env_options()
        _check(lib().chz_engine_create(C.byref(self._h), L, M, in_type, device,
                                       plan.encode() if plan else None, ring_blocks))
        info = ChzInfo()
        _check(lib().chz_engine_info(self._h, C.byref(info)))
        self.L, self.M, self.N, self.in_type, self.bins = info.L, info.M, info.N, info.in_type, info.bins
        self.ring_blocks = info.ring_blocks
        self.plan = info.plan.decode()
        self.axes = (info.Na, info.Nb, info.Nc)
        self.lanes = info.lanes
        self.spec_elems = info.spec_elems
        self.spec_layout = (info.spec_na, info.spec_pitch, info.spec_off)
        self.banks = []

    def close(self):
        if self._h:
            lib().chz_engine_destroy(self._h)
            self._h = _vp()

    def __del__(self):
        try:
            self.close()
        except Exception:
            pass

    def write(self, samples):
        dt = np.float32 if self.in_type == REAL else np.complex64
        samples = np.ascontiguousarray(samples, dt)
        _check(lib().chz_input_write(self._h, samples.ctypes.data, samples.shape[0]))
        _check(lib().chz_sync(self._h))

    def write_i16(self, samples, scale, randomize=False):
        s = np.ascontiguousarray(samples, np.int16).reshape(-1)
        _check(lib().chz_input_write_i16(self._h, s.ctypes.data, s.size, float(scale), 1 if randomize else 0))
        self.sync()

    def input_stats(self, slot):
        en, cl = C.c_ulonglong(0), C.c_uint(0)
        _check(lib().chz_input_stats(self._h, slot, C.byref(en), C.byref(cl)))
        return en.value, cl.value

    def write_device(self, dev_ptr, n):
        _check(lib().chz_input_write_device(self._h, dev_ptr, n))

    def ring(self):
        p, n = _vp(), _l()
        _check(lib().chz_input_ring(self._h, C.byref(p), C.byref(n)))
        return p.value, n.value

    def set_stream(self, hip_stream):
        _check(lib().chz_engine_set_stream(self._h, hip_stream))
        info = ChzInfo()
        _check(lib().chz_engine_info(self._h, C.byref(info)))
        self.lanes = info.lanes

    def forward(self, job):
        _check(lib().chz_forward(self._h, job & 0xFFFFFFFF))

    def set_notches(self, bins, alpha=0.01):
        bins = np.ascontiguousarray(bins, np.int32)
        if np.ndim(alpha) == 0:
            _check(lib().chz_set_notches(self._h, bins.ctypes.data if len(bins) else None, len(bins), float(alpha)))
        else:
            al = np.ascontiguousarray(alpha, np.float64).reshape(-1)
            assert al.shape[0] == bins.shape[0]
            _check(lib().chz_set_notches_alpha(self._h, bins.ctypes.data if len(bins) else None,
                                               al.ctypes.data if len(bins) else None, len(bins)))

    def check(self):
        _check(lib().chz_engine_check(self._h))

    def slot_sync(self, slot):
        _check(lib().chz_slot_sync(self._h, slot))

    def run_blocks_sharded(self, comm, job0, nblocks, root=0, rows=None, samples=False):
        t = ChzTiming()
        if samples:
            _check(lib().chz_run_blocks_sharded(self._h, comm._h, root, 2, None, None, job0 & 0xFFFFFFFF, nblocks, C.byref(t)))
        elif rows is None:
            _check(lib().chz_run_blocks_sharded(self._h, comm._h, root, 0, None, None, job0 & 0xFFFFFFFF, nblocks, C.byref(t)))
        else:
            lo = np.ascontiguousarray(rows[0], np.int32); hi = np.ascontiguousarray(rows[1], np.int32)
            _check(lib().chz_run_blocks_sharded(self._h, comm._h, root, 1, lo.ctypes.data, hi.ctypes.data,
                                                job0 & 0xFFFFFFFF, nblocks, C.byref(t)))
        return t

    def spectrum(self, slot):
        out = np.zeros(self.bins, np.complex64)
        _check(lib().chz_spectrum_read(self._h, slot, out.ctypes.data))
        return out

    def spectrum_ptr(self, slot):
        p = _vp()
        _check(lib().chz_spectrum_device(self._h, slot, C.byref(p)))
        return p.value

    def slot_stream(self, slot):
        p = _vp()
        _check(lib().chz_slot_stream(self._h, slot, C.byref(p)))
        return p.value or 0

    def attach_spectrum(self, slot, dev_ptr):
        _check(lib().chz_spectrum_attach(self._h, slot, dev_ptr))

    def bank(self, P, olen, capacity, real=False, shared_rows=0):
        b = Bank(self, P, olen, capacity, real, shared_rows)
        self.banks.append(b)
        return b

    def welch(self, fft_n, capacity, max_bins, max_avg, packed=None):
        if packed is not None:
            _check(lib().chz_set_option(b"welch_packed", b"1" if packed else b"0"))
        try:
            return Welch(self, fft_n, capacity, max_bins, max_avg)
        finally:
            if packed is not None:
                _check(lib().chz_set_option(b"welch_packed", None))

    def step(self, job):
        _check(lib().chz_step(self._h, job & 0xFFFFFFFF))

    def sync(self):
        _check(lib().chz_sync(self._h))

    def run_blocks(self, job0, nblocks, graph=False, instrument=False):
        t = ChzTiming()
        _check(lib().chz_run_blocks(self._h, job0 & 0xFFFFFFFF, nblocks, 1 if graph else 0,
                                    1 if instrument else 0, C.byref(t)))
        return t


class Bank:
    def __init__(self, eng, P, olen, capacity, real=False, shared_rows=0):
        self.eng, self.P, self.olen, self.capacity, self.real = eng, P, olen, capacity, bool(real)
        L = lib()
        if shared_rows:
            L.chz_bank_create_shared.argtypes = [_vp, _i, _i, _i, _i]
            L.chz_bank_set_rows.argtypes = [_vp, _i, _i, _i, _vp]
            L.chz_bank_set_row_responses.argtypes = [_vp, _i, _i, _i, _vp]
            self.id = _check(L.chz_bank_create_shared(eng._h, P, olen, capacity, shared_rows))
        else:
            make = L.chz_bank_create_real if real else L.chz_bank_create
            self.id = _check(make(eng._h, P, olen, capacity))
        self._dtype = np.float32 if real else np.complex64
        self.active = 0

    def destroy(self):
        if self.id is not None and self.eng._h:
            _check(lib().chz_bank_destroy(self.eng._h, self.id))
        self.id = None

    def set_rows(self, ch0, rows):
        r = np.ascontiguousarray(rows, np.int32)
        _check(lib().chz_bank_set_rows(self.eng._h, self.id, ch0, r.shape[0], r.ctypes.data))

    def set_row_responses(self, row0, resp):
        r = np.ascontiguousarray(resp, np.complex64)
        assert r.ndim == 2 and r.shape[1] == self.P
        _check(lib().chz_bank_set_row_responses(self.eng._h, self.id, row0, r.shape[0], r.ctypes.data))

    def set_responses(self, ch0, resp):
        resp = np.ascontiguousarray(resp, np.complex64).reshape(-1, self.P)
        _check(lib().chz_bank_set_responses(self.eng._h, self.id, ch0, resp.shape[0], resp.ctypes.data))

    def set_shifts(self, ch0, shifts):
        shifts = np.ascontiguousarray(shifts, np.int32).reshape(-1)
        _check(lib().chz_bank_set_shifts(self.eng._h, self.id, ch0, shifts.shape[0], shifts.ctypes.data))

    def set_isb(self, ch0, flags):
        f = np.ascontiguousarray(flags, np.uint8).reshape(-1)
        _check(lib().chz_bank_set_isb(self.eng._h, self.id, ch0, f.shape[0], f.ctypes.data))

    def set_beam(self, ch0, alpha, beta, on):
        alpha = np.asarray(alpha, np.complex128).reshape(-1); beta = np.asarray(beta, np.complex128).reshape(-1)
        ab = np.ascontiguousarray(np.stack([alpha.real, alpha.imag, beta.real, beta.imag], axis=1), np.float64)
        f = np.ascontiguousarray(on, np.uint8).reshape(-1)
        assert ab.shape[0] == f.shape[0]
        _check(lib().chz_bank_set_beam(self.eng._h, self.id, ch0, f.shape[0], ab.ctypes.data, f.ctypes.data))

    def set_active(self, n):
        _check(lib().chz_bank_set_active(self.eng._h, self.id, n))
        self.active = n

    def execute(self, job):
        _check(lib().chz_bank_execute(self.eng._h, self.id, job & 0xFFFFFFFF))

    def execute_range(self, job, ch0, n):
        _check(lib().chz_bank_execute_range(self.eng._h, self.id, job & 0xFFFFFFFF, ch0, n))

    def set_tuning(self, job, ch0, shifts, freq, rate=None):
        shifts = np.ascontiguousarray(shifts, np.int32).reshape(-1)
        freq = np.ascontiguousarray(freq, np.float64).reshape(-1)
        assert freq.shape == shifts.shape
        rp = None
        if rate is not None:
            rate = np.ascontiguousarray(rate, np.float64).reshape(-1)
            assert rate.shape == shifts.shape
            rp = rate.ctypes.data
        _check(lib().chz_bank_set_tuning(self.eng._h, self.id, job & 0xFFFFFFFF, ch0, shifts.shape[0],
                                         shifts.ctypes.data, freq.ctypes.data, rp))

    def set_demod(self, job, ch0, params, blocktime=0.02):
        arr = (DemodParams * len(params))(*params)
        _check(lib().chz_bank_set_demod(self.eng._h, self.id, job & 0xFFFFFFFF, ch0, len(params), arr, float(blocktime)))

    def set_pcm_stride(self, nbytes):
        _check(lib().chz_bank_set_pcm_stride(self.eng._h, self.id, int(nbytes)))

    def read_pcm(self, slot, ch0=0, n=None):
        if n is None:
            n = self.active - ch0
        stride = _check(lib().chz_bank_pcm_stride(self.eng._h, self.id))
        pcm = np.zeros((n, stride), np.uint8)
        st = (DemodStatus * n)()
        _check(lib().chz_bank_read_pcm(self.eng._h, self.id, slot, ch0, n, pcm.ctypes.data, st))
        return pcm, st

    def inject(self, slot, samples, bb_power=None, n0=None, ch0=0):
        x = np.ascontiguousarray(samples, np.complex64)
        pw = None if bb_power is None else np.ascontiguousarray(bb_power, np.float64)
        ne = None if n0 is None else np.ascontiguousarray(n0, np.float64)
        L = lib()
        L.chz_bank_write_block.argtypes = [_vp, _i, _i, _i, _i, _vp, _vp, _vp]
        _check(L.chz_bank_write_block(self.eng._h, self.id, slot, ch0, x.shape[0], x.ctypes.data,
# ... 279 lines not shown
```

Measured before the change: 882,200 channels.

## Fuse forward-rows FFT and a channel-bank IFFT into one launch with device-side handoff

Measured after the change: 310,900 channels. 64.8% lower.

```diff
diff --git a/include/chz_engine.h b/include/chz_engine.h
--- a/include/chz_engine.h
+++ b/include/chz_engine.h
@@ -55,6 +55,7 @@
 int chz_input_mark(chz_engine *e, int k);
 int chz_input_mark_wait(chz_engine *e, int k);
 int chz_engine_notch_order(chz_engine *e, int by_event);
+int chz_engine_rows_chan_fused(const chz_engine *e);
 
 int chz_forward(chz_engine *e, unsigned job);
 int chz_set_notches(chz_engine *e, const int *bins, int n, double alpha);
diff --git a/ka9q-radio_amd/csrc/chz_engine.hip b/ka9q-radio_amd/csrc/chz_engine.hip
--- a/ka9q-radio_amd/csrc/chz_engine.hip
+++ b/ka9q-radio_amd/csrc/chz_engine.hip
@@ -223,6 +223,11 @@
   NotchTables notch_tab; std::vector<double> notch_alpha_h;
   NotchOwn* notch_own = nullptr;
   RowsNotch notch_fold{};
+  int rows_chan_fuse = -1;
+  unsigned* rows_chan_cnt = nullptr;
+  unsigned rows_chan_base[CHZ_ND] = {0, 0, 0, 0};
+  long long dev_lds = 0, dev_waves = 0;
+  long long rows_chan_fused = 0;
   std::vector<Bank> banks;
   std::vector<WelchBank*> welch;
   hipStream_t welch_s = nullptr;
@@ -317,6 +322,7 @@
   int enq_threads = 2;
   int graph_blocks = 32;
   int notch_fold = 1;
+  int rows_chan_fuse = -1;
   int noise_hint = 1;
   int pll_lane0 = 0;
   double notch_wait_ms = 3000.0;
@@ -340,6 +346,7 @@
   else if (n == "enq_threads") g_opt.enq_threads = d ? def.enq_threads : ((iv == 2 || iv == 4) ? iv : 1);
   else if (n == "graph_blocks") g_opt.graph_blocks = (d || iv <= 0 || iv > 4096) ? def.graph_blocks : iv;
   else if (n == "notch_fold") g_opt.notch_fold = d ? def.notch_fold : (value[0] != '0');
+  else if (n == "rows_chan_fuse") g_opt.rows_chan_fuse = d ? def.rows_chan_fuse : (iv < 0 ? -1 : (iv != 0));
   else if (n == "noise_hint") g_opt.noise_hint = d ? def.noise_hint : (value[0] != '0');
   else if (n == "pll_lane0") g_opt.pll_lane0 = d ? def.pll_lane0 : 1;
   else if (n == "notch_wait_ms") g_opt.notch_wait_ms = (d || !(atof(value) > 0)) ? def.notch_wait_ms : atof(value);
@@ -460,10 +467,25 @@
     e->notch_max_wait = (long long)(ms * (double)khz);
   }
   e->graph_min_blocks = opt.graph_blocks;
+  e->rows_chan_fuse = opt.rows_chan_fuse;
+  {
+#ifndef HIPEMU
+    hipDeviceProp_t dp;
+    if (hipGetDeviceProperties(&dp, e->device) == hipSuccess && dp.multiProcessorCount > 0) {
+      e->dev_lds = (long long)dp.multiProcessorCount * (long long)dp.maxSharedMemoryPerMultiProcessor;
+      e->dev_waves = (long long)dp.multiProcessorCount * (dp.maxThreadsPerMultiProcessor / 64);
+    }
+#else
+    e->dev_lds = 256LL * 160 * 1024; e->dev_waves = 256LL * 32;
+#endif
+  }
   if (const char* no = getenv("CHZ_NOTCH_ORDER")) e->notch_order = strcmp(no, "event") == 0 ? 1 : (strcmp(no, "unordered-timing-only") == 0 ? 2 : 0);
   if (own_queues() == 2 && e->notch_order == 0) e->notch_order = 1;
   HIPOK(hipHostMalloc((void**)&e->notch_err, sizeof(unsigned), hipHostMallocMapped));
   *e->notch_err = 0;
+  HIPOK(hipMalloc((void**)&e->rows_chan_cnt, sizeof(unsigned) * 2 * CHZ_ND));
+  HIPOK(hipMemset(e->rows_chan_cnt, 0, sizeof(unsigned) * 2 * CHZ_ND));
+  if (opt.fault_ticket_skew && opt.allow_fault_injection) for (int i = 0; i < CHZ_ND; i++) e->rows_chan_base[i] = (unsigned)opt.fault_ticket_skew;
   for (int i = 0; i < e->nlanes; i++) {
     if (i == 0) e->lanes[i].s = e->stream;
     else HIPOK(stream_create_masked(&e->lanes[i].s, false));
@@ -539,6 +561,7 @@
   hipFree(e->tw_sub_a); hipFree(e->tw_sub_b); hipFree(e->tw_sub_c);
   hipFree(e->tw1_tile); hipFree(e->tw1_col); hipFree(e->tw2_tile); hipFree(e->tw2_col); hipFree(e->tw2_full);
   free_notches(e);
+  hipFree(e->rows_chan_cnt);
   if (e->notch_err) (void)hipHostFree(e->notch_err);
   if (e->upload) hipStreamDestroy(e->upload);
   if (e->tail) hipStreamDestroy(e->tail);
@@ -579,6 +602,9 @@
 
 static int check_device_errors(const chz_engine* e) {
   const unsigned v = e->notch_err ? __atomic_load_n(e->notch_err, __ATOMIC_ACQUIRE) : 0u;
+  if ((v & 0xc0000000u) == CHZ_ROWS_CHAN_ERR)
+    return fail(-8, "a channel bank in the tail of its block's fwd_rows launch waited for the spectrum in vain (target %u): that block's and every "
+                    "later block's outputs of the bank were NOT written; the engine must be re-created (option rows_chan_fuse=0 keeps the bank a launch of its own)", v & 0x3fffffffu);
   if (v) return fail(-8, "spur-notch ordering failed at ticket %u: a block's notch kernel waited for its predecessor in vain; "
                          "the engine must be re-created (CHZ_NOTCH_ORDER=event orders by HIP events instead)", v - 1u);
   return 0;
@@ -860,7 +886,53 @@
   return 0;
 }
 
-static int enqueue_forward(chz_engine* e, unsigned job, Instr* in, NotchTurn* turn = nullptr, int seq = 0, bool capture_first = false, bool capturing = false) {
+static inline float2* bank_out(const Bank& b, int slot);
+struct RowsChanGeom { int per_wg = 0, grid = 0, waves = 0; size_t lds = 0; };
+static inline RowsChanGeom rows_chan_geom(const chz_engine* e, const Bank& b) {
+  RowsChanGeom g;
+  g.per_wg = rows_chan_per_wg(e->plan, b.g); g.waves = e->plan.block3 / 64; g.lds = rows_chan_lds(e->plan, b.g);
+  g.grid = g.per_wg > 0 ? (b.active + g.per_wg - 1) / g.per_wg : 0;
+  return g;
+}
+static inline bool rows_chan_fits(const chz_engine* e, const RowsChanGeom& g) {
+  if (g.grid < 1 || g.lds > CHZ_FWD_LDS_DEFAULT || e->dev_lds <= 0 || e->dev_waves <= 0) return false;
+  const long long wgs = (long long)e->nlanes * g.grid;
+  return 4 * wgs * (long long)g.lds <= e->dev_lds && 4 * wgs * g.waves <= e->dev_waves;
+}
+static int rows_chan_pick(const chz_engine* e, bool eager) {
+  if (!eager || e->rows_chan_fuse == 0 || e->blue || !e->rows_chan_cnt) return -1;
+  if (e->n_notch > 0 && !(e->notch_fold.n > 0 && e->notch_order == 0)) return -1;
+  for (int i = 0; i < (int)e->banks.size(); i++) {
+    const Bank& b = e->banks[(size_t)i];
+    if (b.active <= 0 || !b.resp) continue;
+    if (b.g.any || b.out_real || b.fine || b.power || b.isb || b.beam || (b.n0 && b.noise_samprate > 0.0) || b.dm_on > 0 || b.bb_n > 0) continue;
+    if ((e->chan_stage >= 0 ? e->chan_stage : (b.active >= 16384)) != 0) continue;
+    if (!rows_chan_menu_has(e->plan.rc, b.g.r)) continue;
+    return rows_chan_fits(e, rows_chan_geom(e, b)) ? i : -1;
+  }
+  return -1;
+}
+static int launch_rows_or_fused(chz_engine* e, int fuse_bank, unsigned job, int slot, hipStream_t st, const RowsParams& c, Instr* in) {
+  const FwdPlan& p = e->plan;
+  if (fuse_bank < 0) return launch_rows(p.rc, p.grid3, p.block3, p.lds3, st, c, IN_E0(in), IN_E1(in));
+  const Bank& b = e->banks[(size_t)fuse_bank];
+  const RowsChanGeom g = rows_chan_geom(e, b);
+  RowsChanParams q{};
+  q.r = c;
+  if (!chan_layout(q.c, SpecLayout{p.Na, p.spec_pitch, p.spec_off}, e->bins)) return -1;
+  q.c.spec = e->spec[slot]; q.c.resp = b.resp; q.c.desc = b.desc + (size_t)slot * b.cap; q.c.out = bank_out(b, slot);
+  q.c.ch0 = 0; q.c.nch = b.active; q.c.olen = b.olen; q.c.tw_sub = b.tw_sub; q.c.stage = 0; q.c.job = job;
+  q.grid3 = p.grid3; q.flag_off = (int)(g.lds / sizeof(float2)) - 1;
+  q.cnt = e->rows_chan_cnt + 2 * slot; q.target = e->rows_chan_base[slot] + (unsigned)p.grid3;
+  q.err = e->notch_err; q.max_wait = e->notch_max_wait;
+  if (launch_rows_chan(p.rc, b.g.r, p.grid3 + g.grid, p.block3, g.lds, st, q, IN_E0(in), IN_E1(in))) return -1;
+  e->rows_chan_base[slot] += (unsigned)p.grid3;
+  __atomic_fetch_add(&e->rows_chan_fused, 1LL, __ATOMIC_RELAXED);
+  return 0;
+}
+
+static int enqueue_forward(chz_engine* e, unsigned job, Instr* in, NotchTurn* turn = nullptr, int seq = 0, bool capture_first = false, bool capturing = false,
+                           int fuse_bank = -1) {
   const FwdPlan& p = e->plan;
   const int slot = job % CHZ_ND;
   const int ln = lane_of(e, job, in);
@@ -925,7 +997,7 @@
       c.nf.adv = seq == e->capture_blocks - 1 ? (unsigned)e->capture_blocks : 0u;
     } else if (ticket) { c.nf.ver = e->notch_ver; c.nf.seq = e->notch_tickets; }
     mark(in, st, 2, true);
-    const int lr = launch_rows(p.rc, p.grid3, p.block3, p.lds3, st, c, IN_E0(in), IN_E1(in));
+    const int lr = launch_rows_or_fused(e, fuse_bank, job, slot, st, c, in);
     mark(in, st, 2, false);
     if (!lr && ticket && !capturing) e->notch_tickets++;
     if (turn) {
@@ -936,7 +1008,7 @@
     return 0;
   }
   mark(in, st, 2, true);
-  if (launch_rows(p.rc, p.grid3, p.block3, p.lds3, st, c, IN_E0(in), IN_E1(in))) return fail(-4, "no kernel for axis c");
+  if (launch_rows_or_fused(e, fuse_bank, job, slot, st, c, in)) return fail(-4, "no kernel for axis c");
   mark(in, st, 2, false);
   return enqueue_notch(e, slot, st, in, turn, seq, capture_first, capturing);
 }
@@ -1818,8 +1890,19 @@
   return 0;
 }
 
-static int enqueue_step(chz_engine* e, unsigned job, Instr* in, NotchTurn* turn = nullptr, int seq = 0, bool capture_first = false, bool capturing = false) {
-  int r = enqueue_forward(e, job, in, turn, seq, capture_first, capturing);
+static int enqueue_step(chz_engine* e, unsigned job, Instr* in, NotchTurn* turn = nullptr, int seq = 0, bool capture_first = false, bool capturing = false,
+                        bool eager = false) {
+  const int fused = rows_chan_pick(e, eager && !capturing && !(in && in->on));
+  if (fused >= 0) {
+    Bank& b = e->banks[(size_t)fused];
+    const int slot = (int)(job % CHZ_ND);
+    hipStream_t st = e->lanes[lane_of(e, (unsigned)slot, in)].s;
+    __atomic_store_n(&b.last_slot, slot, __ATOMIC_RELAXED);
+    { int rr = refresh_slot(e, b, slot, st); if (rr) return rr; }
+    if (b.tail_used[slot]) HIPOK(hipStreamWaitEvent(st, b.ev_tail[slot], 0));
+    b.agc_peak_valid[slot] = false;
+  }
+  int r = enqueue_forward(e, job, in, turn, seq, capture_first, capturing, fused);
   if (r) return r;
   bool demod = false;
   for (const Bank& b : e->banks) demod = demod || b.dm_on > 0 || b.bb_n > 0;
@@ -1829,7 +1912,7 @@
       __builtin_ia32_pause();
     }
   }
-  for (int b = 0; b < (int)e->banks.size() && !r; b++) r = enqueue_bank(e, b, job, in);
+  for (int b = 0; b < (int)e->banks.size() && !r; b++) if (b != fused) r = enqueue_bank(e, b, job, in);
   if (demod && turn) {
     if (r) turn->abort.store(1, std::memory_order_relaxed);
     turn->next_tail.store(seq + 1, std::memory_order_release);
@@ -1840,11 +1923,12 @@
 int chz_step(chz_engine* e, unsigned job) {
   if (!e) return fail(-1, "null engine");
   HIPOK(hipSetDevice(e->device));
-  int r = enqueue_step(e, job, nullptr);
+  int r = enqueue_step(e, job, nullptr, nullptr, 0, false, false, true);
   if (r) return r;
   HIPOK(hipGetLastError());
   return 0;
 }
+int chz_engine_rows_chan_fused(const chz_engine* e) { return e ? (int)(__atomic_load_n(&e->rows_chan_fused, __ATOMIC_RELAXED) & 0x7fffffff) : -1; }
 
 static int lanes_fork(chz_engine* e, hipEvent_t ev) {
   if (e->nlanes < 2) return 0;
@@ -1926,7 +2010,7 @@
       const unsigned job = job0 + (unsigned)b;
       const int ln = (int)(job % (unsigned)e->nlanes);
       if (host_join && b < e->nlanes) HIPOK(hipEventRecord(e->ev_begin[ln], e->lanes[ln].s));
-      const int r = enqueue_step(e, job, ins, turn, b);
+      const int r = enqueue_step(e, job, ins, turn, b, false, false, true);
       if (r) return r;
       if (host_join && b >= nblocks - e->nlanes) HIPOK(hipEventRecord(e->ev_end[ln], e->lanes[ln].s));
       return 0;
diff --git a/ka9q-radio_amd/csrc/chz_kernels.h b/ka9q-radio_amd/csrc/chz_kernels.h
--- a/ka9q-radio_amd/csrc/chz_kernels.h
+++ b/ka9q-radio_amd/csrc/chz_kernels.h
@@ -505,9 +505,8 @@
 }
 
 template <int R1, int R2>
-__global__ void fwd_rows(RowsParams p) {
+__device__ __forceinline__ void fwd_rows_body(const RowsParams& p, float2* lds) {
   constexpr int NC = R1 * R2;
-  HIP_DYNAMIC_SHARED(float2, lds)
   const int tid = threadIdx.x, nthr = blockDim.x;
   const int Ta = p.Ta, ld = p.ld, padg = p.padg;
   const int kb = blockIdx.x % p.Nb, at = blockIdx.x / p.Nb;
@@ -631,6 +630,11 @@
   }
   if (nf_owner) rows_notch_publish(p.nf, tid);
 }
+template <int R1, int R2>
+__global__ void fwd_rows(RowsParams p) {
+  HIP_DYNAMIC_SHARED(float2, lds)
+  fwd_rows_body<R1, R2>(p, lds);
+}
 
 struct NotchFixParams {
   float2* spec;
@@ -706,19 +710,18 @@
 #endif
 }
 
-template <int R1, int R2, int EPI>
-__global__ void __launch_bounds__(256, (R1 <= 15 && R2 <= 20) ? (EPI == 0 ? 6 : (EPI == 1 ? 5 : 1)) : 1) chan_ifft(ChanParams p) {
+template <int R1, int R2, int EPI, bool PRE, class Ready>
+__device__ __forceinline__ void chan_ifft_body(const ChanParams& p, float2* lds, const int bid, Ready ready) {
   constexpr int P = R1 * R2;
   constexpr int LPC = R1 > R2 ? R1 : R2;
   constexpr int CPW = 64 / LPC;
   constexpr int LDC = R2 + 1;
   static_assert(CPW >= 1, "radix too wide for one wavefront");
-  HIP_DYNAMIC_SHARED(float2, lds)
   const int tid = threadIdx.x;
   const int wave = tid >> 6, lane = tid & 63;
   const int wpb = blockDim.x >> 6;
   const int cw = lane / LPC, jl = lane - cw * LPC;
-  const int lc = (blockIdx.x * wpb + wave) * CPW + cw;
+  const int lc = (bid * wpb + wave) * CPW + cw;
   const int ch = p.ch0 + lc;
   const bool live = (cw < CPW) && (lc < p.nch);
   float2* my = lds + ((wave * CPW + (cw < CPW ? cw : 0)) * (R1 * LDC));
@@ -726,8 +729,24 @@
 
   float2 v[R1];
   const bool act1 = live && jl < R2;
+  constexpr bool PRE_TW = PRE && R1 <= 16;
+  ChanDesc d_pre{};
+  float2 h_pre[PRE ? R1 : 1], tw_pre[PRE_TW ? R1 : 1];
+  if constexpr (PRE) {
+    if (act1) {
+      d_pre = p.desc[ch];
+      const float2* __restrict__ Hp = p.resp + (long)d_pre.row * P + jl;
+      static_for<R1>([&](auto q) {
+        constexpr int Q = decltype(q)::value;
+        h_pre[Q] = CHZ_LOAD_RESP(Hp + Q * R2);
+        if constexpr (PRE_TW && Q > 0) tw_pre[Q] = tws[jl * R1 + Q];
+      });
+    }
+  }
+  if (!ready()) return;
   if (act1) {
-    const ChanDesc d = p.desc[ch];
+    ChanDesc d;
+    if constexpr (PRE) d = d_pre; else d = p.desc[ch];
     const float2* __restrict__ H = p.resp + (long)d.row * P;
     const float2* __restrict__ X = p.spec;
     float2 h[R1];
@@ -747,7 +766,7 @@
       if (d.wrap && src >= d.wrap) src -= d.wrap;
       if (!ok[Q]) src = 0;
       v[Q] = CHZ_LOAD2(xdesc, X, spec_index(p.lay.off, p.magic, p.dpitch, src));
-      h[Q] = CHZ_LOAD_RESP(Hl + Q * R2);
+      if constexpr (PRE) h[Q] = h_pre[Q]; else h[Q] = CHZ_LOAD_RESP(Hl + Q * R2);
       if constexpr (EPI == 2) srcs[Q] = src;
     });
     bool beamed = false;
@@ -824,7 +843,7 @@
     static_for<R1>([&](auto k1) {
       constexpr int K1 = decltype(k1)::value;
       float2 x = v[K1];
-      if constexpr (K1 > 0) x = cmul(x, tws[jl * R1 + K1]);
+      if constexpr (K1 > 0) { if constexpr (PRE_TW) x = cmul(x, tw_pre[K1]); else x = cmul(x, tws[jl * R1 + K1]); }
       my[K1 * LDC + jl] = x;
     });
   }
@@ -927,7 +946,7 @@
     }
   }
   if (p.stage) {
-    const int first_lc = (blockIdx.x * wpb + wave) * CPW;
+    const int first_lc = (bid * wpb + wave) * CPW;
     int nl = p.nch - first_lc; if (nl > CPW) nl = CPW;
     const int tot2 = nl > 0 ? (nl * p.olen) >> 1 : 0;
     const float2* wl = lds + (wave * CPW) * (R1 * LDC);
@@ -949,6 +968,80 @@
     for (int d = 32; d >= 1; d >>= 1) if (d < LPC) { const double o = __shfl_down(tot, (unsigned)d); if (jl + d < LPC) tot += o; }
     if (live && jl == 0) p.power[ch] = tot / (double)p.olen;
   }
+}
+template <int R1, int R2, int EPI>
+__global__ void __launch_bounds__(256, (R1 <= 15 && R2 <= 20) ? (EPI == 0 ? 6 : (EPI == 1 ? 5 : 1)) : 1) chan_ifft(ChanParams p) {
+  HIP_DYNAMIC_SHARED(float2, lds)
+  chan_ifft_body<R1, R2, EPI, false>(p, lds, (int)blockIdx.x, [] { return true; });
+}
+
+struct RowsChanParams {
+  RowsParams r;
+  ChanParams c;
+  int grid3;
+  int flag_off;
+  unsigned* cnt;
+  unsigned target;
+  unsigned* err;
+  long long max_wait;
+};
+#define CHZ_ROWS_CHAN_ERR 0x40000000u
+__device__ __forceinline__ void rows_chan_hand_in(unsigned* cnt) {
+#if defined(__HIP_DEVICE_COMPILE__)
+  asm volatile("s_waitcnt vmcnt(0)" ::: "memory");
+  __syncthreads();
+  if (threadIdx.x == 0) {
+#if !CHZ_WT
+    __builtin_amdgcn_fence(__ATOMIC_RELEASE, "agent");
+#endif
+    asm volatile("s_waitcnt vmcnt(0)" ::: "memory");
+    (void)__hip_atomic_fetch_add(cnt, 1u, __ATOMIC_RELAXED, __HIP_MEMORY_SCOPE_AGENT);
+  }
+#else
+  __syncthreads();
+  if (threadIdx.x == 0) *cnt += 1u;
+#endif
+}
+__device__ __forceinline__ bool rows_chan_wait(const RowsChanParams& p, float2* lds) {
+  unsigned* flag = reinterpret_cast<unsigned*>(lds + p.flag_off);
+  if (threadIdx.x == 0) {
+    unsigned ok = 0u;
+#if defined(__HIP_DEVICE_COMPILE__)
+    if (__hip_atomic_load(p.cnt + 1, __ATOMIC_RELAXED, __HIP_MEMORY_SCOPE_AGENT) == 0u) {
+      const long long t0 = wall_clock64();
+      for (;;) {
+        const unsigned v = __hip_atomic_load(p.cnt, __ATOMIC_RELAXED, __HIP_MEMORY_SCOPE_AGENT);
+        if ((int)(v - p.target) >= 0) { ok = 1u; break; }
+        if (wall_clock64() - t0 > p.max_wait) break;
+        __builtin_amdgcn_s_sleep(8);
+      }
+      if (!ok) {
+        __hip_atomic_store(p.cnt + 1, 1u, __ATOMIC_RELAXED, __HIP_MEMORY_SCOPE_AGENT);
+        __hip_atomic_store(p.err, CHZ_ROWS_CHAN_ERR | (p.target & 0x3fffffffu), __ATOMIC_RELAXED, __HIP_MEMORY_SCOPE_SYSTEM);
+      }
+    }
+#else
+    if (p.cnt[1] == 0u && (int)(p.cnt[0] - p.target) >= 0) ok = 1u;
+    else { p.cnt[1] = 1u; *p.err = CHZ_ROWS_CHAN_ERR | (p.target & 0x3fffffffu); }
+#endif
+    *flag = ok;
+  }
+  __syncthreads();
+  const bool ok = *flag != 0u;
+#if defined(__HIP_DEVICE_COMPILE__)
+  __builtin_amdgcn_fence(__ATOMIC_ACQUIRE, "agent");
+#endif
+  return ok;
+}
+template <int R1, int R2, int C1, int C2>
+__global__ void __launch_bounds__((R1 > R2 ? R1 : R2) * 16 / 64 * 64 + ((R1 > R2 ? R1 : R2) * 16 % 64 ? 64 : 0), 4) fwd_rows_chan(RowsChanParams p) {
+  HIP_DYNAMIC_SHARED(float2, lds)
+  if ((int)blockIdx.x < p.grid3) {
+    fwd_rows_body<R1, R2>(p.r, lds);
+    rows_chan_hand_in(p.cnt);
+    return;
+  }
+  chan_ifft_body<C1, C2, 0, true>(p.c, lds, (int)blockIdx.x - p.grid3, [&] { return rows_chan_wait(p, lds); });
 }
 
 template <int R1, int R2>
diff --git a/ka9q-radio_amd/csrc/chz_launch.h b/ka9q-radio_amd/csrc/chz_launch.h
--- a/ka9q-radio_amd/csrc/chz_launch.h
+++ b/ka9q-radio_amd/csrc/chz_launch.h
@@ -53,6 +53,18 @@
     else { CHZ_LAUNCH((chan_ifft<a, b, 0>), grid, block, lds, s, e0, e1, p); } \
     return 0; }
   CHZ_CHAN_MENU(X)
+#undef X
+  return -1;
+}
+inline int rows_chan_per_wg(const FwdPlan& p, const ChanGeom& g) { return (p.block3 / 64) * g.cpw; }
+inline size_t rows_chan_bank_lds(const FwdPlan& p, const ChanGeom& g) { return sizeof(f2) * (size_t)rows_chan_per_wg(p, g) * g.r.r1 * (g.r.r2 + 1); }
+inline size_t rows_chan_lds(const FwdPlan& p, const ChanGeom& g) {
+  const size_t b = rows_chan_bank_lds(p, g);
+  return (p.lds3 > b ? p.lds3 : b) + sizeof(f2);
+}
+inline int launch_rows_chan(Radix2 r, Radix2 c, int grid, int block, size_t lds, hipStream_t s, const RowsChanParams& p, hipEvent_t e0 = nullptr, hipEvent_t e1 = nullptr) {
+#define X(a, b, c1, c2) if (r.r1 == a && r.r2 == b && c.r1 == c1 && c.r2 == c2) { CHZ_LAUNCH((fwd_rows_chan<a, b, c1, c2>), grid, block, lds, s, e0, e1, p); return 0; }
+  CHZ_ROWS_CHAN_MENU(X)
 #undef X
   return -1;
 }
diff --git a/ka9q-radio_amd/csrc/chz_plan.h b/ka9q-radio_amd/csrc/chz_plan.h
--- a/ka9q-radio_amd/csrc/chz_plan.h
+++ b/ka9q-radio_amd/csrc/chz_plan.h
@@ -17,7 +17,11 @@
   X(4, 5) X(5, 6) X(10, 15) X(10, 16) X(10, 20) X(15, 20) X(16, 20) X(20, 20) X(20, 24) \
   X(24, 25) X(25, 32) X(30, 32) X(30, 40) X(40, 48)
 
+#define CHZ_ROWS_CHAN_MENU(X) \
+  X(9, 16, 15, 20) X(10, 16, 15, 20) X(10, 16, 24, 25)
+
 struct Radix2 { int r1, r2; };
+inline bool rows_chan_menu_has(Radix2 r, Radix2 c);
 
 inline bool fwd_menu_lookup(int np, Radix2* out) {
 #define X(a, b) if ((a) * (b) == np) { if (out) { out->r1 = a; out->r2 = b; } return true; }
@@ -30,6 +34,12 @@
   CHZ_FWD_MENU(X)
 #undef X
   return fwd_menu_lookup(np, out);
+}
+inline bool rows_chan_menu_has(Radix2 r, Radix2 c) {
+#define X(a, b, c1, c2) if (r.r1 == a && r.r2 == b && c.r1 == c1 && c.r2 == c2) return true;
+  CHZ_ROWS_CHAN_MENU(X)
+#undef X
+  return false;
 }
 inline bool chan_menu_lookup(int p, Radix2* out) {
 #define X(a, b) if ((a) * (b) == p) { if (out) { out->r1 = a; out->r2 = b; } return true; }
diff --git a/ka9q-radio_amd/engine.py b/ka9q-radio_amd/engine.py
--- a/ka9q-radio_amd/engine.py
+++ b/ka9q-radio_amd/engine.py
@@ -54,7 +54,7 @@
     "chz_bank_set_tuning", "chz_bank_read_power", "chz_bank_read_power_async",
     "chz_input_write_i16", "chz_input_write_i16_device", "chz_input_stats",
     "chz_bank_enable_noise", "chz_bank_read_noise", "chz_bank_read_noise_async", "chz_bank_create_real", "chz_bank_set_isb", "chz_bank_set_beam",
-    "chz_set_notches_alpha", "chz_slot_sync", "chz_engine_check", "chz_input_seek", "chz_input_mark", "chz_input_mark_wait", "chz_engine_notch_order",
+    "chz_set_notches_alpha", "chz_slot_sync", "chz_engine_check", "chz_input_seek", "chz_input_mark", "chz_input_mark_wait", "chz_engine_notch_order", "chz_engine_rows_chan_fused",
     "chz_bank_set_demod", "chz_bank_pcm_stride", "chz_bank_set_pcm_stride", "chz_bank_read_pcm", "chz_bank_read_pcm_async",
     "chz_comm_unique_id", "chz_comm_create", "chz_comm_create_file", "chz_comm_destroy", "chz_comm_rank", "chz_comm_world",
     "chz_mini_create", "chz_mini_destroy", "chz_mini_capacity", "chz_mini_add", "chz_mini_release", "chz_mini_set_response", "chz_mini_execute",
@@ -66,7 +66,7 @@
 ]
 
 ENV_OPTIONS = {"CHZ_CHAN_STAGE": "chan_stage", "CHZ_NOISE_ENERGY": "noise_energy", "CHZ_DEMOD_WAVE": "demod_wave", "CHZ_ENQ_THREADS": "enq_threads",
-               "CHZ_GRAPH_BLOCKS": "graph_blocks", "CHZ_NOTCH_FOLD": "notch_fold", "CHZ_NOISE_HINT": "noise_hint", "CHZ_PLL_LANE0": "pll_lane0",
+               "CHZ_GRAPH_BLOCKS": "graph_blocks", "CHZ_NOTCH_FOLD": "notch_fold", "CHZ_ROWS_CHAN_FUSE": "rows_chan_fuse", "CHZ_NOISE_HINT": "noise_hint", "CHZ_PLL_LANE0": "pll_lane0",
                "CHZ_NOTCH_WAIT_MS": "notch_wait_ms", "CHZ_FAULT_TICKET_SKEW": "fault_ticket_skew", "CHZ_ALLOW_FAULT_INJECTION": "allow_fault_injection",
                "CHZ_LAUNCH_ID": "launch_id"}
 
@@ -109,6 +109,7 @@
         L.chz_set_notches_alpha.argtypes = [_vp, _vp, _vp, _i]
         L.chz_slot_sync.argtypes = [_vp, _i]
         L.chz_engine_check.argtypes = [_vp]
+        L.chz_engine_rows_chan_fused.argtypes = [_vp]
         L.chz_bank_set_demod.argtypes = [_vp, _i, _u, _i, _i, _vp, _d]
         L.chz_bank_pcm_stride.argtypes = [_vp, _i]
         L.chz_bank_set_pcm_stride.argtypes = [_vp, _i, _i]
@@ -274,6 +275,9 @@
     def check(self):
         _check(lib().chz_engine_check(self._h))
 
+    def rows_chan_fused(self):
+        return _check(lib().chz_engine_rows_chan_fused(self._h))
+
     def slot_sync(self, slot):
         _check(lib().chz_slot_sync(self._h, slot))
 
```
